# kalj/dealii-cuda

Measured on AMD Instinct MI355X. Metric: DoFs/s on 1305x Laplace vmult (bmop), p=4 3D uniform, higher is better.
Workload: dtype f64; 1 GPU; bmop: DEGREE_FE=4, DIMENSION=3, MATRIX_FREE_UNIFORM_MESH, hyper_cube(-1,1), 54^3 cells, 10218313 DoFs, 1 z-slab(s); cells_per_dir=54, n_dofs=10218313, n_cells=157464, parallelism=slab1, dof_numbering=caller's (lexicographic), finite=True, clock_ramp_steps=2000

## Files before the change

### dealii-cuda_amd/csrc/mfgpu_api.hip

```cpp
#include <hip/hip_runtime.h>

#include <type_traits>

#include <algorithm>
#include <cmath>
#include <cstdlib>
#include <cstring>
#include <memory>
#include <string>
#include <vector>

#include "mfgpu_kernels.h"

using namespace mfgpu;

struct EventTimer {
  std::vector<Event> ev;
  size_t used = 0;
  double ms = 0.0;
  int begin(hipStream_t st) {
    if (used + 2 > ev.size()) {
      Event e0, e1;
      int rc;
      if ((rc = e0.create(hipEventDefault)) || (rc = e1.create(hipEventDefault))) return rc;
      ev.push_back(std::move(e0));
      ev.push_back(std::move(e1));
    }
    HIP_TRY(hipEventRecord(ev[used].get(), st));
    return 0;
  }
  int end(hipStream_t st) {
    HIP_TRY(hipEventRecord(ev[used + 1].get(), st));
    used += 2;
    return 0;
  }
  int drain(double *total) {
    for (size_t i = 0; i + 1 < used; i += 2) {
      float t = 0.f;
      HIP_TRY(hipEventElapsedTime(&t, ev[i].get(), ev[i + 1].get()));
      ms += t;
    }
    used = 0;
    *total = ms;
    return 0;
  }
  void reset() {
    used = 0;
    ms = 0.0;
  }
};

struct mfgpu_handle {
  Plan plan;
  int dim = 0, n = 0, nd = 0, number_type = MFGPU_F64;
  bool hn = false;
  std::vector<double> S, Dt;
  std::vector<double> sv, sg;
  DeviceArray<uint32_t> d_batch_cell_off, d_batch_dof_off, d_bdofs;
  DeviceArray<uint8_t> d_bflags;
  DeviceArray<uint16_t> d_lmap;
  DeviceArray<uint16_t> d_lmapx;
  DeviceArray<uint16_t> d_perm;
  DeviceArray<uint32_t> d_bdofsp, d_idxp;
  DeviceArray<uint32_t> d_shtab;
  bool shared_records = false;
  size_t record_bytes = 0;
  DeviceArray<uint32_t> d_hnrec;
  DeviceArray<uint32_t> d_hn_slot;
  DeviceArray<void> d_coefp;
  DeviceArray<void> d_coef;
  DeviceArray<void> d_mass, d_massp;
  bool updatable = false;
  FoldGeometry geo;
  DeviceArray<uint32_t> d_cell_batch, d_cell_pos;
  size_t n_plane_cells = 0;
  DeviceArray<uint32_t> d_cmask, d_orphans;
  DeviceArray<void> d_hnw;
  DeviceArray<uint32_t> d_constrained;
  uint32_t n_constrained = 0;
  DeviceArray<void> d_tabsd;
  DeviceArray<void> d_tab2;
  bool twopass = true;
  DeviceArray<uint32_t> d_batch_nint, d_halo_off;
  std::vector<uint32_t> seg_end;
  std::vector<DeviceArray<uint32_t>> d_p2arr, d_p2tiles;
  std::vector<uint32_t> n_p2tiles;
  DeviceArray<uint32_t> d_p2rec, d_p2tab;
  bool p2_shared = false, p2_reverse = false, no_shared_records = false;
  Stream side;
  std::vector<Event> ev_seg;
  Event ev_side;
  bool side_pending = false;
  DeviceArray<void> d_halo;
  DeviceArray<unsigned long long> d_stamps;
  size_t lds = 0, device_bytes = 0;
  PlaneKernel planes = PlaneKernel::none;
  BatchKernel batches = BatchKernel::none;
  enum { kPlain, kMasked, kBatch };
  CellKernel<double> kernels_f64[3];
  CellKernel<float> kernels_f32[3];
  template <typename T>
  CellKernel<T> &kernel(int which) {
    if constexpr (std::is_same<T, double>::value) return kernels_f64[which];
    else return kernels_f32[which];
  }
  MultiKernel<double> multi_f64[kMaxFusedWidth - 1];
  MultiKernel<float> multi_f32[kMaxFusedWidth - 1];
  template <typename T>
  MultiKernel<T> &multi(int width) {
    if constexpr (std::is_same<T, double>::value) return multi_f64[width - 2];
    else return multi_f32[width - 2];
  }
  int multi_width = 1;
  DeviceArray<void> d_halo_multi;
  size_t halo_bytes = 0;
  uint32_t n_cus = 0, max_workgroups = 0;
  bool prof = false;
  EventTimer t_cells;
  EventTimer t_pass2;
  uint64_t prof_vmults = 0;
};

namespace {

template <typename T>
hipError_t bind_kernel(const mfgpu_handle *h, PlaneKernel pk, BatchKernel bk, bool hn, bool sh, CellKernel<T> *k) {
  const Plan &P = h->plan;
  const auto bind = pk == PlaneKernel::planes3 ? p_bind<T> : pk == PlaneKernel::planes4 ? q_bind<T>
                    : bk == BatchKernel::batches ? apply_bind<T> : bk == BatchKernel::x ? x_bind<T>
                    : bk == BatchKernel::g ? g_bind<T> : bk == BatchKernel::g2 ? g2_bind<T> : nullptr;
  if (!bind) return hipErrorInvalidValue;
  return bind(P.dim, P.n, hn, h->twopass, sh, h->d_mass.get() != nullptr, P.max_batch_dofs, k);
}

template <typename T>
int launch_bound(mfgpu_handle *h, int which, const ApplyArgs<T> &a, uint32_t nbat, hipStream_t st) {
  const CellKernel<T> &k = h->kernel<T>(which);
  if (!k.launch[0]) {
    set_error("cell-loop kernel not bound");
    return MFGPU_EINVAL;
  }
  uint32_t grid = (uint32_t)(k.per_cu < 1 ? 1 : k.per_cu) * h->n_cus;
  if (h->max_workgroups && h->max_workgroups < grid) grid = h->max_workgroups;
  HIP_TRY(k.launch[a.add != 0](a, h->S.data(), h->Dt.data(), k.lds, nbat < grid ? nbat : grid, st));
  return 0;
}

int check_symmetrize(int n, std::vector<double> &S, std::vector<double> &Dt) {
  const int p = n - 1;
  double err = 0, mag = 0;
  for (int r = 0; r < n; ++r)
    for (int c = 0; c < n; ++c) {
      const double s1 = S[r * n + c], s2 = S[(p - r) * n + (p - c)];
      const double d1 = Dt[r * n + c], d2 = -Dt[(p - r) * n + (p - c)];
      err = std::fmax(err, std::fmax(std::fabs(s1 - s2), std::fabs(d1 - d2)));
      mag = std::fmax(mag, std::fmax(std::fabs(s1), std::fabs(d1)));
    }
  if (err > 1e-10 * mag) {
    set_error("shape tables are not symmetric about the cell midpoint (unsupported)");
    return MFGPU_EUNSUPPORTED;
  }
  for (int r = 0; r < n; ++r)
    for (int c = 0; c < n; ++c) {
      const int r2 = p - r, c2 = p - c;
      if (r * n + c < r2 * n + c2) {
        const double s = 0.5 * (S[r * n + c] + S[r2 * n + c2]);
        S[r * n + c] = S[r2 * n + c2] = s;
        const double d = 0.5 * (Dt[r * n + c] - Dt[r2 * n + c2]);
        Dt[r * n + c] = d;
        Dt[r2 * n + c2] = -d;
      } else if (r == r2 && c == c2) {
        Dt[r * n + c] = 0.0;
      }
    }
  return 0;
}

int upload_pass2(mfgpu_handle *h, const uint32_t *priority, uint32_t n_priority) {
  const Plan &P = h->plan;
  std::vector<uint8_t> prio(P.n_dofs, 0);
  for (uint32_t i = 0; i < n_priority; ++i) {
    if (priority[i] >= P.n_dofs) {
      set_error("priority dof out of range");
      return MFGPU_EINVAL;
    }
    prio[priority[i]] = 1;
  }
  const size_t ng = 1 + h->seg_end.size();
  const bool shared = P.sh_p2_use && !h->no_shared_records && n_priority == 0 && ng == 2;
  std::vector<std::vector<uint32_t>> sd(ng), so(ng, std::vector<uint32_t>(1, 0u)), si(ng);
  auto add = [&](uint32_t dof, const uint32_t *slots, uint32_t k, size_t seg) {
    const size_t g = prio[dof & 0x7fffffffu] ? 0 : 1 + seg;
    sd[g].push_back(dof);
    si[g].insert(si[g].end(), slots, slots + k);
    so[g].push_back((uint32_t)si[g].size());
  };
  for (size_t i = 0; i < P.sdofs.size(); ++i) {
    size_t seg = 0;
    if (shared && P.s_off[i + 1] > P.s_off[i]) continue;
    if (P.s_off[i + 1] > P.s_off[i]) {
      const uint32_t slot = P.s_idx[P.s_off[i + 1] - 1];
      const uint32_t batch = (uint32_t)(std::upper_bound(P.halo_off.begin(), P.halo_off.end(), slot) - P.halo_off.begin()) - 1;
      seg = (size_t)(std::upper_bound(h->seg_end.begin(), h->seg_end.end(), batch) - h->seg_end.begin());
      if (seg >= h->seg_end.size()) seg = h->seg_end.size() - 1;
    }
    add(P.sdofs[i], P.s_idx.data() + P.s_off[i], P.s_off[i + 1] - P.s_off[i], seg);
  }
  const uint32_t zero_slot = P.halo_off.empty() ? 0u : P.halo_off.back();
  for (uint32_t orph : P.orphans) add(orph, &zero_slot, 1, 0);
  std::vector<DeviceArray<uint32_t>> d_arr(ng), d_tiles(ng);
  std::vector<uint32_t> n_tiles(ng, 0u);
  const bool reverse = (size_t)P.halo_off.back() * esize(h->number_type) <= ((size_t)256 << 20);
  DeviceArray<uint32_t> d_rec, d_tab;
  if (shared) {
    int rc;
    if ((rc = d_rec.upload(P.sh_p2rec.data(), P.sh_p2rec.size()))) return rc;
    if ((rc = d_tab.upload(P.sh_p2tab.data(), P.sh_p2tab.size()))) return rc;
  }
  for (size_t g = 0; g < ng; ++g) {
    std::vector<uint32_t> arr, tiles;
    build_pass2_classes(sd[g], so[g], si[g], arr, tiles);
    n_tiles[g] = (uint32_t)(tiles.size() / 4);
    if (reverse) {
      const size_t nt = tiles.size() / 4;
      for (size_t a = 0, b = nt ? nt - 1 : 0; a < b; ++a, --b)
        for (int w = 0; w < 4; ++w) std::swap(tiles[4 * a + w], tiles[4 * b + w]);
    }
    int rc;
    if ((rc = d_arr[g].upload(arr.data(), arr.size()))) return rc;
    if ((rc = d_tiles[g].upload(tiles.data(), tiles.size()))) return rc;
  }
  h->d_p2arr = std::move(d_arr);
  h->d_p2tiles = std::move(d_tiles);
  h->n_p2tiles = std::move(n_tiles);
  h->d_p2rec = std::move(d_rec);
  h->d_p2tab = std::move(d_tab);
  h->p2_shared = shared;
  h->p2_reverse = reverse;
  return 0;
}

template <typename T>
int relayout_planes(mfgpu_handle *h, const uint32_t *cell_batch, const uint32_t *cell_pos, bool coef, bool mass,
                    hipStream_t st) {
  const size_t total = h->n_plane_cells * (size_t)h->nd;
  if (coef)
    HIP_TRY(relayout_coef_launch<T>(h->d_coefp.as<T>(), h->d_coef.as<const T>(), cell_batch, cell_pos, total, h->n, st));
  if (mass)
    HIP_TRY(relayout_coef_launch<T>(h->d_massp.as<T>(), h->d_mass.as<const T>(), cell_batch, cell_pos, total, h->n, st));
  return 0;
}

template <typename T>
int update_typed(mfgpu_handle *h, const void *coef, const void *mass, hipStream_t st) {
  const FoldInputs<T> in = h->geo.inputs<T>();
  if (coef) HIP_TRY(fold_coefficient_launch<T>(h->d_coef.as<T>(), (const T *)coef, in, st));
  if (mass) HIP_TRY(fold_mass_launch<T>(h->d_mass.as<T>(), (const T *)mass, in, st));
  if (h->planes == PlaneKernel::none) return 0;
  return relayout_planes<T>(h, h->d_cell_batch.get(), h->d_cell_pos.get(), coef != nullptr, mass != nullptr, st);
}

template <typename T>
int create_arrays(mfgpu_handle *h, const mfgpu_desc &d) {
  const Plan &P = h->plan;
  const size_t ncell = P.n_cells, nd = (size_t)P.nd;
  size_t &acct = h->device_bytes;
  auto up = [&](auto &arr, const void *src, size_t n) {
    const int rc = arr.upload(src, n);
    acct += arr.bytes();
    return rc;
  };
  int rc;
  if ((rc = up(h->d_batch_cell_off, P.batch_cell_off.data(), P.batch_cell_off.size()))) return rc;
  if ((rc = up(h->d_batch_dof_off, P.batch_dof_off.data(), P.batch_dof_off.size()))) return rc;
  if ((rc = up(h->d_bdofs, P.bdofs.data(), P.bdofs.size()))) return rc;
  if ((rc = up(h->d_bflags, P.bflags.data(), P.bflags.size()))) return rc;
  if ((rc = up(h->d_lmap, P.lmap.data(), P.lmap.size()))) return rc;
  const bool general = h->batches == BatchKernel::g || h->batches == BatchKernel::g2;
  if (h->batches == BatchKernel::x && !h->hn) {
    const int n = P.n, n2 = n * n, PP = n2, CH = 256 / PP, ndl = n2 * n;
    std::vector<uint16_t> perm(512, 0xffff);
    for (int layout = 0; layout < 2; ++layout) {
      uint16_t *lanes = perm.data() + 256 * layout;
      std::vector<int> fill(32, 0), overflow;
      for (int q = 0; q < CH * PP; ++q) {
        const int cell = q / PP, pen = q % PP, a = pen % n, b = pen / n;
        const int base = cell * ndl + (layout == 0 ? a + n2 * b : a + n * b);
        const int r = base & 31;
        if (fill[r] < 8) lanes[32 * fill[r]++ + r] = (uint16_t)q;
        else overflow.push_back(q);
      }
      for (int l = 255; l >= 0 && !overflow.empty(); --l)
        if (lanes[l] == 0xffff) {
          lanes[l] = (uint16_t)overflow.back();
          overflow.pop_back();
        }
    }
    if ((rc = up(h->d_perm, perm.data(), perm.size()))) return rc;
  }
  if (h->batches == BatchKernel::x || general) {
    const size_t n = (size_t)P.n, np = (n + 1) & ~(size_t)1, runs = P.lmap.size() / n;
    std::vector<uint16_t> lx(runs * np, 0);
    for (size_t r = 0; r < runs; ++r)
      for (size_t i = 0; i < n; ++i) lx[r * np + i] = P.lmap[r * n + i];
    if ((rc = up(h->d_lmapx, lx.data(), lx.size()))) return rc;
  }
  if (h->batches == BatchKernel::g2) {
    std::vector<T> sd(2 * (size_t)P.n * P.n);
    for (int i = 0; i < P.n * P.n; ++i) {
      sd[i] = (T)h->S[i];
      sd[P.n * P.n + i] = (T)h->Dt[i];
    }
    if ((rc = up(h->d_tabsd, sd.data(), sd.size() * sizeof(T)))) return rc;
  }
  if (h->planes != PlaneKernel::none) {
    if ((rc = build_plane_records(h->plan, d.constraint_mask))) return rc;
    if (!P.pr_hn.empty()) {
      if ((rc = up(h->d_hnrec, P.pr_hn.data(), P.pr_hn.size()))) return rc;
      if ((rc = up(h->d_hn_slot, P.pr_hn_slot.data(), P.pr_hn_slot.size()))) return rc;
    }
    h->shared_records = P.sh_use && !(d.flags & MFGPU_NO_SHARED_RECORDS) &&
                        kernel_exists(h->planes, P.n, d.number_type, false, true, d.mass_coefficient != nullptr);
    const std::vector<uint32_t> &rd = h->shared_records ? P.sh_dofs : P.pr_dofs;
    const std::vector<uint32_t> &rx = h->shared_records ? P.sh_idx : P.pr_idx;
    if ((rc = up(h->d_bdofsp, rd.data(), rd.size()))) return rc;
    if ((rc = up(h->d_idxp, rx.data(), rx.size()))) return rc;
    if (h->shared_records && (rc = up(h->d_shtab, P.sh_batch.data(), P.sh_batch.size()))) return rc;
    h->record_bytes = h->d_bdofsp.bytes() + h->d_idxp.bytes() + h->d_shtab.bytes();
  }
  if ((rc = up(h->d_orphans, P.orphans.data(), P.orphans.size()))) return rc;
  if (h->twopass) {
    if ((rc = up(h->d_batch_nint, P.batch_nint.data(), P.batch_nint.size()))) return rc;
    if ((rc = up(h->d_halo_off, P.halo_off.data(), P.halo_off.size()))) return rc;
    if (h->planes != PlaneKernel::none && (uint64_t)P.halo_off.back() >= (1ull << 29)) {
      set_error("halo buffer too large for 32-bit byte offsets");
      return MFGPU_EUNSUPPORTED;
    }
    const size_t hb = ((size_t)P.halo_off.back() + 1) * sizeof(T);
    if ((rc = h->d_halo.alloc(hb, true))) return rc;
    acct += hb;
    h->halo_bytes = hb;
  }
  if (h->hn) {
    std::vector<uint32_t> cm(ncell);
    for (size_t i = 0; i < ncell; ++i) cm[i] = d.constraint_mask[P.cell_order[i]];
    if ((rc = up(h->d_cmask, cm.data(), ncell))) return rc;
    std::vector<T> w((size_t)h->n * h->n);
    for (size_t i = 0; i < w.size(); ++i) w[i] = (T)d.constraint_weights[i];
    if ((rc = up(h->d_hnw, w.data(), w.size() * sizeof(T)))) return rc;
  }
  FoldGeometry geo;
  if ((rc = geo.upload(d.JxW, d.inv_jac, P.cell_order.data(), P.dim, (uint32_t)ncell, (uint32_t)nd, general,
                       d.number_type)))
    return rc;
  DeviceArray<T> metric;
  if ((rc = fold_coefficient<T>(metric, d.coefficient, d.quadrature_points, geo.inputs<T>()))) return rc;
  h->d_coef = std::move(metric);
  acct += h->d_coef.bytes();
  if (d.mass_coefficient) {
    DeviceArray<T> mass;
    if ((rc = fold_mass<T>(mass, d.mass_coefficient, geo.inputs<T>()))) return rc;
    h->d_mass = std::move(mass);
    acct += h->d_mass.bytes();
  }
  if (h->updatable) {
    acct += geo.bytes();
    h->geo = std::move(geo);
  }
  if (h->planes != PlaneKernel::none) {
    const int n = P.n, NT = p_cells_per_wave(n) * n;
    const size_t nbat = P.n_plane_batches, total = nbat * (size_t)(n * n) * NT;
    const size_t ncell_p = P.batch_cell_off[nbat];
    std::vector<uint32_t> cb(ncell_p), cp(ncell_p);
    for (size_t b = 0; b < nbat; ++b)
      for (uint32_t c = P.batch_cell_off[b]; c < P.batch_cell_off[b + 1]; ++c) {
        cb[c] = (uint32_t)b;
        cp[c] = c - P.batch_cell_off[b];
      }
    DeviceArray<uint32_t> t_cb, t_cp;
    if ((rc = t_cb.upload(cb.data(), ncell_p))) return rc;
    if ((rc = t_cp.upload(cp.data(), ncell_p))) return rc;
    if ((rc = h->d_coefp.alloc(total * sizeof(T), true))) return rc;
    acct += h->d_coefp.bytes();
    h->n_plane_cells = ncell_p;
    if (d.mass_coefficient) {
      if ((rc = h->d_massp.alloc(total * sizeof(T), true))) return rc;
      acct += h->d_massp.bytes();
    }
    if ((rc = relayout_planes<T>(h, t_cb.get(), t_cp.get(), true, d.mass_coefficient != nullptr, nullptr))) return rc;
    HIP_TRY(hipDeviceSynchronize());
    if (h->updatable) {
      acct += t_cb.bytes() + t_cp.bytes();
      h->d_cell_batch = std::move(t_cb);
      h->d_cell_pos = std::move(t_cp);
    }
  }
  int dev = 0;
  hipDeviceProp_t prop;
  HIP_TRY(hipGetDevice(&dev));
  HIP_TRY(hipGetDeviceProperties(&prop, dev));
  h->n_cus = (uint32_t)prop.multiProcessorCount;
  h->max_workgroups = d.max_workgroups;
  if (h->planes != PlaneKernel::none) {
    CellKernel<T> &plain = h->kernel<T>(mfgpu_handle::kPlain), &masked = h->kernel<T>(mfgpu_handle::kMasked);
    HIP_TRY(bind_kernel<T>(h, h->planes, BatchKernel::none, false, h->shared_records, &plain));
    h->lds = plain.lds;
    if (P.n_plain_plane_batches < P.n_plane_batches) {
      HIP_TRY(bind_kernel<T>(h, h->planes, BatchKernel::none, true, false, &masked));
      h->lds = std::max(h->lds, masked.lds);
    }
  }
  if (h->batches == BatchKernel::none) return 0;
  CellKernel<T> &batch = h->kernel<T>(mfgpu_handle::kBatch);
  const hipError_t bind_batch_family = bind_kernel<T>(h, PlaneKernel::none, h->batches, h->hn, false, &batch);
  h->lds = batch.lds;
  if (h->lds > 160 * 1024) {
    set_error("batch needs more than 160 KiB of LDS; lower max_dofs_per_batch");
    return MFGPU_EINVAL;
  }
  HIP_TRY(bind_batch_family);
  if (h->twopass && h->planes == PlaneKernel::none)
    for (const int w : kFusedWidths) {
      if (!fused_kernel_exists(h->batches, P.n, d.number_type, h->hn, h->d_mass.get() != nullptr, w)) continue;
      MultiKernel<T> &mk = h->multi<T>(w);
      if (gm_bind<T>(P.n, h->hn, h->d_mass.get() != nullptr, w, P.max_batch_dofs, &mk) != hipSuccess) {
        (void)hipGetLastError();
        mk = MultiKernel<T>();
      } else
        h->multi_width = std::max(h->multi_width, w);
    }
  return 0;
}

void choose_segments(mfgpu_handle *h, uint32_t request) {
  const Plan &P = h->plan;
  const uint32_t nb = (uint32_t)(P.batch_cell_off.size() - 1);
  h->seg_end.assign(1, nb);
  if (!h->twopass || nb < 2 || request == 1) return;
  const uint32_t npl = P.n_plane_batches, nplain = P.n_plain_plane_batches;
  std::vector<uint32_t> cuts;
  if (npl > 0 && npl < nb) cuts.push_back(npl);
  if (nplain > 0 && nplain < npl) cuts.push_back(nplain);
  if (request > 1) {
    for (uint32_t i = 1; i < request; ++i) cuts.push_back((uint32_t)((uint64_t)nb * i / request));
  }
  if (request == 0 && !P.pr_hn.empty() && nplain == 0 && P.n == 5) cuts.push_back(nb / 2);
  std::sort(cuts.begin(), cuts.end());
  h->seg_end.clear();
  for (uint32_t c : cuts)
    if (c > 0 && c < nb && (h->seg_end.empty() || h->seg_end.back() != c)) h->seg_end.push_back(c);
  h->seg_end.push_back(nb);
}

template <typename T>
int create_typed(mfgpu_handle *h, const mfgpu_desc &d) {
  int rc = create_arrays<T>(h, d);
  if (rc) return rc;
  choose_segments(h, d.cell_loop_segments);
  if (!h->twopass) return 0;
  if (h->seg_end.size() > 1) {
    int prio_least = 0, prio_greatest = 0;
    HIP_TRY(hipDeviceGetStreamPriorityRange(&prio_least, &prio_greatest));
    if ((rc = h->side.create(hipStreamNonBlocking, prio_least))) return rc;
    if ((rc = h->ev_side.create(hipEventDisableTiming))) return rc;
    h->ev_seg.resize(h->seg_end.size() - 1);
    for (Event &e : h->ev_seg)
      if ((rc = e.create(hipEventDisableTiming))) return rc;
  }
  return upload_pass2(h, nullptr, 0);
}

template <typename T>
int launch_pass2_group(mfgpu_handle *h, size_t group, void *dst, const void *src, hipStream_t st, int add) {
  if (h->p2_shared && group == 1)
    HIP_TRY(reduce_owner_batches_launch<T>((T *)dst, (const T *)src, h->d_halo.as<const T>(), h->d_p2rec.get(),
                                           h->d_p2tab.get(), (uint32_t)(h->plan.batch_cell_off.size() - 1),
                                           (uint32_t)p_hs(h->plan.n) * 64u, h->p2_reverse ? 1 : 0, add, st));
  HIP_TRY(reduce_classes_launch<T>((T *)dst, (const T *)src, h->d_halo.as<const T>(), h->d_p2arr[group].get(),
                                   h->d_p2tiles[group].get(), h->n_p2tiles[group], add, st));
  return 0;
}

template <typename T>
int vmult_pass2(mfgpu_handle *h, int phase, void *dst, const void *src, hipStream_t st, int add) {
  if (!h->twopass) return 0;
  if (phase == 0) return launch_pass2_group<T>(h, 0, dst, src, st, add);
  int rc = launch_pass2_group<T>(h, h->seg_end.size(), dst, src, st, add);
  if (!rc && h->side_pending) {
    HIP_TRY(hipStreamWaitEvent(st, h->ev_side.get(), 0));
    h->side_pending = false;
  }
  return rc;
}

template <typename T>
int launch_cells(mfgpu_handle *h, ApplyArgs<T> a, uint32_t b0, uint32_t b1, hipStream_t st) {
  const Plan &P = h->plan;
  const uint32_t npl = P.n_plane_batches, nplain = P.n_plain_plane_batches;
  if (b0 < nplain) {
    a.batch0 = b0;
    a.batch_end = b1 < nplain ? b1 : nplain;
    if (const int rc = launch_bound<T>(h, mfgpu_handle::kPlain, a, a.batch_end - a.batch0, st)) return rc;
    b0 = a.batch_end;
  }
  if (b0 < npl && b0 < b1) {
    a.batch0 = b0;
    a.batch_end = b1 < npl ? b1 : npl;
    if (const int rc = launch_bound<T>(h, mfgpu_handle::kMasked, a, a.batch_end - a.batch0, st)) return rc;
    b0 = a.batch_end;
  }
  if (b0 >= b1) return 0;
  a.batch0 = b0;
  a.batch_end = b1;
  return launch_bound<T>(h, mfgpu_handle::kBatch, a, b1 - b0, st);
}

template <typename T>
ApplyArgs<T> make_args(mfgpu_handle *h, void *dst, const void *src, int add) {
  const Plan &P = h->plan;
  ApplyArgs<T> a;
  a.batch_cell_off = h->d_batch_cell_off.get();
  a.batch_dof_off = h->d_batch_dof_off.get();
  a.bdofs = h->d_bdofs.get();
  a.bflags = h->d_bflags.get();
  a.lmap = h->d_lmap.get();
  a.lmapx = h->d_lmapx.get();
  a.perm = h->d_perm.get();
  a.bdofsp = h->d_bdofsp.get();
  a.idxp = h->d_idxp.get();
  a.shtab = h->shared_records ? h->d_shtab.get() : nullptr;
  a.hnrec = h->d_hnrec.get();
  a.hn_slot = h->d_hn_slot.get();
  a.coefp = h->d_coefp.as<const T>();
  a.coef = h->d_coef.as<const T>();
  a.mass = h->d_mass.as<const T>();
  a.massp = h->d_massp.as<const T>();
  a.cmask = h->d_cmask.get();
  a.hn_weights = h->d_hnw.as<const T>();
  a.tabS = h->d_tabsd.as<const T>();
  a.tabDt = a.tabS ? a.tabS + (size_t)P.n * P.n : nullptr;
  a.batch_nint = h->d_batch_nint.get();
  a.halo_off = h->d_halo_off.get();
  a.halo = h->d_halo.as<T>();
  a.dst = (T *)dst;
  a.src = (const T *)src;
  a.nb_max = P.max_batch_dofs;
  a.add = add;
  a.stamps = h->d_stamps.get();
  a.dbg = 0;
  return a;
}

template <typename T>
int vmult_main(mfgpu_handle *h, void *dst, const void *src, hipStream_t st, int add) {
  const Plan &P = h->plan;
  ApplyArgs<T> a = make_args<T>(h, dst, src, add);
  int rc;
  if (h->prof && (rc = h->t_cells.begin(st))) return rc;
  if (h->twopass) {
    const size_t nseg = h->seg_end.size();
    if (h->side_pending) {
      HIP_TRY(hipStreamWaitEvent(st, h->ev_side.get(), 0));
      h->side_pending = false;
    }
    for (size_t s = 0; s < nseg; ++s) {
      if ((rc = launch_cells<T>(h, a, s ? h->seg_end[s - 1] : 0u, h->seg_end[s], st))) return rc;
      if (s + 1 < nseg) {
        HIP_TRY(hipEventRecord(h->ev_seg[s].get(), st));
        HIP_TRY(hipStreamWaitEvent(h->side.get(), h->ev_seg[s].get(), 0));
        if ((rc = launch_pass2_group<T>(h, 1 + s, dst, src, h->side.get(), add))) return rc;
      }
    }
    if (nseg > 1) {
      HIP_TRY(hipEventRecord(h->ev_side.get(), h->side.get()));
      h->side_pending = true;
    }
  } else {
    for (size_t c = 0; c + 1 < P.color_batch_off.size(); ++c) {
      if (P.color_batch_off[c + 1] == P.color_batch_off[c]) continue;
      if ((rc = launch_cells<T>(h, a, P.color_batch_off[c], P.color_batch_off[c + 1], st))) return rc;
    }
  }
  if (h->prof && (rc = h->t_cells.end(st))) return rc;
  if (!h->twopass)
    HIP_TRY(orphan_launch<T>((T *)dst, (const T *)src, h->d_orphans.get(), (uint32_t)P.orphans.size(), add, st));
  if (h->prof) h->prof_vmults++;
  return 0;
}

template <typename T>
int vmult_typed(mfgpu_handle *h, void *dst, const void *src, hipStream_t st, int add) {
  int rc = vmult_main<T>(h, dst, src, st, add);
  if (rc) return rc;
  const bool timed = h->prof && h->twopass;
  if (timed && (rc = h->t_pass2.begin(st))) return rc;
  rc = vmult_pass2<T>(h, 0, dst, src, st, add);
  if (!rc) rc = vmult_pass2<T>(h, 1, dst, src, st, add);
  if (!rc && timed) rc = h->t_pass2.end(st);
  return rc;
}

bool fused_by_default(int , int ) { return false; }

template <typename T>
int multi_fused_group(mfgpu_handle *h, T *dst, const T *src, int nv, size_t stride, hipStream_t st, int add) {
  const MultiKernel<T> &k = h->multi<T>(nv);
  if (!k.launch[0]) {
    set_error("fused kernel not bound");
    return MFGPU_EINVAL;
  }
  if (!h->d_halo_multi.get()) {
    const size_t bytes = (size_t)(h->multi_width - 1) * h->halo_bytes;
    if (const int rc = h->d_halo_multi.alloc(bytes, true)) return rc;
    HIP_TRY(hipStreamSynchronize(nullptr));
    h->device_bytes += bytes;
  }
  if (h->side_pending) {
    HIP_TRY(hipStreamWaitEvent(st, h->ev_side.get(), 0));
    h->side_pending = false;
  }
  MultiArgs<T> a;
  static_cast<ApplyArgs<T> &>(a) = make_args<T>(h, dst, src, add);
  a.stride = stride;
  for (int v = 0; v < kMaxFusedWidth; ++v)
    a.halos[v] = v == 0 ? a.halo
                 : v < nv ? reinterpret_cast<T *>(static_cast<char *>(h->d_halo_multi.get()) + (size_t)(v - 1) * h->halo_bytes)
                          : nullptr;
  const uint32_t nbat = (uint32_t)(h->plan.batch_cell_off.size() - 1);
  a.batch0 = 0;
  a.batch_end = nbat;
  uint32_t grid = (uint32_t)(k.per_cu < 1 ? 1 : k.per_cu) * h->n_cus;
  if (h->max_workgroups && h->max_workgroups < grid) grid = h->max_workgroups;
// ... 187 lines not shown
    set_error("JxW, inv_jac, shape tables and coefficient (or quadrature_points) are required");
    return MFGPU_EINVAL;
  }
  const bool hn = (d.flags & MFGPU_HANGING_NODES) != 0;
  if (hn && (!d.constraint_mask || !d.constraint_weights)) {
    set_error("MFGPU_HANGING_NODES needs constraint_mask and constraint_weights");
    return MFGPU_EINVAL;
  }
  std::unique_ptr<mfgpu_handle, decltype(&mfgpu_destroy)> h(new mfgpu_handle(), mfgpu_destroy);
  int rc = choose_kernel_and_plan(d, h->planes, h->batches, h->plan);
  if (rc) return rc;
  h->dim = d.dim;
  h->n = d.degree + 1;
  h->nd = h->plan.nd;
  h->number_type = d.number_type;
  h->hn = hn;
  h->twopass = !(d.flags & MFGPU_COLORED_SCATTER);
  h->no_shared_records = (d.flags & MFGPU_NO_SHARED_RECORDS) != 0;
  h->updatable = (d.flags & MFGPU_UPDATABLE_COEFFICIENTS) != 0;
  const int nn = h->n * h->n;
  std::vector<double> sv(nn), sg(nn);
  for (int i = 0; i < nn; ++i) {
    sv[i] = d.number_type == MFGPU_F64 ? ((const double *)d.shape_values)[i] : ((const float *)d.shape_values)[i];
    sg[i] = d.number_type == MFGPU_F64 ? ((const double *)d.shape_gradients)[i] : ((const float *)d.shape_gradients)[i];
  }
  h->sv = sv;
  h->sg = sg;
  rc = derive_tables(h->n, sv.data(), sg.data(), h->S, h->Dt);
  if (!rc) rc = check_symmetrize(h->n, h->S, h->Dt);
  if (!rc) rc = d.number_type == MFGPU_F64 ? create_typed<double>(h.get(), d) : create_typed<float>(h.get(), d);
  if (!rc && d.n_constrained) {
    h->n_constrained = d.n_constrained;
    rc = h->d_constrained.upload(d.constrained_dofs, d.n_constrained);
    h->device_bytes += h->d_constrained.bytes();
  }
  if (rc) return rc;
  *out = h.release();
  return 0;
}

void mfgpu_destroy(mfgpu_handle *h) {
  if (!h) return;
  if (h->side.get()) hipStreamSynchronize(h->side.get());
  delete h;
}

int mfgpu_vmult(mfgpu_handle *h, void *dst, const void *src, void *stream) {
  if (!h || !dst || !src) {
    set_error("null argument");
    return MFGPU_EINVAL;
  }
  if (dst == src) {
    set_error("vmult: dst and src must not alias");
    return MFGPU_EINVAL;
  }
  return h->number_type == MFGPU_F64 ? vmult_typed<double>(h, dst, src, (hipStream_t)stream, 0)
                                     : vmult_typed<float>(h, dst, src, (hipStream_t)stream, 0);
}

int mfgpu_vmult_add(mfgpu_handle *h, void *dst, const void *src, void *stream) {
  if (!h || !dst || !src) {
    set_error("null argument");
    return MFGPU_EINVAL;
  }
  if (dst == src) {
    set_error("vmult_add: dst and src must not alias");
    return MFGPU_EINVAL;
  }
  return h->number_type == MFGPU_F64 ? vmult_typed<double>(h, dst, src, (hipStream_t)stream, 1)
                                     : vmult_typed<float>(h, dst, src, (hipStream_t)stream, 1);
}

int mfgpu_vmult_multi(mfgpu_handle *h, void *dst, const void *src, uint32_t n_vectors, size_t stride, uint32_t flags,
                      void *stream) {
  if (!h || !dst || !src) {
    set_error("null argument");
    return MFGPU_EINVAL;
  }
  const size_t nd = h->plan.n_dofs;
  if (n_vectors == 0 || (n_vectors > 1 && stride < nd)) {
    set_error("mfgpu_vmult_multi: n_vectors must be >= 1 and stride >= n_dofs");
    return MFGPU_EINVAL;
  }
  if ((flags & ~(MFGPU_MULTI_ADD | MFGPU_MULTI_LOOP | MFGPU_MULTI_FUSED)) ||
      ((flags & MFGPU_MULTI_LOOP) && (flags & MFGPU_MULTI_FUSED))) {
    set_error("mfgpu_vmult_multi: bad flags (MFGPU_MULTI_LOOP and MFGPU_MULTI_FUSED exclude each other)");
    return MFGPU_EINVAL;
  }
  const size_t bytes = ((size_t)(n_vectors - 1) * stride + nd) * esize(h->number_type);
  const char *d0 = (const char *)dst, *s0 = (const char *)src;
  if (d0 < s0 + bytes && s0 < d0 + bytes) {
    set_error("mfgpu_vmult_multi: the dst range overlaps the src range");
    return MFGPU_EINVAL;
  }
  return h->number_type == MFGPU_F64 ? vmult_multi_typed<double>(h, dst, src, n_vectors, stride, flags, (hipStream_t)stream)
                                     : vmult_multi_typed<float>(h, dst, src, n_vectors, stride, flags, (hipStream_t)stream);
}

int mfgpu_multi_width(const mfgpu_handle *h) { return h ? h->multi_width : 0; }

int mfgpu_update_coefficients(mfgpu_handle *h, const void *coefficient_dev, const void *mass_coefficient_dev,
                              void *stream) {
  if (!h) {
    set_error("null argument");
    return MFGPU_EINVAL;
  }
  if (!h->updatable) {
    set_error("mfgpu_update_coefficients: the handle was created without MFGPU_UPDATABLE_COEFFICIENTS");
    return MFGPU_EINVAL;
  }
  if (!coefficient_dev && !mass_coefficient_dev) {
    set_error("mfgpu_update_coefficients: coefficient_dev and mass_coefficient_dev are both NULL");
    return MFGPU_EINVAL;
  }
  if (mass_coefficient_dev && !h->d_mass.get()) {
    set_error("mfgpu_update_coefficients: the handle was created without a mass term (its kernels have no mass "
              "instantiation bound); create it with mass_coefficient");
    return MFGPU_EINVAL;
  }
  return h->number_type == MFGPU_F64 ? update_typed<double>(h, coefficient_dev, mass_coefficient_dev, (hipStream_t)stream)
                                     : update_typed<float>(h, coefficient_dev, mass_coefficient_dev, (hipStream_t)stream);
}

uint32_t mfgpu_n_dofs(const mfgpu_handle *h) { return h ? h->plan.n_dofs : 0; }

size_t mfgpu_memory_consumption(const mfgpu_handle *h) { return h ? h->device_bytes : 0; }

int mfgpu_plan_stats(const mfgpu_handle *h, uint64_t s[8]) {
  if (!h || !s) return MFGPU_EINVAL;
  const Plan &P = h->plan;
  s[0] = P.batch_cell_off.size() - 1;
  s[1] = P.color_batch_off.size() - 1;
  s[2] = P.bdofs.size();
  s[3] = P.max_batch_dofs;
  s[4] = P.max_batch_cells;
  s[5] = P.orphans.size();
  s[6] = P.n_first;
  s[7] = P.n_add;
  if (h->twopass) {
    const uint32_t nb = (uint32_t)s[0], npl = P.n_plane_batches, nplain = P.n_plain_plane_batches;
    const uint32_t edge[4] = {0u, nplain, npl, nb};
    s[1] = 0;
    for (size_t g = 0; g < h->seg_end.size(); ++g) {
      const uint32_t s0 = g ? h->seg_end[g - 1] : 0u, s1 = h->seg_end[g];
      for (int f = 0; f < 3; ++f)
        if (std::max(s0, edge[f]) < std::min(s1, edge[f + 1])) ++s[1];
    }
    s[6] = P.sdofs.size();
    s[7] = P.halo_off.back();
  }
  return 0;
}

int mfgpu_record_stats(const mfgpu_handle *h, uint64_t s[4]) {
  if (!h || !s) return MFGPU_EINVAL;
  const Plan &P = h->plan;
  const size_t n = (size_t)P.n, nb = (size_t)p_kgu((int)n) * 64, nx = ((n * n + 1) / 2) * (p_cells_per_wave((int)n) * n);
  const bool planes = h->planes != PlaneKernel::none;
  s[0] = (h->shared_records ? 1 : 0) | (h->p2_shared ? 2 : 0);
  s[1] = planes ? P.sh_dofs.size() / nb : 0;
  s[2] = planes ? P.sh_idx.size() / nx : 0;
  s[3] = h->record_bytes;
  return 0;
}

const char *mfgpu_kernel_name(const mfgpu_handle *h) {
  if (!h) return "";
  const bool x = h->batches == BatchKernel::x;
  switch (h->planes) {
    case PlaneKernel::planes3: return x ? "apply_planes3+apply_batches_x" : "apply_planes3";
    case PlaneKernel::planes4: return x ? "apply_planes4+apply_batches_x" : "apply_planes4";
    default: break;
  }
  switch (h->batches) {
    case BatchKernel::x: return "apply_batches_x";
    case BatchKernel::g: return "apply_batches_g";
    case BatchKernel::g2: return "apply_batches_g2";
    default: return "apply_batches";
  }
}

int mfgpu_profile_enable(mfgpu_handle *h, int on) {
  if (!h) return MFGPU_EINVAL;
  h->prof = on != 0;
  h->t_cells.reset();
  h->t_pass2.reset();
  h->prof_vmults = 0;
  return 0;
}

int mfgpu_profile_read_pass2(mfgpu_handle *h, double *ms) {
  if (!h || !ms) return MFGPU_EINVAL;
  HIP_TRY(hipDeviceSynchronize());
  return h->t_pass2.drain(ms);
}

int mfgpu_profile_read(mfgpu_handle *h, double *ms, uint64_t *nv) {
  if (!h || !ms || !nv) return MFGPU_EINVAL;
  HIP_TRY(hipDeviceSynchronize());
  if (const int rc = h->t_cells.drain(ms)) return rc;
  *nv = h->prof_vmults;
  return 0;
}

#ifdef MFGPU_STAMPS
int mfgpu_debug_stamps(mfgpu_handle *h, unsigned long long *out, size_t n_batches) {
  if (!h) return MFGPU_EINVAL;
  const size_t nbt = h->plan.batch_cell_off.size() - 1;
  if (!h->d_stamps.get()) return h->d_stamps.alloc(2 * nbt * 16, true);
  if (out && n_batches == nbt) {
    HIP_TRY(hipDeviceSynchronize());
    HIP_TRY(hipMemcpy(out, h->d_stamps.get(), 2 * nbt * 16 * sizeof(unsigned long long), hipMemcpyDeviceToHost));
  }
  return 0;
}
#endif


int mfgpu_compute_inverse_diagonal(mfgpu_handle *h, void *inv_diag, void *stream) {
  if (!h || !inv_diag) {
    set_error("null argument");
    return MFGPU_EINVAL;
  }
  return h->number_type == MFGPU_F64 ? inverse_diagonal_typed<double>(h, inv_diag, (hipStream_t)stream)
                                     : inverse_diagonal_typed<float>(h, inv_diag, (hipStream_t)stream);
}

int mfgpu_set_constrained_values(mfgpu_handle *h, void *vec, double value, void *stream) {
  if (!h || !vec) {
    set_error("null argument");
    return MFGPU_EINVAL;
  }
  if (h->number_type == MFGPU_F64)
    HIP_TRY(set_values_launch<double>((double *)vec, h->d_constrained.get(), h->n_constrained, value, (hipStream_t)stream));
  else
    HIP_TRY(set_values_launch<float>((float *)vec, h->d_constrained.get(), h->n_constrained, (float)value,
                                     (hipStream_t)stream));
  return 0;
}

int mfgpu_vec_sadd(void *v, double s, double a, const void *w, size_t n, int nt, void *stream) {
  return vec_map(0, v, w, s, a, n, nt, stream);
}
int mfgpu_vec_equ(void *v, double a, const void *w, size_t n, int nt, void *stream) {
  return vec_map(1, v, w, 0.0, a, n, nt, stream);
}
int mfgpu_vec_scale(void *v, const void *w, size_t n, int nt, void *stream) {
  return vec_map(2, v, w, 0.0, 0.0, n, nt, stream);
}
int mfgpu_vec_divide(void *v, const void *w, size_t n, int nt, void *stream) {
  return vec_map(3, v, w, 0.0, 0.0, n, nt, stream);
}
int mfgpu_vec_invert(void *v, size_t n, int nt, void *stream) { return vec_map(4, v, nullptr, 0.0, 0.0, n, nt, stream); }
int mfgpu_vec_mul(void *v, double a, size_t n, int nt, void *stream) {
  return vec_map(5, v, nullptr, 0.0, a, n, nt, stream);
}
int mfgpu_vec_dot(const void *v, const void *w, size_t n, int nt, void *stream, double *result) {
  return vec_reduce(0, const_cast<void *>(v), nullptr, w, 0.0, n, nt, stream, result);
}
int mfgpu_vec_l2_norm(const void *v, size_t n, int nt, void *stream, double *result) {
  int rc = vec_reduce(0, const_cast<void *>(v), nullptr, v, 0.0, n, nt, stream, result);
  if (!rc) *result = std::sqrt(*result);
  return rc;
}
int mfgpu_vec_add_and_dot(void *v, double a, const void *x, const void *w, size_t n, int nt, void *stream,
                          double *result) {
  return vec_reduce(1, v, x, w, a, n, nt, stream, result);
}
int mfgpu_vec_all_zero(const void *v, size_t n, int nt, void *stream, int *result) {
  if (!result) return MFGPU_EINVAL;
  double cnt = 0.0;
  int rc = vec_reduce(2, const_cast<void *>(v), nullptr, nullptr, 0.0, n, nt, stream, &cnt);
  if (!rc) *result = cnt == 0.0;
  return rc;
}

int mfgpu_vec_alloc(void **dev, size_t n, int nt) {
  if (!dev) return MFGPU_EINVAL;
  *dev = nullptr;
  if (n == 0) return 0;
  HIP_TRY(hipMalloc(dev, n * esize(nt)));
  HIP_TRY(hipMemset(*dev, 0, n * esize(nt)));
  return 0;
}
int mfgpu_vec_free(void *dev) {
  if (dev) HIP_TRY(hipFree(dev));
  return 0;
}
int mfgpu_vec_fill(void *dev, size_t n, int nt, double value, void *stream) {
  if (!dev && n) return MFGPU_EINVAL;
  if (nt == MFGPU_F32)
    HIP_TRY(fill_launch<float>((float *)dev, n, (float)value, (hipStream_t)stream));
  else
    HIP_TRY(fill_launch<double>((double *)dev, n, value, (hipStream_t)stream));
  return 0;
}
int mfgpu_vec_from_host(void *dev, const void *host, size_t n, int nt) {
  if (n) HIP_TRY(hipMemcpy(dev, host, n * esize(nt), hipMemcpyHostToDevice));
  return 0;
}
int mfgpu_vec_to_host(void *host, const void *dev, size_t n, int nt) {
  if (n) HIP_TRY(hipMemcpy(host, dev, n * esize(nt), hipMemcpyDeviceToHost));
  return 0;
}
int mfgpu_device_synchronize(void) {
  HIP_TRY(hipDeviceSynchronize());
  return 0;
}
int mfgpu_device_memory_info(size_t *free_bytes, size_t *total_bytes) {
  if (!free_bytes || !total_bytes) return MFGPU_EINVAL;
  HIP_TRY(hipMemGetInfo(free_bytes, total_bytes));
  return 0;
}

}
// ... 1 lines not shown
```

### dealii-cuda_amd/csrc/mfgpu_internal.h

```cpp
#ifndef MFGPU_INTERNAL_H
#define MFGPU_INTERNAL_H

#include <cstdint>
#include <string>
#include <vector>

#include "../../include/mfgpu.h"

namespace mfgpu {

void set_error(const std::string &msg);

inline int ipow(int a, int e) {
  int r = 1;
  for (int i = 0; i < e; ++i) r *= a;
  return r;
}

constexpr int p_cells_per_wave(int n) { return 64 / n; }
constexpr int p_ji(int n) { return n == 3 ? 2 : n == 4 ? 5 : n == 5 ? 9 : n == 6 ? 14 : 23; }
constexpr int p_hs(int n) { return n == 3 ? 3 : n == 4 ? 6 : n == 5 ? 9 : n == 6 ? 14 : 18; }
constexpr int p_kgu(int n) { return p_ji(n) + p_hs(n); }
constexpr int p_cell_stride(int n) {
  int s = n * n * n;
  while ((s & 31) != (n & 31)) ++s;
  return s;
}

constexpr int q_plane_stride(int n) { return n >= 6 ? 65 : n == 5 ? 33 : n == 4 ? 17 : 33; }
constexpr int q_cell_stride(int n) { return n * q_plane_stride(n); }
constexpr int p_priv_max(int n) { return n >= 5 ? 384 : n == 4 ? 256 : 192; }
constexpr int kHnOpRounds = 2;
constexpr int p_hn_rows(int n) { return p_priv_max(n) / 64 + 3 * kHnOpRounds * 3 + 2; }

template <typename T>
constexpr size_t q_region_doubles(int n) {
  const size_t t = ((size_t)(p_cells_per_wave(n) + 1) * q_cell_stride(n) * sizeof(T) + 7) / 8;
  const size_t u = (size_t)p_kgu(n) * 64 + p_priv_max(n);
  return t > u ? t : u;
}
template <typename T>
constexpr size_t q_lds_bytes(int n, bool hn) {
  return (q_region_doubles<T>(n) + (hn ? (size_t)n * n : 0)) * 8;
}

constexpr uint8_t kFlagConstrained = 1;
constexpr uint8_t kFlagAdd = 2;

struct Plan {
  int dim = 0, degree = 0, n = 0, nd = 0;
  uint32_t n_dofs = 0, n_cells = 0;
  std::vector<uint32_t> cell_order;
  std::vector<uint32_t> batch_cell_off;
  std::vector<uint32_t> batch_dof_off;
  std::vector<uint32_t> color_batch_off;
  std::vector<uint32_t> bdofs;
  std::vector<uint8_t> bflags;
  std::vector<uint16_t> lmap;
  std::vector<uint32_t> orphans;
  std::vector<uint32_t> batch_nint;
  std::vector<uint32_t> halo_off;
  std::vector<uint32_t> sdofs;
  std::vector<uint32_t> s_off;
  std::vector<uint32_t> s_idx;
  std::vector<uint32_t> chunks;
  std::vector<uint32_t> gstarts;
  uint32_t max_batch_dofs = 0, max_batch_cells = 0;
  uint32_t n_plane_batches = 0;
  uint32_t n_plain_plane_batches = 0;
  std::vector<uint32_t> pr_dofs, pr_idx, pr_hn, pr_hn_slot;
  std::vector<uint32_t> sh_dofs, sh_idx, sh_batch;
  bool sh_use = false;
  std::vector<uint32_t> sh_p2rec, sh_p2tab;
  bool sh_p2_use = false;
  uint64_t n_first = 0, n_add = 0;
};

struct PlanLimits {
  uint32_t max_cells = 0, max_dofs = 0;
  uint32_t interior_max = 0, shared_max = 0, halo_stride = 0;
  bool segregate_masked = false;
  bool masked_planes = false;
  uint32_t private_max = 0;
};

int build_plan(const mfgpu_desc &d, Plan &plan, uint32_t max_chunks = 3, const PlanLimits *limits = nullptr);

struct HnLine {
  uint16_t node[8];
};
void hn_cell_lines(unsigned mask, int n, std::vector<HnLine> (&lines)[3], std::vector<uint16_t> &nodes);

enum class PlaneKernel : uint8_t { none, planes3, planes4 };
enum class BatchKernel : uint8_t { none, batches, x, g, g2 };
int choose_kernel_and_plan(const mfgpu_desc &d, PlaneKernel &pk, BatchKernel &bk, Plan &plan);

constexpr bool planes4_wide(int n) { return n >= 6; }
constexpr bool kernel_exists(PlaneKernel k, int n, int number_type, bool hn, bool sh, bool mass) {
  switch (k) {
    case PlaneKernel::planes3: return n >= 3 && n <= 5 && !(sh && hn);
    case PlaneKernel::planes4:
      return planes4_wide(n) ? n <= 7 && !hn && !sh && !mass
                             : n >= 3 && !sh && !(mass && n == 5 && number_type == MFGPU_F64);
    default: return false;
  }
}
constexpr bool kernel_exists(BatchKernel k, int n, int , bool , bool sh, bool ) {
  return k != BatchKernel::none && n >= 2 && n <= 7 && !sh;
}
constexpr int kFusedWidths[] = {3, 2};
constexpr bool fused_kernel_exists(BatchKernel k, int n, int number_type, bool hn, bool , int nv) {
  return k == BatchKernel::g && n >= 2 && n <= 7 && (nv == 2 || nv == 3) &&
         !(hn && number_type == MFGPU_F64 && n >= (nv == 3 ? 6 : 7));
}
std::vector<uint32_t> multi_groups(uint32_t n_vectors, const std::vector<uint32_t> &widths);
int build_plane_records(Plan &plan, const uint32_t *constraint_mask);
constexpr int kShBatchWords = 4;
constexpr double kShareMaxFraction = 0.5;
void share_plane_records(Plan &plan);
constexpr int kP2Header = 16, kP2MaxK = 12, kP2SlotBits = 12;
void share_pass2_records(Plan &plan);

int derive_tables(int n, const double *shape_values, const double *shape_gradients,
                  std::vector<double> &S, std::vector<double> &Dt);

int handle_number_type(const mfgpu_handle *h);
int handle_set_priority_dofs(mfgpu_handle *h, const uint32_t *ids, uint32_t n);
int handle_vmult_phase(mfgpu_handle *h, int phase, void *dst, const void *src, void *stream, int add);
int handle_n_batches(const mfgpu_handle *h);
bool handle_ranged_ok(const mfgpu_handle *h);
int handle_batches_touching(const mfgpu_handle *h, const uint32_t *ids, uint32_t n, std::vector<uint8_t> &flags);
int handle_cells_range(mfgpu_handle *h, uint32_t b0, uint32_t b1, void *dst, const void *src, void *stream, int add);
int handle_cells_two_ranges(mfgpu_handle *h, uint32_t b0, uint32_t b1, uint32_t c0, uint32_t c1, void *dst,
                            const void *src, void *stream, int add);
int handle_pass2_group(mfgpu_handle *h, int group, void *dst, const void *src, void *stream, int add);

}

struct mfgpu_plan {
  mfgpu::Plan plan;
};

#endif
```

### dealii-cuda_amd/csrc/mfgpu_kernels.h

```cpp
#ifndef MFGPU_KERNELS_H
#define MFGPU_KERNELS_H

#include <hip/hip_runtime.h>

#include <type_traits>

#include "mfgpu_device.h"
#include "mfgpu_internal.h"

namespace mfgpu {

template <typename T>
struct ApplyArgs {
  const uint32_t *batch_cell_off;
  const uint32_t *batch_dof_off;
  const uint32_t *bdofs;
  const uint8_t *bflags;
  const uint16_t *lmap;
  const uint16_t *lmapx;
  const uint16_t *perm;
  const uint32_t *bdofsp;
  const uint32_t *idxp;
  const T *coefp;
  const uint32_t *hnrec;
  const uint32_t *hn_slot;
  const T *coef;
  const uint32_t *cmask;
  const T *hn_weights;
  const T *tabS, *tabDt;
  const uint32_t *batch_nint;
  const uint32_t *halo_off;
  T *halo;
  T *dst;
  const T *src;
  uint32_t batch0;
  uint32_t batch_end;
  uint32_t hole0 = 0xffffffffu, hole_len = 0;
  uint32_t nb_max;
  int add;
  unsigned long long *stamps;
  int dbg;
  const uint32_t *shtab = nullptr;
  const T *mass = nullptr;
  const T *massp = nullptr;
};

constexpr int kMaxFusedWidth = 3;
template <typename T>
struct MultiArgs : ApplyArgs<T> {
  size_t stride = 0;
  T *halos[kMaxFusedWidth];
};
constexpr size_t kMaxLdsBytes = 160 * 1024;

template <typename T, int n>
struct Tables {
  T S[((n + 1) / 2) * n];
  T Dt[((n + 1) / 2) * n];
};

template <typename T, int n>
inline Tables<T, n> make_tables(const double *S, const double *Dt) {
  Tables<T, n> tab;
  for (int i = 0; i < ((n + 1) / 2) * n; ++i) {
    tab.S[i] = (T)S[i];
    tab.Dt[i] = (T)Dt[i];
  }
  return tab;
}

template <typename T, typename Args = ApplyArgs<T>>
struct CellKernel {
  size_t lds = 0;
  int per_cu = 0;
  hipError_t (*launch[2])(const Args &a, const double *S, const double *Dt, size_t lds, uint32_t grid,
                          hipStream_t st) = {nullptr, nullptr};
};

template <typename T, int Block, auto K, auto MakeTab, typename Args = ApplyArgs<T>>
hipError_t launch_cell_kernel(const Args &a, const double *S, const double *Dt, size_t lds, uint32_t grid,
                              hipStream_t st) {
  if constexpr (std::is_null_pointer_v<decltype(MakeTab)>)
    hipLaunchKernelGGL(K, dim3(grid), dim3(Block), lds, st, a);
  else
    hipLaunchKernelGGL(K, dim3(grid), dim3(Block), lds, st, a, MakeTab(S, Dt));
  return hipGetLastError();
}

template <typename T, int Block, auto K0, auto K1, auto MakeTab, typename Args = ApplyArgs<T>>
hipError_t bind_cell_kernel(size_t lds, CellKernel<T, Args> *k) {
  k->lds = lds;
  for (const void *f : {(const void *)K1, (const void *)K0})
    if (const hipError_t e = hipFuncSetAttribute(f, hipFuncAttributeMaxDynamicSharedMemorySize, (int)lds)) return e;
  k->launch[0] = launch_cell_kernel<T, Block, K0, MakeTab, Args>;
  k->launch[1] = launch_cell_kernel<T, Block, K1, MakeTab, Args>;
  return hipOccupancyMaxActiveBlocksPerMultiprocessor(&k->per_cu, (const void *)K0, Block, lds);
}

template <typename F>
hipError_t dispatch_flags(F &&f) { return f(); }
template <typename F, typename... B>
hipError_t dispatch_flags(F &&f, bool flag, B... rest) {
  return dispatch_flags(
      [&](auto... c) { return flag ? f(std::true_type{}, c...) : f(std::false_type{}, c...); }, rest...);
}
template <typename F, typename... B>
hipError_t dispatch_instantiation(int n, F &&f, B... flags) {
  auto at = [&](auto N) { return dispatch_flags([&](auto... c) { return f(N, c...); }, flags...); };
  switch (n) {
    case 2: return at(std::integral_constant<int, 2>{});
    case 3: return at(std::integral_constant<int, 3>{});
    case 4: return at(std::integral_constant<int, 4>{});
    case 5: return at(std::integral_constant<int, 5>{});
    case 6: return at(std::integral_constant<int, 6>{});
    case 7: return at(std::integral_constant<int, 7>{});
    default: return hipErrorInvalidValue;
  }
}
template <typename T>
constexpr int number_type_of = sizeof(T) == 8 ? MFGPU_F64 : MFGPU_F32;

#define MFGPU_CELL_LOOP_FAMILY(F)                                                                              \
  template <typename T>                                                                                        \
  hipError_t F##_bind(int dim, int n, bool hn, bool twopass, bool sh, bool mass, uint32_t nb_max, CellKernel<T> *k);
MFGPU_CELL_LOOP_FAMILY(apply)
MFGPU_CELL_LOOP_FAMILY(x)
MFGPU_CELL_LOOP_FAMILY(g)
MFGPU_CELL_LOOP_FAMILY(g2)
MFGPU_CELL_LOOP_FAMILY(p)
MFGPU_CELL_LOOP_FAMILY(q)
#undef MFGPU_CELL_LOOP_FAMILY
template <typename T>
using MultiKernel = CellKernel<T, MultiArgs<T>>;
template <typename T>
hipError_t gm_bind(int n, bool hn, bool mass, int nv, uint32_t nb_max, MultiKernel<T> *k);

void build_pass2_classes(const std::vector<uint32_t> &sdofs, const std::vector<uint32_t> &s_off,
                         const std::vector<uint32_t> &s_idx, std::vector<uint32_t> &arr, std::vector<uint32_t> &tiles);
template <typename T>
hipError_t reduce_classes_launch(T *dst, const T *src, const T *halo, const uint32_t *arr, const uint32_t *tiles,
                                 uint32_t n_tiles, int add, hipStream_t st);
template <typename T>
hipError_t reduce_classes_multi_launch(int nv, T *dst, const T *src, size_t stride, T *const *halos, const uint32_t *arr,
                                       const uint32_t *tiles, uint32_t n_tiles, int add, hipStream_t st);
template <typename T>
hipError_t reduce_owner_batches_launch(T *dst, const T *src, const T *halo, const uint32_t *rec, const uint32_t *tab,
                                       uint32_t n_batches, uint32_t hstride, int reverse, int add, hipStream_t st);
template <typename T>
hipError_t relayout_coef_launch(T *out, const T *in, const uint32_t *cell_batch, const uint32_t *cell_pos,
                                size_t total, int n, hipStream_t st);
template <typename T>
hipError_t fold_general_launch(T *M, const T *coef, const T *jxw, const T *jinv, const uint32_t *order,
                               uint32_t n_cells, uint32_t nd, hipStream_t st);
template <typename T>
hipError_t fold_general2_launch(T *M, const T *coef, const T *jxw, const T *jinv, const uint32_t *order,
                                uint32_t n_cells, uint32_t nd, hipStream_t st);
template <typename T>
hipError_t orphan_launch(T *dst, const T *src, const uint32_t *orph, uint32_t n, int add, hipStream_t st);
template <typename T>
hipError_t coefficient_launch(T *coef, const T *qpts, size_t nq, int dim, hipStream_t st);
template <typename T>
hipError_t fold_launch(T *c, const T *coef, const T *jxw, const T *j0, const uint32_t *order,
                       uint32_t n_cells, uint32_t nd, hipStream_t st);
template <typename T>
hipError_t fill_launch(T *v, size_t n, T a, hipStream_t st);
template <typename T>
struct FoldInputs {
  const T *jxw = nullptr, *jinv = nullptr;
  const uint32_t *order = nullptr;
  int dim = 0;
  uint32_t n_cells = 0, nd = 0;
  bool general = false;
  size_t metric_entries() const { return (size_t)n_cells * nd * (general ? (dim == 3 ? 6 : 3) : 1); }
};
template <typename T>
hipError_t fold_coefficient_launch(T *out, const T *coef, const FoldInputs<T> &in, hipStream_t st);
template <typename T>
hipError_t fold_mass_launch(T *out, const T *c, const FoldInputs<T> &in, hipStream_t st);
struct FoldGeometry {
  DeviceArray<void> jxw, jinv;
  DeviceArray<uint32_t> order;
  int dim = 0;
  uint32_t n_cells = 0, nd = 0;
  bool general = false;
  int upload(const void *JxW, const void *inv_jac, const uint32_t *cell_order, int dim_, uint32_t n_cells_, uint32_t nd_,
             bool general_, int number_type);
  size_t bytes() const { return jxw.bytes() + jinv.bytes() + order.bytes(); }
  template <typename T>
  FoldInputs<T> inputs(const T *jxw_resident = nullptr) const {
    FoldInputs<T> in;
    in.jxw = jxw_resident ? jxw_resident : jxw.as<const T>();
    in.jinv = jinv.as<const T>();
    in.order = order.get();
    in.dim = dim, in.n_cells = n_cells, in.nd = nd, in.general = general;
    return in;
  }
};
template <typename T>
int fold_mass(DeviceArray<T> &out, const void *mass_coefficient, const FoldInputs<T> &in);
template <typename T>
int fold_coefficient(DeviceArray<T> &out, const void *coefficient, const void *quadrature_points,
                     const FoldInputs<T> &in);

template <typename T>
hipError_t diag_launch(int dim, int n, T *diag, uint32_t n_batches, const uint32_t *batch_cell_off,
                       const uint32_t *batch_dof_off, const uint32_t *bdofs, const uint16_t *lmap, const T *coef,
                       const uint32_t *cmask, const T *hn_weights, const T *tab2, hipStream_t st);
template <typename T>
hipError_t diag_general_launch(int n, T *diag, uint32_t n_batches, const uint32_t *batch_cell_off,
                               const uint32_t *batch_dof_off, const uint32_t *bdofs, const uint16_t *lmap,
                               const T *metric, const uint32_t *cmask, const T *hn_weights, const T *tab,
                               hipStream_t st);
template <typename T>
hipError_t diag_general2_launch(int n, T *diag, uint32_t n_batches, const uint32_t *batch_cell_off,
                                const uint32_t *batch_dof_off, const uint32_t *bdofs, const uint16_t *lmap,
                                const T *metric, const uint32_t *cmask, const T *hn_weights, const T *tab,
                                hipStream_t st);
template <typename T>
hipError_t diag_mass_launch(int dim, int n, T *diag, uint32_t n_batches, const uint32_t *batch_cell_off,
                            const uint32_t *batch_dof_off, const uint32_t *bdofs, const uint16_t *lmap, const T *mass,
                            const uint32_t *cmask, const T *hn_weights, const T *tab, bool squared, hipStream_t st);
template <typename T>
hipError_t set_values_launch(T *v, const uint32_t *idx, uint32_t n, T value, hipStream_t st);
template <typename T>
hipError_t vec_map_launch(int op, T *v, const T *w, T s, T a, size_t n, hipStream_t st);
template <typename T>
hipError_t vec_reduce_launch(int op, T *v, const T *x, const T *w, T a, size_t n, hipStream_t st, double *out);

}
#endif
```

### dealii-cuda_amd/csrc/mfgpu_kernels_p.hip

```cpp
#include <hip/hip_runtime.h>

#include "mfgpu_cell.h"
#include "mfgpu_kernels.h"
#include "mfgpu_planes.h"

namespace mfgpu {

#define MFGPU_PIN_VMEM() __builtin_amdgcn_sched_barrier(0x380)

template <int n, typename T, bool ADD, bool HN, bool SH = false, bool MASS = false>
__global__ void __launch_bounds__(64) __attribute__((amdgpu_waves_per_eu(1, 1)))
apply_planes3(const ApplyArgs<T> A, const TablesEO<T, n> tab) {
  constexpr int n2 = n * n;
  constexpr int CW = p_cells_per_wave(n);
  constexpr int NT = CW * n;
  constexpr int KGU = p_kgu(n);
  constexpr int JI = p_ji(n);
  constexpr int HS = KGU - JI;
  constexpr int SA = p_cell_stride(n);
  constexpr int NIW = (n2 + 1) / 2;
  extern __shared__ __attribute__((aligned(16))) unsigned char smem_raw[];
  constexpr int PRIV = HN ? p_priv_max(n) : 0;
  double *ua = reinterpret_cast<double *>(smem_raw);
  T *Aw = reinterpret_cast<T *>(ua + KGU * 64 + PRIV + (HN ? n2 : 0));
  T *Bw = Aw + (CW + 1) * SA;
  double *Wl = ua + KGU * 64 + PRIV;

  const int lane = threadIdx.x;
  if (HN) {
    if (lane < n2) Wl[lane] = (double)A.hn_weights[lane];
  }
  const int lc = lane / n, k = lane - lc * n;
  const bool lane_on = lane < NT;
  const int tk = lane_on ? lane : NT - 1;

  uint32_t b, bstride, bend;
  {
    const uint32_t nbt = A.batch_end - A.batch0 - A.hole_len, G = gridDim.x;
    if (G >= 8 && nbt >= G) {
      const uint32_t xcd = blockIdx.x & 7u, slot = blockIdx.x >> 3;
      const uint32_t q = G >> 3, rem = G & 7u;
      const uint32_t wlo = xcd * q + (xcd < rem ? xcd : rem);
      const uint32_t w = q + (xcd < rem ? 1u : 0u);
      b = A.batch0 + (uint32_t)((uint64_t)nbt * wlo / G) + slot;
      bend = A.batch0 + (uint32_t)((uint64_t)nbt * (wlo + w) / G);
      bstride = w;
    } else {
      b = A.batch0 + blockIdx.x;
      bend = A.batch_end - A.hole_len;
      bstride = G;
    }
  }
  if (b >= bend) return;
  const uint32_t hole0 = A.hole0, hole_len = A.hole_len;
  auto next_of = [&](uint32_t x) {
    const uint32_t l = (x >= hole0 ? x - hole_len : x) + bstride;
    return l < bend ? (l >= hole0 ? l + hole_len : l) : x;
  };
  if (b >= hole0) b += hole_len;
  static_assert(kernel_exists(PlaneKernel::planes3, n, number_type_of<T>, HN, SH, MASS), "no such instantiation");
  struct Meta {
    uint32_t base, drec, irec;
  };
  auto meta_request = [&](uint32_t bb) -> uint32_t {
    return A.shtab[(size_t)bb * kShBatchWords + (lane & (kShBatchWords - 1))];
  };
  auto meta_of = [&](uint32_t v) -> Meta {
    return Meta{(uint32_t)__builtin_amdgcn_readlane((int)v, 0), (uint32_t)__builtin_amdgcn_readlane((int)v, 1),
                (uint32_t)__builtin_amdgcn_readlane((int)v, 2)};
  };

  auto load_dofs = [&](uint32_t rec, uint32_t (&g)[KGU]) {
    const uint32_t *p = A.bdofsp + (size_t)rec * (KGU * 64) + lane;
#pragma unroll
    for (int j = 0; j < KGU; ++j) g[j] = SH ? p[j * 64] : nt_load(p + j * 64);
  };
  auto src_at = [&](uint32_t base, uint32_t g) -> T {
    const T *const sp = SH ? A.src + base : A.src;
    return *reinterpret_cast<const T *>(reinterpret_cast<const char *>(sp) + (uint32_t)(g * (uint32_t)sizeof(T)));
  };
  auto dst_at = [&](uint32_t base, uint32_t g) -> T * {
    T *const dp = SH ? A.dst + base : A.dst;
    return reinterpret_cast<T *>(reinterpret_cast<char *>(dp) + (uint32_t)(g * (uint32_t)sizeof(T)));
  };
  auto load_ix = [&](uint32_t rec, uint32_t (&ix)[NIW]) {
    const uint32_t *p = A.idxp + (size_t)rec * (NIW * NT) + tk;
#pragma unroll
    for (int w = 0; w < NIW; ++w) ix[w] = SH ? p[w * NT] : nt_load(p + w * NT);
  };
  auto stage_src = [&](const uint32_t (&g)[KGU], const T (&sv)[KGU]) {
#pragma unroll
    for (int j = 0; j < KGU; ++j) {
      double v = (double)sv[j];
      if (j >= JI) {
        const unsigned long long keep = (unsigned long long)(long long)~((int)g[j] >> 31);
        v = __longlong_as_double((long long)((unsigned long long)__double_as_longlong(v) & keep));
      }
      ua[lane + j * 64] = v;
    }
  };
  auto ixb = [&](const uint32_t (&ix)[NIW], int i) -> uint32_t {
    return (i & 1) ? (ix[i >> 1] >> 16) : (ix[i >> 1] & 0xffffu);
  };
  auto scatter_slot = [&](int j, uint32_t bb, uint32_t base, uint32_t g, T r, T oldv) {
    if (j < JI) {
      *dst_at(base, g) = ADD ? oldv + r : r;
    } else {
      T *const hp = A.halo + (size_t)bb * (HS * 64) + lane;
      hp[(j - JI) * 64] = r;
    }
  };

  uint32_t b1 = next_of(b), b2 = next_of(b1);
  uint32_t Gp[KGU], Gc[KGU], Gn[KGU], Gnn[KGU];
  uint32_t IXc[NIW], IXn[NIW];
  constexpr int CR = PRIV / 64, HROWS = HN ? p_hn_rows(n) : 1;
  uint32_t Hc[HROWS], Hn[HROWS];
  auto load_hn = [&](uint32_t bb, uint32_t (&H)[HROWS]) {
    const uint32_t slot = A.hn_slot[bb];
    if (slot != 0xffffffffu) {
      const uint32_t *p = A.hnrec + (size_t)slot * (HROWS * 64) + lane;
#pragma unroll
      for (int w = 0; w < HROWS; ++w) H[w] = nt_load(p + w * 64);
    } else {
#pragma unroll
      for (int w = 0; w < HROWS; ++w) H[w] = 0u;
    }
  };
  T Cc[n2];
  T Mm[MASS ? n2 : 1];
  T SVn[KGU], R[KGU], old[KGU];
  Meta Mp{0u, 0u, 0u}, Mc = Mp, M1 = Mp, M2 = Mp;
  uint32_t Mv = 0u;
  if (SH) {
    Mc = meta_of(meta_request(b));
    M1 = meta_of(meta_request(b1));
    M2 = meta_of(meta_request(b2));
    Mp = Mc;
  }
  load_dofs(SH ? Mc.drec : b, Gc);
  load_dofs(SH ? M1.drec : b1, Gn);
  load_ix(SH ? Mc.irec : b, IXc);
  if (HN) load_hn(b, Hc);
  constexpr uint32_t kDummyIx = 8u * (uint32_t)(KGU * 64 - 1) * 0x10001u;
#pragma unroll
  for (int w = 0; w < NIW; ++w) IXc[w] = lane_on ? IXc[w] : kDummyIx;
  {
    const T *p = A.coefp + (size_t)b * (n2 * NT) + tk;
#pragma unroll
    for (int r = 0; r < n2; ++r) Cc[r] = nt_load(p + r * NT);
  }
  if (MASS) {
    const T *p = A.massp + (size_t)b * (n2 * NT) + tk;
#pragma unroll
    for (int r = 0; r < n2; ++r) Mm[r] = nt_load(p + r * NT);
  }
#pragma unroll
  for (int j = 0; j < KGU; ++j) {
    SVn[j] = src_at(Mc.base, Gc[j]);
    Gp[j] = Gc[j];
    R[j] = T(0);
    old[j] = T(0);
  }
  stage_src(Gc, SVn);
  WaveSync::sync();

  const int pxy = lc * SA + n2 * k;
  const int pyz = lc * SA + k;
  uint32_t bp = b;

  while (true) {
    const bool has_next = b1 != b;
    constexpr int kH2 = HN ? HROWS - 2 : 0, kH1 = HN ? HROWS - 1 : 0;
    const uint32_t hn_ncopy = HN ? (uint32_t)__builtin_amdgcn_readfirstlane(Hc[kH2] & 0xffffu) : 0u;
    auto hn_count = [&](int dir) -> uint32_t {
      const uint32_t w = dir == 0 ? Hc[kH2] >> 16 : dir == 1 ? Hc[kH1] & 0xffffu : Hc[kH1] >> 16;
      return (uint32_t)__builtin_amdgcn_readfirstlane(w);
    };
    auto hn_pass = [&](int dir, bool transposed, const double (&Wr)[n2]) {
      const uint32_t count = hn_count(dir);
#pragma unroll
      for (int r = 0; r < kHnOpRounds; ++r) {
        if ((uint32_t)(r * 64) >= count) break;
        const bool on = (uint32_t)(r * 64 + lane) < count;
        const uint32_t *ww = &Hc[CR + (dir * kHnOpRounds + r) * 3];
        double v[n], o[n];
        uint32_t pos[n];
#pragma unroll
        for (int t = 0; t < n; ++t) {
          pos[t] = on ? (ww[t >> 1] >> (16 * (t & 1))) & 0xffffu : (uint32_t)(KGU * 64 + PRIV - 1);
          v[t] = ua[pos[t]];
        }
#pragma unroll
        for (int i = 0; i < n; ++i) {
          double acc = 0.0;
#pragma unroll
          for (int k2 = 0; k2 < n; ++k2) acc = fma(transposed ? Wr[k2 * n + i] : Wr[i * n + k2], v[k2], acc);
          o[i] = acc;
        }
        if (on) {
#pragma unroll
          for (int i = 0; i < n; ++i) ua[pos[i]] = o[i];
        }
      }
    };
    if (HN && hn_ncopy) {
      double Wr[n2];
#pragma unroll
      for (int i = 0; i < n2; ++i) Wr[i] = Wl[i];
      double cv[CR > 0 ? CR : 1];
#pragma unroll
      for (int r = 0; r < CR; ++r) cv[r] = (uint32_t)(r * 64 + lane) < hn_ncopy ? ua[Hc[r] & 0xffffu] : 0.0;
#pragma unroll
      for (int r = 0; r < CR; ++r)
        if ((uint32_t)(r * 64 + lane) < hn_ncopy) ua[Hc[r] >> 16] = cv[r];
      WaveSync::sync();
      hn_pass(0, false, Wr);
      WaveSync::sync();
      hn_pass(1, false, Wr);
      WaveSync::sync();
      hn_pass(2, false, Wr);
      WaveSync::sync();
    }
    STAMP(0);
    RSTAMP(8);
    WGSTAMP(10);
    load_dofs(SH ? M2.drec : b2, Gnn);
    load_ix(SH ? M1.irec : b1, IXn);
    if (SH) Mv = meta_request(next_of(b2));
    if (HN) load_hn(b1, Hn);
    if (ADD) {
#pragma unroll
      for (int j = 0; j < JI; ++j) old[j] = *dst_at(Mp.base, Gp[j]);
    }
    STAMP(1);
    auto hookA = [&](int) {};
    auto hookB = [&](int s) {
      MFGPU_PIN_VMEM();
#pragma unroll
      for (int j = (KGU * s) / (5 * n); j < (KGU * (s + 1)) / (5 * n); ++j)
        scatter_slot(j, bp, Mp.base, Gp[j], R[j], old[j]);
#pragma unroll
      for (int j = (KGU * s) / (5 * n); j < (KGU * (s + 1)) / (5 * n); ++j)
        SVn[j] = src_at(M1.base, Gn[j]);
      MFGPU_PIN_VMEM();
    };
    const T *const cnext = A.coefp + (size_t)b1 * (n2 * NT) + tk;
    const T *const mnext = MASS ? A.massp + (size_t)b1 * (n2 * NT) + tk : nullptr;
    auto hookC = [&](int s) {
      MFGPU_PIN_VMEM();
#pragma unroll
      for (int r = (n2 * s) / (2 * n); r < (n2 * (s + 1)) / (2 * n); ++r)
        Cc[r] = nt_load(cnext + r * NT);
      if (MASS) {
#pragma unroll
        for (int r = (n2 * s) / (2 * n); r < (n2 * (s + 1)) / (2 * n); ++r)
          Mm[r] = nt_load(mnext + r * NT);
      }
      MFGPU_PIN_VMEM();
    };

    {
// ... 253 lines not shown
```

### dealii-cuda_amd/csrc/mfgpu_pass2.hip

```cpp
#include <hip/hip_runtime.h>

#include <algorithm>

#include "mfgpu_kernels.h"

namespace mfgpu {

namespace {

template <typename T, int K>
__device__ __forceinline__ void reduce_two(T *__restrict__ dst, const T *__restrict__ src, const T *__restrict__ halo,
                                           const uint32_t *__restrict__ p, uint32_t cnt, uint32_t i0, uint32_t k,
                                           int add) {
  const uint32_t i1 = i0 + 256u;
  const uint32_t d0 = p[i0], d1 = p[i1];
  constexpr int KU = K > 0 ? K : 1;
  uint32_t s0[KU], s1[KU];
#pragma unroll
  for (int t = 0; t < KU; ++t) {
    s0[t] = p[(size_t)(1 + t) * cnt + i0];
    s1[t] = p[(size_t)(1 + t) * cnt + i1];
  }
  const bool on0 = d0 != 0xffffffffu, on1 = d1 != 0xffffffffu;
  const uint32_t g0 = d0 & 0x7fffffffu, g1 = d1 & 0x7fffffffu;
  T v0 = T(0), v1 = T(0), o0 = T(0), o1 = T(0);
  if (on0) {
    if (d0 >> 31) {
      v0 = src[g0];
    } else {
      T q[KU];
#pragma unroll
      for (int t = 0; t < KU; ++t) q[t] = halo[s0[t]];
      v0 = q[0];
#pragma unroll
      for (int t = 1; t < KU; ++t) v0 += q[t];
      if (K == 0)
        for (uint32_t t = 1; t < k; ++t) v0 += halo[p[(size_t)(1 + t) * cnt + i0]];
    }
    if (add) o0 = dst[g0];
  }
  if (on1) {
    if (d1 >> 31) {
      v1 = src[g1];
    } else {
      T q[KU];
#pragma unroll
      for (int t = 0; t < KU; ++t) q[t] = halo[s1[t]];
      v1 = q[0];
#pragma unroll
      for (int t = 1; t < KU; ++t) v1 += q[t];
      if (K == 0)
        for (uint32_t t = 1; t < k; ++t) v1 += halo[p[(size_t)(1 + t) * cnt + i1]];
    }
    if (add) o1 = dst[g1];
  }
  if (on0) dst[g0] = add ? o0 + v0 : v0;
  if (on1) dst[g1] = add ? o1 + v1 : v1;
}

template <typename T>
__global__ void __launch_bounds__(256)
reduce_classes(T *__restrict__ dst, const T *__restrict__ src, const T *__restrict__ halo,
               const uint32_t *__restrict__ arr, const uint4 *__restrict__ tiles, int add) {
  const uint4 td = tiles[blockIdx.x];
  const uint32_t *p = arr + td.x;
  const uint32_t i0 = td.w + threadIdx.x;
  switch (td.y) {
    case 1: reduce_two<T, 1>(dst, src, halo, p, td.z, i0, 1, add); break;
    case 2: reduce_two<T, 2>(dst, src, halo, p, td.z, i0, 2, add); break;
    case 3: reduce_two<T, 3>(dst, src, halo, p, td.z, i0, 3, add); break;
    case 4: reduce_two<T, 4>(dst, src, halo, p, td.z, i0, 4, add); break;
    case 8: reduce_two<T, 8>(dst, src, halo, p, td.z, i0, 8, add); break;
    default: reduce_two<T, 0>(dst, src, halo, p, td.z, i0, td.y, add); break;
  }
}

template <typename T>
struct MultiHalos {
  const T *h[kMaxFusedWidth];
};

template <typename T, int K, int NV>
__device__ __forceinline__ void reduce_two_multi(T *__restrict__ dst, const T *__restrict__ src, size_t stride,
                                                 const MultiHalos<T> &halos, const uint32_t *__restrict__ p,
                                                 uint32_t cnt, uint32_t i0, uint32_t k, int add) {
  const uint32_t i1 = i0 + 256u;
  const uint32_t d0 = p[i0], d1 = p[i1];
  constexpr int KU = K > 0 ? K : 1;
  uint32_t s0[KU], s1[KU];
#pragma unroll
  for (int t = 0; t < KU; ++t) {
    s0[t] = p[(size_t)(1 + t) * cnt + i0];
    s1[t] = p[(size_t)(1 + t) * cnt + i1];
  }
  const bool on0 = d0 != 0xffffffffu, on1 = d1 != 0xffffffffu;
  const uint32_t g0 = d0 & 0x7fffffffu, g1 = d1 & 0x7fffffffu;
#pragma unroll
  for (int v = 0; v < NV; ++v) {
    const T *__restrict__ halo = halos.h[v];
    const T *__restrict__ sv = src + (size_t)v * stride;
    T *__restrict__ dv = dst + (size_t)v * stride;
    T v0 = T(0), v1 = T(0), o0 = T(0), o1 = T(0);
    if (on0) {
      if (d0 >> 31) {
        v0 = sv[g0];
      } else {
        T q[KU];
#pragma unroll
        for (int t = 0; t < KU; ++t) q[t] = halo[s0[t]];
        v0 = q[0];
#pragma unroll
        for (int t = 1; t < KU; ++t) v0 += q[t];
        if (K == 0)
          for (uint32_t t = 1; t < k; ++t) v0 += halo[p[(size_t)(1 + t) * cnt + i0]];
      }
      if (add) o0 = dv[g0];
    }
    if (on1) {
      if (d1 >> 31) {
        v1 = sv[g1];
      } else {
        T q[KU];
#pragma unroll
        for (int t = 0; t < KU; ++t) q[t] = halo[s1[t]];
        v1 = q[0];
#pragma unroll
        for (int t = 1; t < KU; ++t) v1 += q[t];
        if (K == 0)
          for (uint32_t t = 1; t < k; ++t) v1 += halo[p[(size_t)(1 + t) * cnt + i1]];
      }
      if (add) o1 = dv[g1];
    }
    if (on0) dv[g0] = add ? o0 + v0 : v0;
    if (on1) dv[g1] = add ? o1 + v1 : v1;
  }
}

template <typename T, int NV>
__global__ void __launch_bounds__(256)
reduce_classes_multi(T *__restrict__ dst, const T *__restrict__ src, size_t stride, const MultiHalos<T> halos,
                     const uint32_t *__restrict__ arr, const uint4 *__restrict__ tiles, int add) {
  const uint4 td = tiles[blockIdx.x];
  const uint32_t *p = arr + td.x;
  const uint32_t i0 = td.w + threadIdx.x;
  switch (td.y) {
    case 1: reduce_two_multi<T, 1, NV>(dst, src, stride, halos, p, td.z, i0, 1, add); break;
    case 2: reduce_two_multi<T, 2, NV>(dst, src, stride, halos, p, td.z, i0, 2, add); break;
    case 3: reduce_two_multi<T, 3, NV>(dst, src, stride, halos, p, td.z, i0, 3, add); break;
    case 4: reduce_two_multi<T, 4, NV>(dst, src, stride, halos, p, td.z, i0, 4, add); break;
    case 8: reduce_two_multi<T, 8, NV>(dst, src, stride, halos, p, td.z, i0, 8, add); break;
    default: reduce_two_multi<T, 0, NV>(dst, src, stride, halos, p, td.z, i0, td.y, add); break;
  }
}

template <typename T, int K>
__device__ __forceinline__ void reduce_owned(T *__restrict__ dst, const T *__restrict__ src,
                                             const T *__restrict__ halo, const uint32_t *__restrict__ r, uint32_t e,
                                             uint32_t d, uint32_t kk, uint32_t kw, uint32_t hslot0, uint32_t hstride,
                                             int add) {
  const T *const hb = halo + hslot0;
  auto partial = [&](uint32_t w) -> T {
    return hb[(w >> kP2SlotBits) * hstride + (w & ((1u << kP2SlotBits) - 1u))];
  };
  constexpr int KU = K > 0 ? K : 1;
  uint32_t w[KU];
#pragma unroll
  for (int t = 0; t < KU; ++t) w[t] = (uint32_t)t < kk ? r[r[3 + t] + e] : 0u;
  if (d == 0xffffffffu) return;
  T v;
  if (d >> 31) {
    v = src[d & 0x7fffffffu];
  } else {
    T q[KU];
#pragma unroll
    for (int t = 0; t < KU; ++t) q[t] = (uint32_t)t < kk ? partial(w[t]) : T(0);
    v = q[0];
#pragma unroll
    for (int t = 1; t < KU; ++t)
      if ((uint32_t)t < kk) v += q[t];
    if (K == 0)
      for (uint32_t t = 1; t < kw; ++t)
        if (t < kk) v += partial(r[r[3 + t] + e]);
  }
  T *const out = dst + (d & 0x7fffffffu);
  *out = add ? *out + v : v;
}

template <typename T>
__global__ void __launch_bounds__(256)
reduce_owner_batches(T *__restrict__ dst, const T *__restrict__ src, const T *__restrict__ halo,
                     const uint32_t *__restrict__ rec, const uint2 *__restrict__ tab, uint32_t n_batches,
                     uint32_t hstride, int reverse, int add) {
  const uint32_t ob = reverse ? n_batches - 1u - blockIdx.x : blockIdx.x;
  const uint2 t = tab[ob];
  const uint32_t *const r = rec + t.y;
  const uint32_t e0 = r[1];
  dst += t.x;
  src += t.x;
  for (uint32_t e = threadIdx.x; e < e0; e += 256u) {
    const uint32_t d = r[kP2Header + e], kk = r[kP2Header + e0 + e];
    const uint32_t kw = (uint32_t)__builtin_amdgcn_readfirstlane((int)kk);
    const uint32_t h0 = ob * hstride;
    switch (kw) {
      case 0: break;
      case 1: reduce_owned<T, 1>(dst, src, halo, r, e, d, kk, kw, h0, hstride, add); break;
      case 2: reduce_owned<T, 2>(dst, src, halo, r, e, d, kk, kw, h0, hstride, add); break;
      case 3: reduce_owned<T, 3>(dst, src, halo, r, e, d, kk, kw, h0, hstride, add); break;
      case 4: reduce_owned<T, 4>(dst, src, halo, r, e, d, kk, kw, h0, hstride, add); break;
      case 5: case 6: case 7:
      case 8: reduce_owned<T, 8>(dst, src, halo, r, e, d, kk, kw, h0, hstride, add); break;
      default: reduce_owned<T, 0>(dst, src, halo, r, e, d, kk, kw, h0, hstride, add); break;
    }
  }
}

}

void build_pass2_classes(const std::vector<uint32_t> &sdofs, const std::vector<uint32_t> &s_off,
                         const std::vector<uint32_t> &s_idx, std::vector<uint32_t> &arr, std::vector<uint32_t> &tiles) {
  arr.clear();
  tiles.clear();
  const size_t ns = sdofs.size();
  uint32_t kmax = 0;
  for (size_t i = 0; i < ns; ++i) kmax = std::max(kmax, s_off[i + 1] - s_off[i]);
  std::vector<std::vector<uint32_t>> members(kmax + 1);
  for (size_t i = 0; i < ns; ++i) {
    uint32_t k = s_off[i + 1] - s_off[i];
    if (k == 0) k = 1;
    members[k].push_back((uint32_t)i);
  }
  for (uint32_t k = 1; k <= kmax; ++k) {
    const std::vector<uint32_t> &m = members[k];
    if (m.empty()) continue;
    const uint32_t entries = (uint32_t)((m.size() + 511) / 512 * 512);
    const uint32_t base = (uint32_t)arr.size();
    arr.resize(arr.size() + (size_t)(1 + k) * entries, 0u);
    for (uint32_t e = 0; e < entries; ++e) arr[base + e] = e < m.size() ? sdofs[m[e]] : 0xffffffffu;
    for (size_t e = 0; e < m.size(); ++e) {
      const uint32_t i = m[e], cnt = s_off[i + 1] - s_off[i];
      for (uint32_t t = 0; t < k; ++t) arr[base + (size_t)(1 + t) * entries + e] = t < cnt ? s_idx[s_off[i] + t] : 0u;
    }
    for (uint32_t first = 0; first < entries; first += 512) {
      tiles.push_back(base);
      tiles.push_back(k);
      tiles.push_back(entries);
      tiles.push_back(first);
    }
  }
}

template <typename T>
hipError_t reduce_classes_launch(T *dst, const T *src, const T *halo, const uint32_t *arr, const uint32_t *tiles,
                                 uint32_t n_tiles, int add, hipStream_t st) {
  if (n_tiles == 0) return hipSuccess;
  hipLaunchKernelGGL(reduce_classes<T>, dim3(n_tiles), dim3(256), 0, st, dst, src, halo, arr,
                     reinterpret_cast<const uint4 *>(tiles), add);
  return hipGetLastError();
}
template <typename T>
hipError_t reduce_classes_multi_launch(int nv, T *dst, const T *src, size_t stride, T *const *halos, const uint32_t *arr,
                                       const uint32_t *tiles, uint32_t n_tiles, int add, hipStream_t st) {
  if (n_tiles == 0) return hipSuccess;
  if (nv != 2 && nv != 3) return hipErrorInvalidValue;
  MultiHalos<T> mh;
  for (int v = 0; v < kMaxFusedWidth; ++v) mh.h[v] = v < nv ? halos[v] : nullptr;
  const uint4 *t4 = reinterpret_cast<const uint4 *>(tiles);
  if (nv == 2)
    hipLaunchKernelGGL((reduce_classes_multi<T, 2>), dim3(n_tiles), dim3(256), 0, st, dst, src, stride, mh, arr, t4, add);
  else
    hipLaunchKernelGGL((reduce_classes_multi<T, 3>), dim3(n_tiles), dim3(256), 0, st, dst, src, stride, mh, arr, t4, add);
  return hipGetLastError();
}
template hipError_t reduce_classes_multi_launch<double>(int, double *, const double *, size_t, double *const *,
                                                        const uint32_t *, const uint32_t *, uint32_t, int, hipStream_t);
template hipError_t reduce_classes_multi_launch<float>(int, float *, const float *, size_t, float *const *,
                                                       const uint32_t *, const uint32_t *, uint32_t, int, hipStream_t);
template <typename T>
hipError_t reduce_owner_batches_launch(T *dst, const T *src, const T *halo, const uint32_t *rec, const uint32_t *tab,
                                       uint32_t n_batches, uint32_t hstride, int reverse, int add, hipStream_t st) {
  if (n_batches == 0) return hipSuccess;
  hipLaunchKernelGGL(reduce_owner_batches<T>, dim3(n_batches), dim3(256), 0, st, dst, src, halo, rec,
                     reinterpret_cast<const uint2 *>(tab), n_batches, hstride, reverse, add);
  return hipGetLastError();
}
template hipError_t reduce_owner_batches_launch<double>(double *, const double *, const double *, const uint32_t *,
                                                        const uint32_t *, uint32_t, uint32_t, int, int, hipStream_t);
template hipError_t reduce_owner_batches_launch<float>(float *, const float *, const float *, const uint32_t *,
                                                       const uint32_t *, uint32_t, uint32_t, int, int, hipStream_t);
template hipError_t reduce_classes_launch<double>(double *, const double *, const double *, const uint32_t *,
                                                  const uint32_t *, uint32_t, int, hipStream_t);
template hipError_t reduce_classes_launch<float>(float *, const float *, const float *, const uint32_t *,
                                                 const uint32_t *, uint32_t, int, hipStream_t);

}
```

### dealii-cuda_amd/csrc/mfgpu_plan.cpp

```cpp
#include <algorithm>
#include <cassert>
#include <cmath>
#include <cstring>
#include <numeric>
#include <unordered_map>

#include "mfgpu_internal.h"

namespace mfgpu {

static thread_local std::string g_err;
void set_error(const std::string &msg) { g_err = msg; }
const char *last_error() { return g_err.c_str(); }

int derive_tables(int n, const double *sv, const double *sg, std::vector<double> &S,
                  std::vector<double> &Dt) {
  std::vector<long double> A(n * n), B(n * n);
  for (int i = 0; i < n * n; ++i) {
    A[i] = sv[i];
    B[i] = sg[i];
  }
  for (int c = 0; c < n; ++c) {
    int piv = c;
    for (int r = c + 1; r < n; ++r)
// ... 327 lines not shown
      for (size_t k = 0; k < cand.size(); ++k) {
        const uint32_t c2 = cand[k];
        if (cell_batch[c2] != NONE) continue;
        cand[w++] = c2;
        if (gain[c2] > best_gain) {
          best_gain = gain[c2];
          best = c2;
        }
      }
      cand.resize(w);
      if (best == NONE) break;
      if (ndofs + (nd - best_gain) > NBmax_b) break;
      if (cls && masked_planes && npriv + priv_of(best) > limits->private_max) break;
      next = best;
    }
    if (last_ok == 0) last_ok = 1;
    for (size_t k = last_ok; k < cells.size(); ++k) cell_batch[cells[k]] = NONE;
    cells.resize(last_ok);
    if (seed < nc && cell_batch[seed] != b) seed = 0;
  }
  if (segregate && !masked_planes) {
    std::vector<uint32_t> idx(batches.size());
    std::iota(idx.begin(), idx.end(), 0u);
    std::stable_sort(idx.begin(), idx.end(), [&](uint32_t a, uint32_t b2) { return batch_masked[a] < batch_masked[b2]; });
    std::vector<std::vector<uint32_t>> sorted_batches(batches.size());
    std::vector<uint8_t> sorted_masked(batches.size());
    for (size_t k = 0; k < idx.size(); ++k) {
      sorted_batches[k] = std::move(batches[idx[k]]);
      sorted_masked[k] = batch_masked[idx[k]];
    }
    batches.swap(sorted_batches);
    batch_masked.swap(sorted_masked);
  } else if (!segregate) {
    batch_masked.assign(batches.size(), 0);
  }
  uint32_t nb = (uint32_t)batches.size();
  if ((d.flags & MFGPU_HANGING_NODES) && d.constraint_mask)
    for (auto &cells : batches)
      std::stable_partition(cells.begin(), cells.end(), [&](uint32_t c) { return d.constraint_mask[c] != 0; });

  const uint32_t interior_max = limits ? limits->interior_max : 0u;
  std::vector<std::vector<uint32_t>> bd;
  std::vector<uint32_t> ntouch, nint;
  std::vector<uint8_t> shared_flag;
  for (;;) {
    nb = (uint32_t)batches.size();
    bd.assign(nb, {});
    ntouch.assign(N, 0);
    for (uint32_t b = 0; b < nb; ++b) {
      std::vector<uint32_t> &v = bd[b];
      v.reserve(batches[b].size() * nd);
      for (uint32_t c : batches[b])
        for (uint32_t i = 0; i < nd; ++i) v.push_back(l2g[(uint64_t)c * nd + i]);
      std::sort(v.begin(), v.end());
      v.erase(std::unique(v.begin(), v.end()), v.end());
      if (v.size() > (batch_masked[b] && !masked_planes ? NBmax1 : NBmax) || v.size() > 8191u) {
        set_error("internal: batch exceeds the kernel's dof slots (degenerate loc2glob?)");
        return MFGPU_EINVAL;
      }
      for (uint32_t g : v) ntouch[g]++;
    }
    shared_flag.assign(N, 0);
    for (uint32_t g = 0; g < N; ++g) shared_flag[g] = ntouch[g] >= 2;
    if (interior_max)
      for (uint32_t b = 0; b < nb; ++b)
        if (!batch_masked[b] || masked_planes)
          for (uint32_t g : bd[b])
            if (ntouch[g] == 1 && constrained[g]) shared_flag[g] = 1;
    nint.assign(nb, 0);
    std::vector<uint32_t> too_big;
    for (uint32_t b = 0; b < nb; ++b) {
      std::vector<uint32_t> &v = bd[b];
      std::stable_partition(v.begin(), v.end(), [&](uint32_t g) { return !shared_flag[g]; });
      uint32_t k = 0;
      while (k < v.size() && !shared_flag[v[k]]) ++k;
      if (interior_max && (!batch_masked[b] || masked_planes)) {
        uint32_t keep = std::min(k, interior_max);
        if (keep == v.size() && keep > 0) --keep;
        for (uint32_t t = keep; t < k; ++t) shared_flag[v[t]] = 1;
        k = keep;
        if (v.size() - k > limits->shared_max) too_big.push_back(b);
      }
      nint[b] = k;
    }
    if (too_big.empty()) break;
    for (size_t i = too_big.size(); i-- > 0;) {
      const uint32_t b = too_big[i];
      if (batches[b].size() < 2) {
        set_error("one cell has more pass-2 dofs than the plane kernel's dof-list slots hold");
        return MFGPU_EUNSUPPORTED;
      }
      const size_t half = batches[b].size() / 2;
      std::vector<uint32_t> second(batches[b].begin() + half, batches[b].end());
      batches[b].resize(half);
      batches.insert(batches.begin() + b + 1, std::move(second));
      batch_masked.insert(batch_masked.begin() + b + 1, batch_masked[b]);
    }
  }

  std::vector<uint64_t> dof_colors(N, 0);
  std::vector<uint32_t> bcolor(nb, 0);
  uint32_t ncolors = 0;
  for (uint32_t b = 0; b < nb; ++b) {
    uint64_t forbidden = 0;
    for (uint32_t g : bd[b]) forbidden |= dof_colors[g];
    uint32_t c = 0;
    while (c < 64 && (forbidden >> c) & 1) ++c;
    if (c >= 64) {
      set_error("more than 64 batch colours needed");
      return MFGPU_EUNSUPPORTED;
    }
    bcolor[b] = c;
    ncolors = std::max(ncolors, c + 1);
    for (uint32_t g : bd[b]) dof_colors[g] |= (1ull << c);
  }
  const bool colored = (d.flags & MFGPU_COLORED_SCATTER) != 0;
  std::vector<uint32_t> order(nb);
  std::iota(order.begin(), order.end(), 0u);
  if (colored) {
    std::stable_sort(order.begin(), order.end(),
                     [&](uint32_t a, uint32_t b2) { return bcolor[a] < bcolor[b2]; });
    P.color_batch_off.assign(ncolors + 1, 0);
    for (uint32_t b = 0; b < nb; ++b) P.color_batch_off[bcolor[b] + 1]++;
    for (uint32_t c = 0; c < ncolors; ++c) P.color_batch_off[c + 1] += P.color_batch_off[c];
  } else {
    P.color_batch_off.assign({0u, nb});
  }

  std::vector<uint32_t> rank_of(nb);
  for (uint32_t k = 0; k < nb; ++k) rank_of[order[k]] = k;
  std::vector<uint32_t> shared_ids;
  for (uint32_t g = 0; g < N; ++g)
    if (shared_flag[g]) shared_ids.push_back(g);
  const size_t ns = shared_ids.size();
  std::vector<uint32_t> sid(N, NONE), t_off(ns + 1, 0);
  for (size_t i = 0; i < ns; ++i) {
    sid[shared_ids[i]] = (uint32_t)i;
    t_off[i + 1] = t_off[i] + ntouch[shared_ids[i]];
  }
  std::vector<uint32_t> touchers(t_off[ns]);
  {
    std::vector<uint32_t> fill(t_off.begin(), t_off.end() - 1);
    for (uint32_t k = 0; k < nb; ++k)
      for (size_t t = nint[order[k]]; t < bd[order[k]].size(); ++t) touchers[fill[sid[bd[order[k]][t]]]++] = k;
  }
  auto seq_less = [&](uint32_t a, uint32_t b2) {
    const uint32_t la = t_off[a + 1] - t_off[a], lb = t_off[b2 + 1] - t_off[b2];
    const uint32_t *pa = &touchers[t_off[a]], *pb = &touchers[t_off[b2]];
    for (uint32_t i = 0; i < la && i < lb; ++i)
      if (pa[i] != pb[i]) return pa[i] < pb[i];
    if (la != lb) return la < lb;
    return a < b2;
  };
  auto same_group = [&](uint32_t a, uint32_t b2) {
    const uint32_t la = t_off[a + 1] - t_off[a], lb = t_off[b2 + 1] - t_off[b2];
    return la == lb && std::equal(&touchers[t_off[a]], &touchers[t_off[a]] + la, &touchers[t_off[b2]]);
  };
  std::vector<uint32_t> sorder(ns);
  std::iota(sorder.begin(), sorder.end(), 0u);
  std::sort(sorder.begin(), sorder.end(), seq_less);
  std::vector<uint32_t> spos(N, NONE);
  for (size_t i = 0; i < ns; ++i) spos[shared_ids[sorder[i]]] = (uint32_t)i;
  for (uint32_t b = 0; b < nb; ++b)
    std::sort(bd[b].begin() + nint[b], bd[b].end(), [&](uint32_t x, uint32_t y) { return spos[x] < spos[y]; });

  P.cell_order.clear();
  P.cell_order.reserve(nc);
  P.batch_cell_off.assign(1, 0);
  P.batch_dof_off.assign(1, 0);
  P.bdofs.clear();
  P.bflags.clear();
  P.lmap.assign((size_t)nc * nd, 0);
  std::vector<uint8_t> touched(N, 0);
  std::vector<uint16_t> pos_in_batch(N, 0);
  P.max_batch_dofs = P.max_batch_cells = 0;
  P.n_first = P.n_add = 0;
  P.batch_nint.clear();
  P.halo_off.assign(1, 0);
  for (uint32_t k = 0; k < nb; ++k) {
    const uint32_t b = order[k];
    const std::vector<uint32_t> &v = bd[b];
    P.batch_nint.push_back(nint[b]);
    P.halo_off.push_back(P.halo_off.back() +
                         (interior_max && (!batch_masked[b] || masked_planes) ? limits->halo_stride
                                                                              : (uint32_t)(v.size() - nint[b])));
    for (uint32_t g : v) {
      uint8_t f = 0;
      if (constrained[g]) f |= kFlagConstrained;
      if (touched[g]) {
        f |= kFlagAdd;
        ++P.n_add;
      } else {
        touched[g] = 1;
        ++P.n_first;
      }
      P.bdofs.push_back(g | (constrained[g] ? 0x80000000u : 0u));
      P.bflags.push_back(f);
    }
    for (size_t t = 0; t < v.size(); ++t) pos_in_batch[v[t]] = (uint16_t)t;
    for (uint32_t c : batches[b]) {
      const size_t pos = P.cell_order.size();
      P.cell_order.push_back(c);
      for (uint32_t i = 0; i < nd; ++i) P.lmap[pos * nd + i] = pos_in_batch[l2g[(uint64_t)c * nd + i]];
    }
    P.batch_cell_off.push_back((uint32_t)P.cell_order.size());
    P.batch_dof_off.push_back((uint32_t)P.bdofs.size());
    P.max_batch_dofs = std::max<uint32_t>(P.max_batch_dofs, (uint32_t)v.size());
    P.max_batch_cells = std::max<uint32_t>(P.max_batch_cells, (uint32_t)batches[b].size());
  }
  P.n_plane_batches = P.n_plain_plane_batches = 0;
  if (interior_max) {
    for (uint32_t k = 0; k < nb; ++k) {
      P.n_plain_plane_batches += batch_masked[order[k]] ? 0u : 1u;
      P.n_plane_batches += (batch_masked[order[k]] && !masked_planes) ? 0u : 1u;
    }
    if (masked_planes && P.n_plain_plane_batches < P.n_plane_batches) P.n_plain_plane_batches = 0;
  }
  P.orphans.clear();
  for (uint32_t g = 0; g < N; ++g)
    if (!touched[g]) P.orphans.push_back(g | (constrained[g] ? 0x80000000u : 0u));
  {
    P.sdofs.resize(ns);
    for (size_t i = 0; i < ns; ++i) {
      const uint32_t g = shared_ids[sorder[i]];
      P.sdofs[i] = g | (constrained[g] ? 0x80000000u : 0u);
    }
    P.s_off.assign(ns + 1, 0);
    for (size_t i = 0; i < ns; ++i) P.s_off[i + 1] = P.s_off[i] + ntouch[P.sdofs[i] & 0x7fffffffu];
    P.s_idx.assign(P.s_off[ns], 0);
    std::vector<uint32_t> fill(P.s_off.begin(), P.s_off.end() - 1);
    for (uint32_t k = 0; k < nb; ++k) {
      const uint32_t ni = P.batch_nint[k];
      const uint32_t d0 = P.batch_dof_off[k], d1 = P.batch_dof_off[k + 1];
      for (uint32_t t = d0 + ni; t < d1; ++t) {
        const uint32_t g = P.bdofs[t] & 0x7fffffffu;
        P.s_idx[fill[spos[g]]++] = P.halo_off[k] + (t - d0 - ni);
      }
    }
    P.chunks.clear();
    P.gstarts.clear();
    for (size_t i = 0; i < ns;) {
      size_t j = i + 1;
      while (j < ns && same_group(sorder[i], sorder[j])) ++j;
      const uint32_t k = P.s_off[i + 1] - P.s_off[i], tstart = (uint32_t)P.gstarts.size();
      for (uint32_t t = 0; t < k; ++t) P.gstarts.push_back(P.s_idx[P.s_off[i] + t]);
      for (size_t o = i; o < j; o += 64) {
        const uint32_t cnt = (uint32_t)std::min<size_t>(64, j - o);
        P.chunks.push_back((uint32_t)o);
        P.chunks.push_back(cnt | (k << 16));
        P.chunks.push_back(tstart);
        P.chunks.push_back((uint32_t)(o - i));
      }
      i = j;
    }
  }
  return 0;
}

int build_plane_records(Plan &P, const uint32_t *constraint_mask) {
  const int n = P.n, n2 = n * n, NT = p_cells_per_wave(n) * n, NIW = (n2 + 1) / 2;
  const int JI = p_ji(n) * 64, NB = p_kgu(n) * 64;
  const size_t nbat = P.n_plane_batches;
  const uint32_t dummy = 8u * (uint32_t)(NB - 1);
  std::vector<uint32_t> &bd = P.pr_dofs, &ix = P.pr_idx;
  bd.assign((size_t)NB * nbat, 0u);
  ix.assign((size_t)NIW * NT * nbat, dummy | (dummy << 16));
  std::vector<uint32_t> slot_of;
  const int HROWS = p_hn_rows(n), CR = p_priv_max(n) / 64;
  std::vector<uint32_t> &hnrec = P.pr_hn;
  hnrec.clear();
  P.pr_hn_slot.assign(nbat, 0xffffffffu);
  std::vector<HnLine> lines[3];
  std::vector<uint16_t> pnodes;
  std::vector<uint32_t> priv_pos((size_t)P.nd);
  for (size_t b = 0; b < nbat; ++b) {
    const uint32_t c0 = P.batch_cell_off[b], nc = P.batch_cell_off[b + 1] - c0;
    const uint32_t d0 = P.batch_dof_off[b], nbd = P.batch_dof_off[b + 1] - d0, ni = P.batch_nint[b];
    if ((int)nc * n > NT || (int)ni > JI || (int)(nbd - ni) >= NB - JI || nbd == ni) {
      set_error("internal: batch does not fit the plane kernel's dof-list slots");
      return MFGPU_EINVAL;
    }
    slot_of.assign(nbd, 0u);
    for (uint32_t t = 0; t < nbd; ++t) slot_of[t] = t < ni ? t : (uint32_t)JI + (t - ni);
    for (int t = 0; t < NB; ++t) {
      uint32_t src_t;
      if (t < JI) src_t = (uint32_t)t < ni ? (uint32_t)t : ni;
      else src_t = std::min<uint32_t>(ni + (uint32_t)(t - JI), nbd - 1);
      bd[b * NB + t] = P.bdofs[d0 + src_t];
    }
    bool hnb = false;
    if (constraint_mask && b >= P.n_plain_plane_batches)
      for (uint32_t c = 0; c < nc; ++c) hnb = hnb || constraint_mask[P.cell_order[c0 + c]] != 0;
    uint32_t next_priv = (uint32_t)NB;
    std::vector<uint32_t> copies, ops_d[3];
    for (uint32_t c = 0; c < nc; ++c) {
      const unsigned mask = hnb ? constraint_mask[P.cell_order[c0 + c]] : 0u;
      std::fill(priv_pos.begin(), priv_pos.end(), 0xffffffffu);
      if (mask) {
        hn_cell_lines(mask, n, lines, pnodes);
        for (uint16_t node : pnodes) {
          if (next_priv >= (uint32_t)NB + (uint32_t)p_priv_max(n)) {
            set_error("internal: batch exceeds the plane kernel's private hanging-node entries");
            return MFGPU_EINVAL;
          }
          priv_pos[node] = next_priv;
          copies.push_back((next_priv << 16) | slot_of[P.lmap[(size_t)(c0 + c) * P.nd + node]]);
          ++next_priv;
        }
        for (int dir = 0; dir < 3; ++dir)
          for (const HnLine &L : lines[dir]) {
            uint32_t w[3] = {0u, 0u, 0u};
            for (int t = 0; t < n; ++t) w[t >> 1] |= priv_pos[L.node[t]] << (16 * (t & 1));
            ops_d[dir].insert(ops_d[dir].end(), w, w + 3);
          }
      }
      for (int k = 0; k < n; ++k)
        for (int i = 0; i < n2; ++i) {
          const int node = i + n2 * k;
          const uint32_t pos = priv_pos[node] != 0xffffffffu ? priv_pos[node] : slot_of[P.lmap[(size_t)(c0 + c) * P.nd + node]];
          const uint32_t off = 8u * pos;
          uint32_t &w = ix[(b * NIW + i / 2) * NT + c * n + k];
          w = (i & 1) ? ((w & 0xffffu) | (off << 16)) : ((w & 0xffff0000u) | off);
        }
    }
    if (hnb) {
      P.pr_hn_slot[b] = (uint32_t)(hnrec.size() / ((size_t)HROWS * 64));
      hnrec.resize(hnrec.size() + (size_t)HROWS * 64, 0u);
      uint32_t *rec = hnrec.data() + (size_t)P.pr_hn_slot[b] * HROWS * 64;
      for (size_t e = 0; e < copies.size(); ++e) rec[e] = copies[e];
      for (int dir = 0; dir < 3; ++dir) {
        const size_t nops = ops_d[dir].size() / 3;
        if (nops > (size_t)kHnOpRounds * 64) {
          set_error("internal: more hanging-node lines in a batch than the plane kernel's record holds");
          return MFGPU_EINVAL;
        }
        for (size_t e = 0; e < nops; ++e)
          for (int w = 0; w < 3; ++w)
            rec[(size_t)(CR + (dir * kHnOpRounds + (int)(e / 64)) * 3 + w) * 64 + e % 64] = ops_d[dir][e * 3 + w];
      }
      const uint32_t h0 = (uint32_t)copies.size() | ((uint32_t)(ops_d[0].size() / 3) << 16);
      const uint32_t h1 = (uint32_t)(ops_d[1].size() / 3) | ((uint32_t)(ops_d[2].size() / 3) << 16);
      for (int l = 0; l < 64; ++l) {
        rec[(size_t)(HROWS - 2) * 64 + l] = h0;
        rec[(size_t)(HROWS - 1) * 64 + l] = h1;
      }
    }
  }
  share_plane_records(P);
  share_pass2_records(P);
  return 0;
}

namespace {
uint64_t hash_words(const uint32_t *w, size_t n) {
  uint64_t h = 1469598103934665603ull;
  for (size_t i = 0; i < n; ++i) h = (h ^ w[i]) * 1099511628211ull;
  return h;
}

uint32_t intern_record(std::vector<uint32_t> &table, std::unordered_multimap<uint64_t, uint32_t> &seen,
                       const uint32_t *rec, size_t len) {
  const uint64_t h = hash_words(rec, len);
  const auto range = seen.equal_range(h);
  for (auto it = range.first; it != range.second; ++it)
    if (!std::memcmp(table.data() + (size_t)it->second * len, rec, len * sizeof(uint32_t))) return it->second;
  const uint32_t id = (uint32_t)(table.size() / len);
  table.insert(table.end(), rec, rec + len);
  seen.emplace(h, id);
  return id;
}
}

void share_plane_records(Plan &P) {
  const int n = P.n, NT = p_cells_per_wave(n) * n, NIW = (n * n + 1) / 2;
  const size_t NB = (size_t)p_kgu(n) * 64, NX = (size_t)NIW * NT, nbat = P.n_plane_batches;
  P.sh_dofs.clear();
  P.sh_idx.clear();
  P.sh_batch.assign(nbat * kShBatchWords, 0u);
  std::unordered_multimap<uint64_t, uint32_t> seen_d, seen_x;
  std::vector<uint32_t> rel(NB);
  for (size_t b = 0; b < nbat; ++b) {
    const uint32_t *g = P.pr_dofs.data() + b * NB;
    uint32_t base = 0x7fffffffu;
    for (size_t t = 0; t < NB; ++t) base = std::min(base, g[t] & 0x7fffffffu);
    for (size_t t = 0; t < NB; ++t) rel[t] = g[t] - base;
    uint32_t *e = P.sh_batch.data() + b * kShBatchWords;
    e[0] = base;
    e[1] = intern_record(P.sh_dofs, seen_d, rel.data(), NB);
    e[2] = intern_record(P.sh_idx, seen_x, P.pr_idx.data() + b * NX, NX);
  }
  const size_t shared = P.sh_dofs.size() + P.sh_idx.size() + P.sh_batch.size();
  const size_t expanded = P.pr_dofs.size() + P.pr_idx.size();
  P.sh_use = nbat > 0 && P.pr_hn.empty() && (double)shared <= kShareMaxFraction * (double)expanded;
}

void share_pass2_records(Plan &P) {
  P.sh_p2rec.clear();
  P.sh_p2tab.clear();
  P.sh_p2_use = false;
  const size_t nb = P.batch_cell_off.size() - 1;
  const uint32_t hs = (uint32_t)p_hs(P.n) * 64u;
  if (nb == 0 || P.n_plane_batches != nb || P.halo_off.size() != nb + 1 || hs > (1u << kP2SlotBits)) return;
  for (size_t b = 0; b <= nb; ++b)
    if (P.halo_off[b] != (uint64_t)b * hs) return;
  std::vector<std::vector<uint32_t>> owned(nb);
  size_t expanded = 0;
  for (size_t i = 0; i < P.sdofs.size(); ++i) {
    const uint32_t k = P.s_off[i + 1] - P.s_off[i];
    expanded += 1 + (k ? k : 1);
    if (k == 0) continue;
    if (k > (uint32_t)kP2MaxK) return;
    const uint32_t owner = P.s_idx[P.s_off[i]] / hs;
    for (uint32_t t = 0; t < k; ++t) {
      const uint32_t tb = P.s_idx[P.s_off[i] + t] / hs;
      if (tb >= nb || tb < owner || tb - owner >= (1u << (32 - kP2SlotBits))) return;
    }
    owned[owner].push_back((uint32_t)i);
  }
  P.sh_p2tab.assign(2 * nb, 0u);
  std::unordered_multimap<uint64_t, std::pair<uint32_t, uint32_t>> seen;
  std::vector<uint32_t> rec;
  for (size_t b = 0; b < nb; ++b) {
    std::vector<uint32_t> &m = owned[b];
    auto k_of = [&](uint32_t i) { return P.s_off[i + 1] - P.s_off[i]; };
    std::stable_sort(m.begin(), m.end(), [&](uint32_t x, uint32_t y) { return k_of(x) > k_of(y); });
    const uint32_t base = P.sh_batch[b * kShBatchWords], ne = (uint32_t)m.size(), kmax = ne ? k_of(m[0]) : 0u;
    auto pad = [](uint32_t x) { return (x + 63u) & ~63u; };
    const uint32_t e0 = pad(ne);
    rec.assign(kP2Header, 0u);
    rec[0] = ne;
    rec[1] = e0;
    rec[2] = kmax;
    rec.resize(kP2Header + 2 * (size_t)e0, 0u);
    for (uint32_t e = 0; e < e0; ++e) rec[kP2Header + e] = e < ne ? P.sdofs[m[e]] - base : 0xffffffffu;
    for (uint32_t e = 0; e < ne; ++e) rec[kP2Header + e0 + e] = k_of(m[e]);
    for (uint32_t t = 0; t < kmax; ++t) {
      uint32_t cnt = 0;
      while (cnt < ne && k_of(m[cnt]) > t) ++cnt;
      rec[3 + t] = (uint32_t)rec.size();
      rec.resize(rec.size() + pad(cnt), 0u);
      for (uint32_t e = 0; e < cnt; ++e) {
        const uint32_t slot = P.s_idx[P.s_off[m[e]] + t], tb = slot / hs;
        rec[rec[3 + t] + e] = ((tb - (uint32_t)b) << kP2SlotBits) | (slot - tb * hs);
      }
    }
    const uint64_t h = hash_words(rec.data(), rec.size());
    uint32_t off = 0xffffffffu;
    const auto range = seen.equal_range(h);
    for (auto it = range.first; it != range.second && off == 0xffffffffu; ++it)
      if (it->second.second == rec.size() &&
          !std::memcmp(P.sh_p2rec.data() + it->second.first, rec.data(), rec.size() * sizeof(uint32_t)))
        off = it->second.first;
    if (off == 0xffffffffu) {
      off = (uint32_t)P.sh_p2rec.size();
      P.sh_p2rec.insert(P.sh_p2rec.end(), rec.begin(), rec.end());
      seen.emplace(h, std::make_pair(off, (uint32_t)rec.size()));
    }
    P.sh_p2tab[2 * b] = base;
    P.sh_p2tab[2 * b + 1] = off;
  }
  const size_t shared = P.sh_p2rec.size() + P.sh_p2tab.size();
  P.sh_p2_use = (double)shared <= kShareMaxFraction * (double)expanded;
}

int choose_kernel_and_plan(const mfgpu_desc &d, PlaneKernel &pk, BatchKernel &bk, Plan &plan) {
  const bool general = !(d.flags & MFGPU_UNIFORM_J0), hn = (d.flags & MFGPU_HANGING_NODES) != 0;
  const bool colored = (d.flags & MFGPU_COLORED_SCATTER) != 0;
  if (d.kernel > MFGPU_KERNEL_PLANES_2W) {
    set_error("unknown mfgpu_desc.kernel");
    return MFGPU_EINVAL;
  }
  const bool pk_ok = d.dim == 3 && !general && !colored && d.degree >= 2 && d.degree <= 6 &&
                     d.n_dofs < (1u << 29);
  const bool xk_ok = d.dim == 3 && !general && !colored;
  const bool want_planes = d.kernel == MFGPU_KERNEL_PLANES || d.kernel == MFGPU_KERNEL_PLANES_2W;
  if ((want_planes && !pk_ok) || (d.kernel == MFGPU_KERNEL_PENCILS_X && !xk_ok) ||
      (d.kernel == MFGPU_KERNEL_PENCILS && general)) {
    set_error("mfgpu_desc.kernel: this kernel family does not cover the description (see include/mfgpu.h)");
    return MFGPU_EUNSUPPORTED;
  }
  const bool planes4 = d.kernel == MFGPU_KERNEL_PLANES_2W || d.degree >= 5 ||
                       (d.kernel == MFGPU_KERNEL_AUTO && d.degree == 3 && d.number_type == MFGPU_F64);
  const PlaneKernel plane_kind = planes4 ? PlaneKernel::planes4 : PlaneKernel::planes3;
  const bool mass = d.mass_coefficient != nullptr;
  auto plane_kernel_exists = [&](bool with_hn) {
    return kernel_exists(plane_kind, d.degree + 1, d.number_type, with_hn, false, mass);
  };
  const bool mass_without_planes = mass && pk_ok && !plane_kernel_exists(false);
  if (mass_without_planes && want_planes) {
    set_error("mfgpu_desc.kernel: this plane kernel has no mass-term instantiation at this degree (apply_planes4w at "
              "p = 5, 6; apply_planes4 at p = 4 in double); use MFGPU_KERNEL_AUTO or MFGPU_KERNEL_PENCILS_X");
    return MFGPU_EUNSUPPORTED;
  }
  bool planes = pk_ok && !mass_without_planes && (want_planes || (d.kernel == MFGPU_KERNEL_AUTO &&
                                     (d.degree >= 4 || (d.degree == 3 && (hn || d.number_type == MFGPU_F64)))));
  bool pencils_x = xk_ok && !planes && d.kernel != MFGPU_KERNEL_PENCILS;
  PlanLimits lim;
  if (planes) {
    lim.max_cells = (uint32_t)p_cells_per_wave(d.degree + 1);
    lim.max_dofs = (uint32_t)p_kgu(d.degree + 1) * 64u - 1u;
    lim.interior_max = (uint32_t)p_ji(d.degree + 1) * 64u;
    lim.halo_stride = (uint32_t)p_hs(d.degree + 1) * 64u;
    lim.shared_max = lim.halo_stride - 1u;
    lim.segregate_masked = hn;
    lim.masked_planes = hn && plane_kernel_exists(true);
    lim.private_max = (uint32_t)p_priv_max(d.degree + 1);
  }
  int rc = build_plan(d, plan, (pencils_x && d.degree == 3) ? 4u : 3u, planes ? &lim : nullptr);
  if (rc == MFGPU_EUNSUPPORTED && planes && d.kernel == MFGPU_KERNEL_AUTO && xk_ok) {
    planes = false;
    pencils_x = true;
    plan = Plan();
    rc = build_plan(d, plan, d.degree == 3 ? 4u : 3u, nullptr);
  }
  if (!rc && planes) {
    const uint32_t nbat = (uint32_t)plan.batch_cell_off.size() - 1;
    pencils_x = plan.n_plane_batches < nbat;
    if (plan.n_plane_batches == 0) planes = false;
  }
  pk = planes ? plane_kind : PlaneKernel::none;
  bk = pencils_x ? BatchKernel::x : general ? (d.dim == 2 ? BatchKernel::g2 : BatchKernel::g)
                                   : planes ? BatchKernel::none : BatchKernel::batches;
  assert(rc || (pk != PlaneKernel::none) == (plan.n_plane_batches > 0));
  return rc;
}

}

namespace mfgpu {
std::vector<uint32_t> multi_groups(uint32_t n_vectors, const std::vector<uint32_t> &widths) {
  std::vector<uint32_t> groups;
  uint32_t left = n_vectors;
  for (uint32_t w : widths)
    for (; w > 1 && left >= w; left -= w) groups.push_back(w);
  groups.insert(groups.end(), left, 1u);
  return groups;
}
}

extern "C" {

const char *mfgpu_last_error(void) { return mfgpu::last_error(); }

int mfgpu_plan_create(const mfgpu_desc *desc, mfgpu_plan **out) {
  if (!desc || !out) {
    mfgpu::set_error("null argument");
    return MFGPU_EINVAL;
  }
  mfgpu_plan *p = new mfgpu_plan();
  mfgpu::PlaneKernel pk;
  mfgpu::BatchKernel bk;
  mfgpu_desc d = *desc;
  d.mass_coefficient = nullptr;
  int rc = mfgpu::choose_kernel_and_plan(d, pk, bk, p->plan);
  if (!rc && pk != mfgpu::PlaneKernel::none) rc = mfgpu::build_plane_records(p->plan, desc->constraint_mask);
  if (rc) {
    delete p;
    return rc;
  }
  *out = p;
  return 0;
}

void mfgpu_plan_destroy(mfgpu_plan *p) { delete p; }

size_t mfgpu_desc_size(void) { return sizeof(mfgpu_desc); }

int mfgpu_suggest_renumbering(const mfgpu_desc *desc, uint32_t *new_index) {
  if (!desc || !new_index) {
    mfgpu::set_error("null argument");
    return MFGPU_EINVAL;
  }
  mfgpu::Plan P;
  mfgpu::PlaneKernel pk;
  mfgpu::BatchKernel bk;
  mfgpu_desc d = *desc;
  d.mass_coefficient = nullptr;
  int rc = mfgpu::choose_kernel_and_plan(d, pk, bk, P);
  if (rc) return rc;
  const uint32_t NONE = 0xffffffffu;
  std::fill(new_index, new_index + desc->n_dofs, NONE);
  uint32_t next = 0;
  const size_t nb = P.batch_cell_off.size() - 1;
  for (size_t b = 0; b < nb; ++b) {
    const uint32_t d0 = P.batch_dof_off[b];
    const uint32_t ni = P.batch_nint.empty() ? P.batch_dof_off[b + 1] - d0 : P.batch_nint[b];
    for (uint32_t t = 0; t < ni; ++t) {
      const uint32_t g = P.bdofs[d0 + t] & 0x7fffffffu;
      if (new_index[g] == NONE) new_index[g] = next++;
    }
  }
  for (uint32_t e : P.sdofs) {
    const uint32_t g = e & 0x7fffffffu;
    if (new_index[g] == NONE) new_index[g] = next++;
  }
  for (uint32_t g = 0; g < desc->n_dofs; ++g)
    if (new_index[g] == NONE) new_index[g] = next++;
  if (next != desc->n_dofs) {
    mfgpu::set_error("internal: renumbering is not a permutation");
    return MFGPU_EINVAL;
  }
  return 0;
}

int64_t mfgpu_plan_array_u32(const mfgpu_plan *p, int what, const uint32_t **ptr) {
  if (!p || !ptr) return MFGPU_EINVAL;
  const std::vector<uint32_t> *v = nullptr;
  switch (what) {
    case 0: v = &p->plan.batch_cell_off; break;
    case 1: v = &p->plan.batch_dof_off; break;
    case 2: v = &p->plan.color_batch_off; break;
    case 3: v = &p->plan.cell_order; break;
    case 4: v = &p->plan.bdofs; break;
    case 5: v = &p->plan.orphans; break;
    case 6: v = &p->plan.batch_nint; break;
    case 7: v = &p->plan.halo_off; break;
    case 8: v = &p->plan.sdofs; break;
    case 9: v = &p->plan.s_off; break;
    case 10: v = &p->plan.s_idx; break;
    case 11: v = &p->plan.chunks; break;
    case 12: v = &p->plan.gstarts; break;
    case 13: v = &p->plan.pr_dofs; break;
    case 14: v = &p->plan.pr_idx; break;
    case 15: v = &p->plan.pr_hn; break;
    case 16: v = &p->plan.pr_hn_slot; break;
    case 17: v = &p->plan.sh_dofs; break;
    case 18: v = &p->plan.sh_idx; break;
    case 19: v = &p->plan.sh_batch; break;
    case 20: v = &p->plan.sh_p2rec; break;
    case 21: v = &p->plan.sh_p2tab; break;
    default: mfgpu::set_error("bad array id"); return MFGPU_EINVAL;
  }
  *ptr = v->data();
  return (int64_t)v->size();
}

int mfgpu_plan_multi_groups(uint32_t n_vectors, const uint32_t *widths, uint32_t n_widths, uint32_t *groups,
                            uint32_t capacity) {
  if ((!widths && n_widths) || (!groups && capacity)) return MFGPU_EINVAL;
  const std::vector<uint32_t> g = mfgpu::multi_groups(n_vectors, std::vector<uint32_t>(widths, widths + n_widths));
  for (size_t i = 0; i < g.size() && i < capacity; ++i) groups[i] = g[i];
  return (int)g.size();
}

int mfgpu_plan_shares_records(const mfgpu_plan *p) {
  return p ? (p->plan.sh_use ? 1 : 0) | (p->plan.sh_p2_use ? 2 : 0) : 0;
}

int64_t mfgpu_plan_lmap(const mfgpu_plan *p, const uint16_t **ptr) {
  if (!p || !ptr) return MFGPU_EINVAL;
  *ptr = p->plan.lmap.data();
  return (int64_t)p->plan.lmap.size();
}

int64_t mfgpu_plan_bflags(const mfgpu_plan *p, const uint8_t **ptr) {
  if (!p || !ptr) return MFGPU_EINVAL;
  *ptr = p->plan.bflags.data();
  return (int64_t)p->plan.bflags.size();
}

}
```

### dealii-cuda_amd/pymfgpu/__init__.py

```python
from __future__ import annotations

import ctypes as C
import os

import numpy as np

_HERE = os.path.dirname(os.path.abspath(__file__))
LIB_PATH = os.environ.get("MFGPU_LIB") or os.path.join(os.path.dirname(_HERE), "lib", "libmfgpu.so")

F64, F32 = 0, 1
OK, EINVAL = 0, -1
EUNSUPPORTED = -4
MULTI_ADD, MULTI_LOOP, MULTI_FUSED = 1, 2, 4
UNIFORM_J0, HANGING_NODES, COLORED_SCATTER, NO_SHARED_RECORDS = 1, 2, 1 << 8, 1 << 9
UPDATABLE_COEFFICIENTS = 1 << 10
KERNEL_AUTO, KERNEL_PENCILS, KERNEL_PENCILS_X, KERNEL_PLANES, KERNEL_PLANES_2W = 0, 1, 2, 3, 4


class MfgpuError(RuntimeError):
    pass


class Desc(C.Structure):
    _fields_ = [
        ("dim", C.c_int32), ("degree", C.c_int32), ("number_type", C.c_int32), ("flags", C.c_uint32),
        ("n_dofs", C.c_uint32), ("n_cells", C.c_uint32),
        ("loc2glob", C.c_void_p), ("constraint_mask", C.c_void_p),
        ("JxW", C.c_void_p), ("inv_jac", C.c_void_p), ("coefficient", C.c_void_p),
        ("quadrature_points", C.c_void_p), ("shape_values", C.c_void_p), ("shape_gradients", C.c_void_p),
        ("constraint_weights", C.c_void_p), ("constrained_dofs", C.c_void_p),
        ("n_constrained", C.c_uint32), ("max_cells_per_batch", C.c_uint32), ("max_dofs_per_batch", C.c_uint32),
        ("kernel", C.c_uint32), ("cell_loop_segments", C.c_uint32), ("max_workgroups", C.c_uint32),
        ("mass_coefficient", C.c_void_p),
    ]


SYMBOLS = [
    "mfgpu_vmult_multi", "mfgpu_multi_width", "mfgpu_plan_multi_groups",
    "mfgpu_create", "mfgpu_vmult", "mfgpu_vmult_add", "mfgpu_n_dofs", "mfgpu_memory_consumption",
    "mfgpu_destroy", "mfgpu_last_error", "mfgpu_plan_stats", "mfgpu_kernel_name", "mfgpu_compute_inverse_diagonal", "mfgpu_set_constrained_values",
    "mfgpu_vec_sadd", "mfgpu_vec_equ", "mfgpu_vec_scale", "mfgpu_vec_divide", "mfgpu_vec_invert", "mfgpu_vec_mul",
    "mfgpu_vec_dot", "mfgpu_vec_l2_norm", "mfgpu_vec_add_and_dot", "mfgpu_vec_all_zero", "mfgpu_profile_enable", "mfgpu_profile_read", "mfgpu_profile_read_pass2",
    "mfgpu_plan_create", "mfgpu_plan_destroy", "mfgpu_plan_array_u32", "mfgpu_plan_lmap", "mfgpu_plan_bflags",
    "mfgpu_plan_shares_records", "mfgpu_record_stats",
    "mfgpu_vec_alloc", "mfgpu_vec_free", "mfgpu_vec_fill", "mfgpu_vec_from_host", "mfgpu_vec_to_host",
    "mfgpu_device_synchronize", "mfgpu_device_memory_info", "mfgpu_mesh_create_uniform", "mfgpu_mesh_create_adaptive", "mfgpu_mesh_create_ball", "mfgpu_mesh_create_from_leaves",
    "mfgpu_mesh_cell_levels", "mfgpu_mesh_destroy",
    "mfgpu_mesh_desc", "mfgpu_mesh_dof_coords", "mfgpu_mesh_interface_dofs",
    "mfgpu_dist_unique_id", "mfgpu_dist_create", "mfgpu_dist_connect_local", "mfgpu_dist_attach", "mfgpu_dist_schedule",
    "mfgpu_vmult_dist_begin", "mfgpu_vmult_dist_end", "mfgpu_vmult_dist", "mfgpu_dist_destroy",
    "mfgpu_transfer_create", "mfgpu_transfer_create_from_meshes", "mfgpu_transfer_prolongate",
    "mfgpu_transfer_restrict_and_add", "mfgpu_transfer_memory_consumption", "mfgpu_transfer_destroy",
    "mfgpu_mesh_transfer_patches", "mfgpu_suggest_renumbering", "mfgpu_mesh_renumber",
    "mfgpu_level_create", "mfgpu_level_operator", "mfgpu_level_vmult_interface_down", "mfgpu_level_vmult_interface_up",
    "mfgpu_level_destroy", "mfgpu_index_pairs_create", "mfgpu_vec_copy_pairs", "mfgpu_index_pairs_destroy",
    "mfgpu_mesh_create_adaptive_mg", "mfgpu_mg_hierarchy_create", "mfgpu_mg_n_levels", "mfgpu_mg_level_mesh",
    "mfgpu_mg_edge_dofs", "mfgpu_mg_copy_pairs", "mfgpu_mg_transfer_arrays", "mfgpu_mg_hierarchy_destroy",
    "mfgpu_integrator_create", "mfgpu_integrator_rhs", "mfgpu_integrator_l2_error", "mfgpu_integrator_error_points",
    "mfgpu_integrator_destroy",
    "mfgpu_vec_convert", "mfgpu_vec_copy_pairs_convert", "mfgpu_vec_chebyshev_start", "mfgpu_vec_chebyshev_update",
    "mfgpu_desc_size",
    "mfgpu_update_coefficients", "mfgpu_level_update_coefficients", "mfgpu_integrator_update_coefficients",
    "mfgpu_integrator_evaluate",
]

_lib = None


def lib():
    global _lib
    if _lib is None:
        if not os.path.exists(LIB_PATH):
            raise MfgpuError(f"{LIB_PATH} not found: build it with __graft_entry__.build() "
                             "(make -C dealii-cuda_amd); there is no fallback path")
        L = C.CDLL(LIB_PATH)
        L.mfgpu_last_error.restype = C.c_char_p
        L.mfgpu_create.argtypes = [C.POINTER(Desc), C.POINTER(C.c_void_p)]
        L.mfgpu_desc_size.argtypes = []
        L.mfgpu_desc_size.restype = C.c_size_t
        L.mfgpu_vmult.argtypes = [C.c_void_p, C.c_void_p, C.c_void_p, C.c_void_p]
        L.mfgpu_vmult_add.argtypes = [C.c_void_p, C.c_void_p, C.c_void_p, C.c_void_p]
        L.mfgpu_n_dofs.argtypes = [C.c_void_p]
        L.mfgpu_n_dofs.restype = C.c_uint32
        L.mfgpu_memory_consumption.argtypes = [C.c_void_p]
        L.mfgpu_memory_consumption.restype = C.c_size_t
        L.mfgpu_destroy.argtypes = [C.c_void_p]
        L.mfgpu_destroy.restype = None
        L.mfgpu_plan_stats.argtypes = [C.c_void_p, C.POINTER(C.c_uint64)]
        L.mfgpu_device_memory_info.argtypes = [C.POINTER(C.c_size_t), C.POINTER(C.c_size_t)]
        L.mfgpu_kernel_name.argtypes = [C.c_void_p]
        L.mfgpu_kernel_name.restype = C.c_char_p
        L.mfgpu_compute_inverse_diagonal.argtypes = [C.c_void_p, C.c_void_p, C.c_void_p]
        L.mfgpu_set_constrained_values.argtypes = [C.c_void_p, C.c_void_p, C.c_double, C.c_void_p]
        vp, d, z, i = C.c_void_p, C.c_double, C.c_size_t, C.c_int
        L.mfgpu_vec_sadd.argtypes = [vp, d, d, vp, z, i, vp]
        L.mfgpu_vec_equ.argtypes = [vp, d, vp, z, i, vp]
        L.mfgpu_vec_scale.argtypes = [vp, vp, z, i, vp]
        L.mfgpu_vec_divide.argtypes = [vp, vp, z, i, vp]
        L.mfgpu_vec_invert.argtypes = [vp, z, i, vp]
        L.mfgpu_vec_mul.argtypes = [vp, d, z, i, vp]
        L.mfgpu_vec_dot.argtypes = [vp, vp, z, i, vp, C.POINTER(d)]
        L.mfgpu_vec_l2_norm.argtypes = [vp, z, i, vp, C.POINTER(d)]
        L.mfgpu_vec_add_and_dot.argtypes = [vp, d, vp, vp, z, i, vp, C.POINTER(d)]
        L.mfgpu_vec_all_zero.argtypes = [vp, z, i, vp, C.POINTER(i)]
        L.mfgpu_profile_enable.argtypes = [C.c_void_p, C.c_int]
        L.mfgpu_profile_read.argtypes = [C.c_void_p, C.POINTER(C.c_double), C.POINTER(C.c_uint64)]
        L.mfgpu_profile_read_pass2.argtypes = [C.c_void_p, C.POINTER(C.c_double)]
        L.mfgpu_plan_create.argtypes = [C.POINTER(Desc), C.POINTER(C.c_void_p)]
        L.mfgpu_plan_destroy.argtypes = [C.c_void_p]
        L.mfgpu_plan_destroy.restype = None
        L.mfgpu_plan_array_u32.argtypes = [C.c_void_p, C.c_int, C.POINTER(C.c_void_p)]
        L.mfgpu_plan_array_u32.restype = C.c_int64
        L.mfgpu_plan_lmap.argtypes = [C.c_void_p, C.POINTER(C.c_void_p)]
        L.mfgpu_plan_lmap.restype = C.c_int64
        L.mfgpu_plan_bflags.argtypes = [C.c_void_p, C.POINTER(C.c_void_p)]
        L.mfgpu_plan_bflags.restype = C.c_int64
        L.mfgpu_plan_shares_records.argtypes = [C.c_void_p]
        L.mfgpu_record_stats.argtypes = [C.c_void_p, C.POINTER(C.c_uint64)]
        L.mfgpu_vec_alloc.argtypes = [C.POINTER(C.c_void_p), C.c_size_t, C.c_int]
        L.mfgpu_vec_free.argtypes = [C.c_void_p]
        L.mfgpu_vec_fill.argtypes = [C.c_void_p, C.c_size_t, C.c_int, C.c_double, C.c_void_p]
        L.mfgpu_vec_from_host.argtypes = [C.c_void_p, C.c_void_p, C.c_size_t, C.c_int]
        L.mfgpu_vec_to_host.argtypes = [C.c_void_p, C.c_void_p, C.c_size_t, C.c_int]
        L.mfgpu_mesh_create_uniform.argtypes = [C.c_int, C.c_int, C.POINTER(C.c_uint32), C.c_double, C.c_double,
                                                C.c_uint32, C.c_uint32, C.c_int, C.POINTER(C.c_void_p)]
        L.mfgpu_mesh_create_adaptive.argtypes = [C.c_int, C.c_int, C.c_int, C.c_int, C.POINTER(C.c_void_p)]
        L.mfgpu_mesh_create_ball.argtypes = [C.c_int, C.c_int, C.c_int, C.c_int, C.POINTER(C.c_void_p)]
        L.mfgpu_mesh_create_from_leaves.argtypes = [C.c_int, C.c_int, C.c_void_p, C.c_uint32, C.c_int, C.POINTER(C.c_void_p)]
        L.mfgpu_mesh_cell_levels.argtypes = [C.c_void_p, C.POINTER(C.c_void_p)]
        L.mfgpu_mesh_cell_levels.restype = C.c_int64
        L.mfgpu_mesh_destroy.argtypes = [C.c_void_p]
        L.mfgpu_mesh_destroy.restype = None
        L.mfgpu_mesh_desc.argtypes = [C.c_void_p, C.POINTER(Desc)]
        L.mfgpu_mesh_dof_coords.argtypes = [C.c_void_p, C.POINTER(C.c_void_p)]
        L.mfgpu_mesh_dof_coords.restype = C.c_int64
        L.mfgpu_mesh_interface_dofs.argtypes = [C.c_void_p, C.c_int, C.POINTER(C.c_void_p)]
        L.mfgpu_mesh_interface_dofs.restype = C.c_int64
        L.mfgpu_transfer_create.argtypes = [C.c_int, C.c_int, C.c_int, C.c_uint32, C.c_void_p, C.c_void_p, C.c_uint32,
                                            C.c_uint32, C.c_void_p, C.c_uint32, C.c_void_p, C.POINTER(C.c_void_p)]
        L.mfgpu_transfer_create_from_meshes.argtypes = [C.c_void_p, C.c_void_p, C.POINTER(C.c_void_p)]
        L.mfgpu_transfer_prolongate.argtypes = [C.c_void_p, C.c_void_p, C.c_void_p, C.c_void_p]
        L.mfgpu_transfer_restrict_and_add.argtypes = [C.c_void_p, C.c_void_p, C.c_void_p, C.c_void_p]
        L.mfgpu_transfer_memory_consumption.argtypes = [C.c_void_p]
        L.mfgpu_transfer_memory_consumption.restype = C.c_size_t
        L.mfgpu_mesh_transfer_patches.argtypes = [C.c_void_p, C.c_void_p, C.c_void_p, C.c_void_p]
        L.mfgpu_mesh_transfer_patches.restype = C.c_int64
        L.mfgpu_suggest_renumbering.argtypes = [C.POINTER(Desc), C.c_void_p]
        L.mfgpu_mesh_renumber.argtypes = [C.c_void_p, C.c_void_p]
        L.mfgpu_level_create.argtypes = [C.POINTER(Desc), C.c_void_p, C.c_uint32, C.POINTER(C.c_void_p)]
        L.mfgpu_level_operator.argtypes = [C.c_void_p]
        L.mfgpu_level_operator.restype = C.c_void_p
        L.mfgpu_level_vmult_interface_down.argtypes = [C.c_void_p, C.c_void_p, C.c_void_p, C.c_void_p]
        L.mfgpu_level_vmult_interface_up.argtypes = [C.c_void_p, C.c_void_p, C.c_void_p, C.c_void_p]
        L.mfgpu_mesh_create_adaptive_mg.argtypes = [C.c_int, C.c_int, C.c_int, C.c_int, C.POINTER(C.c_void_p)]
        L.mfgpu_mg_hierarchy_create.argtypes = [C.c_void_p, C.POINTER(C.c_void_p)]
        L.mfgpu_mg_n_levels.argtypes = [C.c_void_p]
        L.mfgpu_mg_level_mesh.argtypes = [C.c_void_p, C.c_int]
        L.mfgpu_mg_level_mesh.restype = C.c_void_p
        L.mfgpu_mg_edge_dofs.argtypes = [C.c_void_p, C.c_int, C.POINTER(C.c_void_p)]
        L.mfgpu_mg_edge_dofs.restype = C.c_int64
        L.mfgpu_mg_copy_pairs.argtypes = [C.c_void_p, C.c_int, C.POINTER(C.c_void_p), C.POINTER(C.c_void_p)]
        L.mfgpu_mg_copy_pairs.restype = C.c_int64
        L.mfgpu_mg_transfer_arrays.argtypes = [C.c_void_p, C.c_int, C.POINTER(C.c_void_p), C.POINTER(C.c_void_p)]
        L.mfgpu_mg_transfer_arrays.restype = C.c_int64
        L.mfgpu_mg_hierarchy_destroy.argtypes = [C.c_void_p]
        L.mfgpu_mg_hierarchy_destroy.restype = None
        L.mfgpu_index_pairs_create.argtypes = [C.c_void_p, C.c_void_p, C.c_uint32, C.POINTER(C.c_void_p)]
# ... 106 lines not shown
        return int(self.desc.n_cells)

    @property
    def nd(self):
        return (self.desc.degree + 1) ** self.desc.dim

    def arrays(self):
        d = self.desc
        dt = np_dtype(d.number_type)
        nd, nc, n = self.nd, d.n_cells, d.degree + 1
        out = dict(
            loc2glob=_view(d.loc2glob, nc * nd, np.uint32).reshape(nc, nd),
            JxW=_view(d.JxW, nc * nd, dt).reshape(nc, nd),
            inv_jac=(_view(d.inv_jac, nc, dt) if d.flags & UNIFORM_J0
                     else _view(d.inv_jac, nc * nd * d.dim * d.dim, dt).reshape(nc, nd, d.dim, d.dim)),
            quadrature_points=_view(d.quadrature_points, nc * nd * d.dim, dt).reshape(nc, nd, d.dim),
            shape_values=_view(d.shape_values, n * n, dt),
            shape_gradients=_view(d.shape_gradients, n * n, dt),
            constraint_weights=_view(d.constraint_weights, n * n, np.float64),
            constrained_dofs=_view(d.constrained_dofs, d.n_constrained, np.uint32),
            constraint_mask=_view(d.constraint_mask, nc, np.uint32) if d.constraint_mask else None,
        )
        return out

    def set_mass_coefficient(self, c):
        if c is None:
            self._mass, self.desc.mass_coefficient = None, None
            return
        self._mass = np.ascontiguousarray(c, dtype=np_dtype(self.desc.number_type)).reshape(-1)
        assert self._mass.size == self.n_cells * self.nd
        self.desc.mass_coefficient = self._mass.ctypes.data

    def dof_coords(self):
        p = C.c_void_p()
        cnt = lib().mfgpu_mesh_dof_coords(self._h, C.byref(p))
        return _view(p.value, cnt, np.float64).reshape(-1, self.desc.dim)

    def suggest_renumbering(self):
        out = np.zeros(self.n_dofs, dtype=np.uint32)
        _check(lib().mfgpu_suggest_renumbering(C.byref(self.desc), out.ctypes.data))
        return out

    def renumber(self, new_index):
        ni = np.ascontiguousarray(new_index, dtype=np.uint32)
        assert ni.size == self.n_dofs
        _check(lib().mfgpu_mesh_renumber(self._h, ni.ctypes.data))
        _check(lib().mfgpu_mesh_desc(self._h, C.byref(self.desc)))

    def transfer_patches(self, fine: "Mesh"):
        p, dim = self.desc.degree, self.desc.dim
        cd = np.zeros((self.n_cells, (p + 1) ** dim), dtype=np.uint32)
        fd = np.zeros((self.n_cells, (2 * p + 1) ** dim), dtype=np.uint32)
        rc = lib().mfgpu_mesh_transfer_patches(self._h, fine._h, cd.ctypes.data, fd.ctypes.data)
        if rc < 0:
            _check(int(rc))
        return cd, fd

    def interface_dofs(self, which):
        p = C.c_void_p()
        cnt = lib().mfgpu_mesh_interface_dofs(self._h, which, C.byref(p))
        return _view(p.value, cnt, np.uint32).copy()


def make_desc(dim, degree, n_dofs, loc2glob, JxW, inv_jac, coefficient, constrained,
              shape_values, shape_gradients, number_type=F64, constraint_mask=None,
              constraint_weights=None, quadrature_points=None, max_cells_per_batch=0, max_dofs_per_batch=0,
              colored=False, kernel=0, cell_loop_segments=0, max_workgroups=0, mass_coefficient=None):
    dt = np_dtype(number_type)
    keep = []

    def ptr(a, dtype):
        if a is None:
            return None
        a = np.ascontiguousarray(a, dtype=dtype)
        keep.append(a)
        return a.ctypes.data

    d = Desc()
    d.dim, d.degree, d.number_type = dim, degree, number_type
    l2g = np.ascontiguousarray(loc2glob, dtype=np.uint32)
    d.n_dofs = int(n_dofs)
    d.n_cells = l2g.size // ((degree + 1) ** dim)
    uniform = np.asarray(inv_jac).size == d.n_cells
    assert uniform or np.asarray(inv_jac).size == l2g.size * dim * dim
    d.flags = ((UNIFORM_J0 if uniform else 0) | (HANGING_NODES if constraint_mask is not None else 0)
               | (COLORED_SCATTER if colored else 0))
    d.loc2glob = ptr(l2g, np.uint32)
    d.constraint_mask = ptr(constraint_mask, np.uint32)
    d.JxW = ptr(JxW, dt)
    d.inv_jac = ptr(inv_jac, dt)
    d.coefficient = ptr(coefficient, dt)
    d.quadrature_points = ptr(quadrature_points, dt)
    d.shape_values = ptr(shape_values, dt)
    d.shape_gradients = ptr(shape_gradients, dt)
    d.constraint_weights = ptr(constraint_weights, np.float64)
    c = np.ascontiguousarray(constrained, dtype=np.uint32)
    d.constrained_dofs = ptr(c, np.uint32)
    d.n_constrained = c.size
    d.max_cells_per_batch = max_cells_per_batch
    d.max_dofs_per_batch = max_dofs_per_batch
    d.kernel = kernel
    d.cell_loop_segments = cell_loop_segments
    d.max_workgroups = max_workgroups
    d.mass_coefficient = ptr(mass_coefficient, dt)
    return d, keep


class Plan:

    def __init__(self, desc: Desc, keep=None):
        self._keep = keep
        self.nd = (desc.degree + 1) ** desc.dim
        h = C.c_void_p()
        _check(lib().mfgpu_plan_create(C.byref(desc), C.byref(h)))
        self._h = h

    def __del__(self):
        if getattr(self, "_h", None) and _lib is not None:
            _lib.mfgpu_plan_destroy(self._h)
            self._h = None

    def _u32(self, what):
        p = C.c_void_p()
        cnt = lib().mfgpu_plan_array_u32(self._h, what, C.byref(p))
        if cnt < 0:
            _check(int(cnt))
        return _view(p.value, cnt, np.uint32).copy()

    batch_cell_off = property(lambda s: s._u32(0))
    batch_dof_off = property(lambda s: s._u32(1))
    color_batch_off = property(lambda s: s._u32(2))
    cell_order = property(lambda s: s._u32(3))
    bdofs = property(lambda s: s._u32(4) & np.uint32(0x7fffffff))
    bdofs_constrained = property(lambda s: (s._u32(4) >> np.uint32(31)).astype(bool))
    orphans = property(lambda s: s._u32(5))
    batch_nint = property(lambda s: s._u32(6))
    halo_off = property(lambda s: s._u32(7))
    sdofs = property(lambda s: s._u32(8))
    s_off = property(lambda s: s._u32(9))
    s_idx = property(lambda s: s._u32(10))
    chunks = property(lambda s: s._u32(11).reshape(-1, 4))
    gstarts = property(lambda s: s._u32(12))
    pr_dofs = property(lambda s: s._u32(13))
    pr_idx = property(lambda s: s._u32(14))
    pr_hn = property(lambda s: s._u32(15))
    pr_hn_slot = property(lambda s: s._u32(16))
    sh_dofs = property(lambda s: s._u32(17))
    sh_idx = property(lambda s: s._u32(18))
    sh_batch = property(lambda s: s._u32(19).reshape(-1, 4))
    shares_records = property(lambda s: bool(lib().mfgpu_plan_shares_records(s._h) & 1))
    sh_p2rec = property(lambda s: s._u32(20))
    sh_p2tab = property(lambda s: s._u32(21).reshape(-1, 2))
    shares_pass2_records = property(lambda s: bool(lib().mfgpu_plan_shares_records(s._h) & 2))

    @property
    def lmap(self):
        p = C.c_void_p()
        cnt = lib().mfgpu_plan_lmap(self._h, C.byref(p))
        return _view(p.value, cnt, np.uint16).reshape(-1, self.nd).copy()

    @property
    def bflags(self):
        p = C.c_void_p()
        cnt = lib().mfgpu_plan_bflags(self._h, C.byref(p))
        return _view(p.value, cnt, np.uint8).copy()


class DeviceVector:

    def __init__(self, n, number_type=F64):
        self.n, self.number_type = int(n), number_type
        p = C.c_void_p()
        _check(lib().mfgpu_vec_alloc(C.byref(p), self.n, number_type))
        self.ptr = p.value

    def __del__(self):
        if getattr(self, "ptr", None) and _lib is not None:
            _lib.mfgpu_vec_free(self.ptr)
            self.ptr = None

    def fill(self, value, stream=None):
        _check(lib().mfgpu_vec_fill(self.ptr, self.n, self.number_type, float(value), stream))

    def from_host(self, a):
        a = np.ascontiguousarray(a, dtype=np_dtype(self.number_type))
        assert a.size == self.n
        _check(lib().mfgpu_vec_from_host(self.ptr, a.ctypes.data, self.n, self.number_type))

    def to_host(self):
        a = np.empty(self.n, dtype=np_dtype(self.number_type))
        _check(lib().mfgpu_vec_to_host(a.ctypes.data, self.ptr, self.n, self.number_type))
        return a

    def swap(self, other):
        self.ptr, other.ptr = other.ptr, self.ptr
        self.n, other.n = other.n, self.n

    def _a(self, other=None):
        if other is not None:
            assert other.n == self.n and other.number_type == self.number_type
        return self.n, self.number_type

    def sadd(self, s, a, w, stream=None):
        _check(lib().mfgpu_vec_sadd(self.ptr, float(s), float(a), w.ptr, *self._a(w), stream))

    def add(self, a, w, stream=None):
        self.sadd(1.0, a, w, stream)

    def equ(self, a, w, stream=None):
        _check(lib().mfgpu_vec_equ(self.ptr, float(a), w.ptr, *self._a(w), stream))

    def scale(self, w, stream=None):
        _check(lib().mfgpu_vec_scale(self.ptr, w.ptr, *self._a(w), stream))

    def divide(self, w, stream=None):
        _check(lib().mfgpu_vec_divide(self.ptr, w.ptr, *self._a(w), stream))

    def invert(self, stream=None):
        _check(lib().mfgpu_vec_invert(self.ptr, *self._a(), stream))

    def mul(self, a, stream=None):
        _check(lib().mfgpu_vec_mul(self.ptr, float(a), *self._a(), stream))

    def dot(self, w, stream=None):
        r = C.c_double()
        _check(lib().mfgpu_vec_dot(self.ptr, w.ptr, *self._a(w), stream, C.byref(r)))
        return r.value

    def l2_norm(self, stream=None):
        r = C.c_double()
        _check(lib().mfgpu_vec_l2_norm(self.ptr, *self._a(), stream, C.byref(r)))
        return r.value

    def add_and_dot(self, a, x, w, stream=None):
        r = C.c_double()
        self._a(x)
        _check(lib().mfgpu_vec_add_and_dot(self.ptr, float(a), x.ptr, w.ptr, *self._a(w), stream, C.byref(r)))
        return r.value

    def all_zero(self, stream=None):
        r = C.c_int()
        _check(lib().mfgpu_vec_all_zero(self.ptr, *self._a(), stream, C.byref(r)))
        return bool(r.value)


class Operator:

    def __init__(self, desc: Desc, keep=None):
        self._keep = keep
        self.number_type = desc.number_type
        h = C.c_void_p()
        _check(lib().mfgpu_create(C.byref(desc), C.byref(h)))
        self._h = h

    def __del__(self):
        self.clear()

    def clear(self):
        if getattr(self, "_h", None) and _lib is not None:
            _lib.mfgpu_destroy(self._h)
            self._h = None

    def n(self):
        return int(lib().mfgpu_n_dofs(self._h))

    m = n

    def vmult(self, dst, src, stream=None):
        _check(lib().mfgpu_vmult(self._h, _ptr(dst), _ptr(src), stream))

    def vmult_add(self, dst, src, stream=None):
        _check(lib().mfgpu_vmult_add(self._h, _ptr(dst), _ptr(src), stream))

    def vmult_multi(self, dst, src, n_vectors, stride=None, add=False, mode=None, stream=None):
        flags = (MULTI_ADD if add else 0) | (mode or 0)
        _check(lib().mfgpu_vmult_multi(self._h, _ptr(dst), _ptr(src), int(n_vectors),
                                       self.n() if stride is None else int(stride), flags, stream))

    def multi_width(self):
        return int(lib().mfgpu_multi_width(self._h))

    def memory_consumption(self):
        return int(lib().mfgpu_memory_consumption(self._h))

    def plan_stats(self):
        s = (C.c_uint64 * 8)()
        _check(lib().mfgpu_plan_stats(self._h, s))
        keys = ["n_batches", "n_launches", "batch_dofs", "max_batch_dofs", "max_batch_cells", "n_orphans",
                "first_touch_or_shared_dofs", "rmw_adds_or_halo_slots"]
        out = dict(zip(keys, [int(v) for v in s]))
        r = (C.c_uint64 * 4)()
        _check(lib().mfgpu_record_stats(self._h, r))
        out.update(index_records="shared" if r[0] & 1 else "expanded",
                   pass2_records="shared" if r[0] & 2 else "expanded", distinct_dof_records=int(r[1]),
                   distinct_index_records=int(r[2]), index_record_bytes=int(r[3]))
        return out

    def kernel_name(self):
        return lib().mfgpu_kernel_name(self._h).decode()

    def compute_inverse_diagonal(self, inv_diag, stream=None):
        _check(lib().mfgpu_compute_inverse_diagonal(self._h, _ptr(inv_diag), stream))

    def set_constrained_values(self, vec, value, stream=None):
        _check(lib().mfgpu_set_constrained_values(self._h, _ptr(vec), float(value), stream))

    def update_coefficients(self, coef=None, mass=None, stream=None):
        _check(lib().mfgpu_update_coefficients(self._h, _optr(coef), _optr(mass), stream))

    def profile_enable(self, on=True):
        _check(lib().mfgpu_profile_enable(self._h, int(on)))

    def profile_read(self):
        ms, nv = C.c_double(), C.c_uint64()
        _check(lib().mfgpu_profile_read(self._h, C.byref(ms), C.byref(nv)))
        return ms.value, int(nv.value)

    def profile_read_pass2(self):
        ms = C.c_double()
        _check(lib().mfgpu_profile_read_pass2(self._h, C.byref(ms)))
        return ms.value


class Integrator:

    def __init__(self, desc: Desc, keep=None):
        self._keep = keep
        self.dim, self.degree, self.n_cells = int(desc.dim), int(desc.degree), int(desc.n_cells)
        h = C.c_void_p()
        _check(lib().mfgpu_integrator_create(C.byref(desc), C.byref(h)))
        self._h = h

    def __del__(self):
        if getattr(self, "_h", None) and _lib is not None:
            _lib.mfgpu_integrator_destroy(self._h)
            self._h = None

    @property
    def n_error_points(self):
        return (self.degree + 2) ** self.dim

    def rhs(self, dst, f=None, u_b=None, stream=None):
        _check(lib().mfgpu_integrator_rhs(self._h, _ptr(dst), None if f is None else _ptr(f),
                                          None if u_b is None else _ptr(u_b), stream))

    def l2_error(self, u, exact=None, per_cell=None, stream=None):
        r = C.c_double()
        _check(lib().mfgpu_integrator_l2_error(self._h, _ptr(u), None if exact is None else _ptr(exact),
                                               None if per_cell is None else _ptr(per_cell), stream, C.byref(r)))
        return r.value

    def update_coefficients(self, coef=None, mass=None, stream=None):
        _check(lib().mfgpu_integrator_update_coefficients(self._h, _optr(coef), _optr(mass), stream))

    def evaluate(self, u, values=None, gradients=None, stream=None):
        _check(lib().mfgpu_integrator_evaluate(self._h, _ptr(u), _optr(values), _optr(gradients), stream))

    def error_points(self):
        v = DeviceVector(self.n_cells * self.n_error_points * self.dim)
        _check(lib().mfgpu_integrator_error_points(self._h, v.ptr, None))
        return v.to_host().reshape(self.n_cells, self.n_error_points, self.dim)


class MgHierarchy:

    def __init__(self, mesh: "Mesh"):
        h = C.c_void_p()
        _check(lib().mfgpu_mg_hierarchy_create(mesh._h, C.byref(h)))
        self._h = h
        self.n_levels = int(lib().mfgpu_mg_n_levels(h))

    def level_mesh(self, level):
        m = Mesh.__new__(Mesh)
        m._owner = self
        m._h = C.c_void_p(lib().mfgpu_mg_level_mesh(self._h, level))
        m.desc = Desc()
        _check(lib().mfgpu_mesh_desc(m._h, C.byref(m.desc)))
        return m

    def edge_dofs(self, level):
        p = C.c_void_p()
        n = lib().mfgpu_mg_edge_dofs(self._h, level, C.byref(p))
        return _view(p.value, n, np.uint32).copy()

    def copy_pairs(self, level):
        a, b = C.c_void_p(), C.c_void_p()
        n = lib().mfgpu_mg_copy_pairs(self._h, level, C.byref(a), C.byref(b))
        return _view(a.value, n, np.uint32).copy(), _view(b.value, n, np.uint32).copy()

    def transfer_arrays(self, level, nd, nfd):
        a, b = C.c_void_p(), C.c_void_p()
        n = lib().mfgpu_mg_transfer_arrays(self._h, level, C.byref(a), C.byref(b))
        return _view(a.value, n * nd, np.uint32).reshape(n, nd).copy(), _view(b.value, n * nfd, np.uint32).reshape(n, nfd).copy()

    def __del__(self):
        if getattr(self, "_h", None) and _lib is not None:
            _lib.mfgpu_mg_hierarchy_destroy(self._h)
            self._h = None


class Level:

    def __init__(self, desc: Desc, edge_dofs, keep=None):
        self._keep = keep
        e = np.ascontiguousarray(edge_dofs, dtype=np.uint32)
        h = C.c_void_p()
        _check(lib().mfgpu_level_create(C.byref(desc), e.ctypes.data if e.size else None, e.size, C.byref(h)))
        self._h = h
        self.number_type = desc.number_type

    def vmult(self, dst, src, stream=None):
        _check(lib().mfgpu_vmult(lib().mfgpu_level_operator(self._h), _ptr(dst), _ptr(src), stream))

    def compute_inverse_diagonal(self, inv_diag, stream=None):
        _check(lib().mfgpu_compute_inverse_diagonal(lib().mfgpu_level_operator(self._h), _ptr(inv_diag), stream))

    def update_coefficients(self, coef=None, mass=None, stream=None):
        _check(lib().mfgpu_level_update_coefficients(self._h, _optr(coef), _optr(mass), stream))

    def vmult_interface_down(self, dst, src, stream=None):
        _check(lib().mfgpu_level_vmult_interface_down(self._h, _ptr(dst), _ptr(src), stream))

    def vmult_interface_up(self, dst, src, stream=None):
        _check(lib().mfgpu_level_vmult_interface_up(self._h, _ptr(dst), _ptr(src), stream))

    def __del__(self):
        if getattr(self, "_h", None) and _lib is not None:
            _lib.mfgpu_level_destroy(self._h)
            self._h = None


class Transfer:

    def __init__(self, handle):
        self._h = handle

    @classmethod
    def from_arrays(cls, dim, degree, coarse_cell_dofs, fine_patch_dofs, n_coarse_dofs, n_fine_dofs, coarse_dirichlet,
                    number_type=F64, prolongation_1d=None):
        cd = np.ascontiguousarray(coarse_cell_dofs, dtype=np.uint32)
        fd = np.ascontiguousarray(fine_patch_dofs, dtype=np.uint32)
        di = np.ascontiguousarray(coarse_dirichlet, dtype=np.uint32)
        p1 = None if prolongation_1d is None else np.ascontiguousarray(prolongation_1d, dtype=np.float64)
        n_cells = cd.size // ((degree + 1) ** dim)
        assert fd.size == n_cells * (2 * degree + 1) ** dim
        h = C.c_void_p()
        _check(lib().mfgpu_transfer_create(dim, degree, number_type, n_cells, cd.ctypes.data, fd.ctypes.data, n_coarse_dofs,
                                           n_fine_dofs, di.ctypes.data if di.size else None, di.size,
# ... 152 lines not shown
```

### include/mfgpu.h

```cpp
#ifndef MFGPU_H
#define MFGPU_H

#include <stddef.h>
#include <stdint.h>

#ifdef __cplusplus
extern "C" {
#endif

#define MFGPU_OK 0
#define MFGPU_EINVAL (-1)
#define MFGPU_EHIP (-2)
#define MFGPU_ENOMEM (-3)
#define MFGPU_EUNSUPPORTED (-4)

#define MFGPU_F64 0
#define MFGPU_F32 1

#define MFGPU_UNIFORM_J0 (1u << 0)
#define MFGPU_HANGING_NODES (1u << 1)

#define MFGPU_COLORED_SCATTER (1u << 8)

#define MFGPU_NO_SHARED_RECORDS (1u << 9)

#define MFGPU_UPDATABLE_COEFFICIENTS (1u << 10)

typedef struct mfgpu_handle mfgpu_handle;

typedef struct mfgpu_desc {
  int32_t dim;
  int32_t degree;
  int32_t number_type;
  uint32_t flags;
  uint32_t n_dofs;
  uint32_t n_cells;
  const uint32_t *loc2glob;
  const uint32_t *constraint_mask;
  const void *JxW;
  const void *inv_jac;
  const void *coefficient;
  const void *quadrature_points;
  const void *shape_values;
  const void *shape_gradients;
  const double *constraint_weights;
  const uint32_t *constrained_dofs;
  uint32_t n_constrained;
  uint32_t max_cells_per_batch;
  uint32_t max_dofs_per_batch;
  uint32_t kernel;
  uint32_t cell_loop_segments;
  uint32_t max_workgroups;
  const void *mass_coefficient;
} mfgpu_desc;

size_t mfgpu_desc_size(void);

#define MFGPU_KERNEL_AUTO 0
#define MFGPU_KERNEL_PENCILS 1
#define MFGPU_KERNEL_PENCILS_X 2
#define MFGPU_KERNEL_PLANES 3
#define MFGPU_KERNEL_PLANES_2W 4


int mfgpu_create(const mfgpu_desc *desc, mfgpu_handle **out);

int mfgpu_vmult(mfgpu_handle *h, void *dst_dev, const void *src_dev, void *stream);

int mfgpu_vmult_add(mfgpu_handle *h, void *dst_dev, const void *src_dev, void *stream);

#define MFGPU_MULTI_ADD   (1u << 0)
#define MFGPU_MULTI_LOOP  (1u << 1)
#define MFGPU_MULTI_FUSED (1u << 2)

int mfgpu_vmult_multi(mfgpu_handle *h, void *dst_dev, const void *src_dev, uint32_t n_vectors, size_t stride,
                      uint32_t flags, void *stream);
int mfgpu_multi_width(const mfgpu_handle *h);

int mfgpu_update_coefficients(mfgpu_handle *h, const void *coefficient_dev, const void *mass_coefficient_dev,
                              void *stream);

uint32_t mfgpu_n_dofs(const mfgpu_handle *h);

size_t mfgpu_memory_consumption(const mfgpu_handle *h);

void mfgpu_destroy(mfgpu_handle *h);

const char *mfgpu_last_error(void);

int mfgpu_plan_stats(const mfgpu_handle *h, uint64_t stats[8]);

int mfgpu_record_stats(const mfgpu_handle *h, uint64_t stats[4]);

const char *mfgpu_kernel_name(const mfgpu_handle *h);

int mfgpu_profile_enable(mfgpu_handle *h, int on);
int mfgpu_profile_read(mfgpu_handle *h, double *kernel_ms_total, uint64_t *n_vmults);
int mfgpu_profile_read_pass2(mfgpu_handle *h, double *pass2_ms_total);

typedef struct mfgpu_plan mfgpu_plan;
int mfgpu_plan_create(const mfgpu_desc *desc, mfgpu_plan **out);
void mfgpu_plan_destroy(mfgpu_plan *p);
int64_t mfgpu_plan_array_u32(const mfgpu_plan *p, int what, const uint32_t **ptr);
int mfgpu_plan_shares_records(const mfgpu_plan *p);
int mfgpu_plan_multi_groups(uint32_t n_vectors, const uint32_t *widths, uint32_t n_widths, uint32_t *groups,
                            uint32_t capacity);
int64_t mfgpu_plan_lmap(const mfgpu_plan *p, const uint16_t **ptr);
int64_t mfgpu_plan_bflags(const mfgpu_plan *p, const uint8_t **ptr);

int mfgpu_suggest_renumbering(const mfgpu_desc *desc, uint32_t *new_index );

int mfgpu_compute_inverse_diagonal(mfgpu_handle *h, void *inv_diag, void *stream);
int mfgpu_set_constrained_values(mfgpu_handle *h, void *vec, double value, void *stream);

int mfgpu_vec_sadd(void *v, double s, double a, const void *w, size_t n, int number_type, void *stream);
int mfgpu_vec_equ(void *v, double a, const void *w, size_t n, int number_type, void *stream);
int mfgpu_vec_scale(void *v, const void *w, size_t n, int number_type, void *stream);
int mfgpu_vec_divide(void *v, const void *w, size_t n, int number_type, void *stream);
int mfgpu_vec_invert(void *v, size_t n, int number_type, void *stream);
int mfgpu_vec_mul(void *v, double a, size_t n, int number_type, void *stream);
int mfgpu_vec_dot(const void *v, const void *w, size_t n, int number_type, void *stream, double *result);
int mfgpu_vec_l2_norm(const void *v, size_t n, int number_type, void *stream, double *result);
int mfgpu_vec_add_and_dot(void *v, double a, const void *x, const void *w, size_t n, int number_type,
                          void *stream, double *result);
int mfgpu_vec_all_zero(const void *v, size_t n, int number_type, void *stream, int *result);

int mfgpu_vec_alloc(void **dev, size_t n, int number_type);
int mfgpu_vec_free(void *dev);
int mfgpu_vec_fill(void *dev, size_t n, int number_type, double value, void *stream);
int mfgpu_vec_from_host(void *dev, const void *host, size_t n, int number_type);
int mfgpu_vec_to_host(void *host, const void *dev, size_t n, int number_type);
int mfgpu_device_synchronize(void);
int mfgpu_device_memory_info(size_t *free_bytes, size_t *total_bytes);

typedef struct mfgpu_dist mfgpu_dist;
int mfgpu_dist_unique_id(void *id128);
int mfgpu_dist_create(const void *id128, int rank, int world, const uint32_t *lower_ids, uint32_t n_lower,
                      const uint32_t *upper_ids, uint32_t n_upper, const uint32_t *constrained_dofs,
                      uint32_t n_constrained, uint32_t n_dofs, int number_type, mfgpu_dist **out);
int mfgpu_dist_connect_local(mfgpu_dist *lower_rank, mfgpu_dist *upper_rank);
int mfgpu_dist_attach(mfgpu_dist *d, mfgpu_handle *h);
int mfgpu_dist_schedule(const mfgpu_dist *d, uint32_t info[4]);
int mfgpu_vmult_dist_begin(mfgpu_handle *h, mfgpu_dist *d, void *dst_dev, const void *src_dev, void *stream);
int mfgpu_vmult_dist_end(mfgpu_handle *h, mfgpu_dist *d, void *dst_dev, void *stream);
int mfgpu_vmult_dist(mfgpu_handle *h, mfgpu_dist *d, void *dst_dev, const void *src_dev, void *stream);
void mfgpu_dist_destroy(mfgpu_dist *d);

typedef struct mfgpu_transfer mfgpu_transfer;
int mfgpu_transfer_create(int dim, int degree, int number_type, uint32_t n_coarse_cells,
                          const uint32_t *coarse_cell_dofs ,
                          const uint32_t *fine_patch_dofs  , uint32_t n_coarse_dofs,
                          uint32_t n_fine_dofs, const uint32_t *coarse_dirichlet, uint32_t n_coarse_dirichlet,
                          const double *prolongation_1d ,
                          mfgpu_transfer **out);
int mfgpu_transfer_prolongate(mfgpu_transfer *t, void *dst_fine_dev, const void *src_coarse_dev, void *stream);
int mfgpu_transfer_restrict_and_add(mfgpu_transfer *t, void *dst_coarse_dev, const void *src_fine_dev, void *stream);
size_t mfgpu_transfer_memory_consumption(const mfgpu_transfer *t);
void mfgpu_transfer_destroy(mfgpu_transfer *t);

typedef struct mfgpu_level mfgpu_level;
int mfgpu_level_create(const mfgpu_desc *desc, const uint32_t *edge_dofs, uint32_t n_edge, mfgpu_level **out);
mfgpu_handle *mfgpu_level_operator(mfgpu_level *level);
int mfgpu_level_vmult_interface_down(mfgpu_level *level, void *dst_dev, const void *src_dev, void *stream);
int mfgpu_level_vmult_interface_up(mfgpu_level *level, void *dst_dev, const void *src_dev, void *stream);
int mfgpu_level_update_coefficients(mfgpu_level *level, const void *coefficient_dev, const void *mass_coefficient_dev,
                                    void *stream);
void mfgpu_level_destroy(mfgpu_level *level);

typedef struct mfgpu_index_pairs mfgpu_index_pairs;
int mfgpu_index_pairs_create(const uint32_t *dst_idx, const uint32_t *src_idx, uint32_t n, mfgpu_index_pairs **out);
int mfgpu_vec_copy_pairs(const mfgpu_index_pairs *p, void *dst_dev, const void *src_dev, int number_type, void *stream);
void mfgpu_index_pairs_destroy(mfgpu_index_pairs *p);

int mfgpu_vec_convert(void *dst, int dst_type, const void *src, int src_type, size_t n, void *stream);
int mfgpu_vec_copy_pairs_convert(const mfgpu_index_pairs *p, void *dst, int dst_type, const void *src, int src_type,
                                 void *stream);
int mfgpu_vec_chebyshev_start(void *x, void *upd, void *r, const void *b, const void *t, const void *dinv, double f,
                              int zero_start, size_t n, int number_type, void *stream);
int mfgpu_vec_chebyshev_update(void *x, void *upd, void *r, const void *t, const void *dinv, double f1, double f2,
                               size_t n, int number_type, void *stream);

typedef struct mfgpu_integrator mfgpu_integrator;
int mfgpu_integrator_create(const mfgpu_desc *desc, mfgpu_integrator **out);
int mfgpu_integrator_rhs(mfgpu_integrator *it, void *rhs, const void *f_qp, const void *u_b, void *stream);
int mfgpu_integrator_l2_error(mfgpu_integrator *it, const void *u, const void *exact, void *per_cell, void *stream,
                              double *l2);
int mfgpu_integrator_error_points(mfgpu_integrator *it, void *points, void *stream);
int mfgpu_integrator_update_coefficients(mfgpu_integrator *it, const void *coefficient_dev,
                                         const void *mass_coefficient_dev, void *stream);
int mfgpu_integrator_evaluate(mfgpu_integrator *it, const void *u, void *values_qp, void *gradients_qp, void *stream);
void mfgpu_integrator_destroy(mfgpu_integrator *it);

typedef struct mfgpu_mesh mfgpu_mesh;

int mfgpu_mesh_create_uniform(int dim, int degree, const uint32_t *n_per_dir, double lo, double hi,
                              uint32_t slab_begin, uint32_t slab_end, int number_type,
                              mfgpu_mesh **out);
int mfgpu_mesh_create_adaptive(int dim, int degree, int n_ref, int number_type, mfgpu_mesh **out);
int mfgpu_mesh_create_ball(int dim, int degree, int n_ref, int number_type, mfgpu_mesh **out);
int mfgpu_transfer_create_from_meshes(const mfgpu_mesh *coarse, const mfgpu_mesh *fine, mfgpu_transfer **out);
int64_t mfgpu_mesh_transfer_patches(const mfgpu_mesh *coarse, const mfgpu_mesh *fine, uint32_t *coarse_cell_dofs,
                                    uint32_t *fine_patch_dofs);
int mfgpu_mesh_renumber(mfgpu_mesh *m, const uint32_t *new_index);
int mfgpu_mesh_create_adaptive_mg(int dim, int degree, int n_ref, int number_type, mfgpu_mesh **out);
typedef struct mfgpu_mg_hierarchy mfgpu_mg_hierarchy;
int mfgpu_mg_hierarchy_create(const mfgpu_mesh *adaptive, mfgpu_mg_hierarchy **out);
int mfgpu_mg_n_levels(const mfgpu_mg_hierarchy *h);
const mfgpu_mesh *mfgpu_mg_level_mesh(const mfgpu_mg_hierarchy *h, int level);
int64_t mfgpu_mg_edge_dofs(const mfgpu_mg_hierarchy *h, int level, const uint32_t **ptr);
int64_t mfgpu_mg_copy_pairs(const mfgpu_mg_hierarchy *h, int level, const uint32_t **active_dofs, const uint32_t **level_dofs);
int64_t mfgpu_mg_transfer_arrays(const mfgpu_mg_hierarchy *h, int level, const uint32_t **coarse_cell_dofs,
                                 const uint32_t **fine_patch_dofs);
void mfgpu_mg_hierarchy_destroy(mfgpu_mg_hierarchy *h);
int mfgpu_mesh_create_from_leaves(int dim, int degree, const uint32_t *leaves, uint32_t n_leaves,
                                  int number_type, mfgpu_mesh **out);
int64_t mfgpu_mesh_cell_levels(const mfgpu_mesh *m, const uint32_t **ptr);
void mfgpu_mesh_destroy(mfgpu_mesh *m);
int mfgpu_mesh_desc(const mfgpu_mesh *m, mfgpu_desc *desc);
int64_t mfgpu_mesh_dof_coords(const mfgpu_mesh *m, const double **ptr);
int64_t mfgpu_mesh_interface_dofs(const mfgpu_mesh *m, int which, const uint32_t **ptr);

#ifdef __cplusplus
}
#endif
#endif
```

Before: 81.58 billion DoFs/s.

## Let owning batch store shared dofs directly to dst instead of halo

Each shared dof on a plane batch gets an owner batch. In pass 1 that batch writes its partial sum straight into the destination vector rather than into a halo slot. Pass 2 then reads that partial from dst, and skips the dof entirely when it has only one toucher. The aim is less halo traffic and fewer pass-2 reads and writes. The costs are a flag bit stolen from dof ids, an ownership mask in the shared pass-2 records, and a padding-target change that must avoid conflicting writes.

Result: slower. 71.59 billion DoFs/s (-12.2%).

```diff
diff --git a/dealii-cuda_amd/csrc/mfgpu_api.hip b/dealii-cuda_amd/csrc/mfgpu_api.hip
--- a/dealii-cuda_amd/csrc/mfgpu_api.hip
+++ b/dealii-cuda_amd/csrc/mfgpu_api.hip
@@ -87,6 +87,8 @@
   std::vector<uint32_t> n_p2tiles;
   DeviceArray<uint32_t> d_p2rec, d_p2tab;
   bool p2_shared = false, p2_reverse = false, no_shared_records = false;
+  bool owner_store = false;
+  uint64_t n_owner_stored = 0, n_dof_records = 0;
   Stream side;
   std::vector<Event> ev_seg;
   Event ev_side;
@@ -190,7 +192,7 @@
   const bool shared = P.sh_p2_use && !h->no_shared_records && n_priority == 0 && ng == 2;
   std::vector<std::vector<uint32_t>> sd(ng), so(ng, std::vector<uint32_t>(1, 0u)), si(ng);
   auto add = [&](uint32_t dof, const uint32_t *slots, uint32_t k, size_t seg) {
-    const size_t g = prio[dof & 0x7fffffffu] ? 0 : 1 + seg;
+    const size_t g = prio[dof & (h->owner_store ? kDofIdMask : 0x7fffffffu)] ? 0 : 1 + seg;
     sd[g].push_back(dof);
     si[g].insert(si[g].end(), slots, slots + k);
     so[g].push_back((uint32_t)si[g].size());
@@ -204,7 +206,8 @@
       seg = (size_t)(std::upper_bound(h->seg_end.begin(), h->seg_end.end(), batch) - h->seg_end.begin());
       if (seg >= h->seg_end.size()) seg = h->seg_end.size() - 1;
     }
-    add(P.sdofs[i], P.s_idx.data() + P.s_off[i], P.s_off[i + 1] - P.s_off[i], seg);
+    const bool own = h->owner_store && i < P.s_own.size() && P.s_own[i];
+    add(P.sdofs[i] | (own ? kOwnerStoreBit : 0u), P.s_idx.data() + P.s_off[i], P.s_off[i + 1] - P.s_off[i], seg);
   }
   const uint32_t zero_slot = P.halo_off.empty() ? 0u : P.halo_off.back();
   for (uint32_t orph : P.orphans) add(orph, &zero_slot, 1, 0);
@@ -214,7 +217,10 @@
   DeviceArray<uint32_t> d_rec, d_tab;
   if (shared) {
     int rc;
-    if ((rc = d_rec.upload(P.sh_p2rec.data(), P.sh_p2rec.size()))) return rc;
+    std::vector<uint32_t> marked;
+    if (h->owner_store) mark_owner_stores_pass2(P, marked);
+    const std::vector<uint32_t> &rec = h->owner_store ? marked : P.sh_p2rec;
+    if ((rc = d_rec.upload(rec.data(), rec.size()))) return rc;
     if ((rc = d_tab.upload(P.sh_p2tab.data(), P.sh_p2tab.size()))) return rc;
   }
   for (size_t g = 0; g < ng; ++g) {
@@ -321,11 +327,20 @@
     }
     h->shared_records = P.sh_use && !(d.flags & MFGPU_NO_SHARED_RECORDS) &&
                         kernel_exists(h->planes, P.n, d.number_type, false, true, d.mass_coefficient != nullptr);
-    const std::vector<uint32_t> &rd = h->shared_records ? P.sh_dofs : P.pr_dofs;
+    h->owner_store = h->twopass && owner_store_exists(h->planes) && !(d.flags & MFGPU_NO_OWNER_STORE);
+    std::vector<uint32_t> m_dofs, m_sh_dofs, m_sh_batch;
+    if (h->owner_store) {
+      mark_owner_stores(P, m_dofs, m_sh_dofs, m_sh_batch);
+      for (const uint32_t o : P.s_own) h->n_owner_stored += o;
+    }
+    const std::vector<uint32_t> &rd = h->shared_records ? (h->owner_store ? m_sh_dofs : P.sh_dofs)
+                                                        : (h->owner_store ? m_dofs : P.pr_dofs);
     const std::vector<uint32_t> &rx = h->shared_records ? P.sh_idx : P.pr_idx;
+    const std::vector<uint32_t> &rb = h->owner_store ? m_sh_batch : P.sh_batch;
+    h->n_dof_records = (h->owner_store ? m_sh_dofs : P.sh_dofs).size() / ((size_t)p_kgu(P.n) * 64);
     if ((rc = up(h->d_bdofsp, rd.data(), rd.size()))) return rc;
     if ((rc = up(h->d_idxp, rx.data(), rx.size()))) return rc;
-    if (h->shared_records && (rc = up(h->d_shtab, P.sh_batch.data(), P.sh_batch.size()))) return rc;
+    if (h->shared_records && (rc = up(h->d_shtab, rb.data(), rb.size()))) return rc;
     h->record_bytes = h->d_bdofsp.bytes() + h->d_idxp.bytes() + h->d_shtab.bytes();
   }
   if ((rc = up(h->d_orphans, P.orphans.data(), P.orphans.size()))) return rc;
@@ -477,7 +492,7 @@
                                            h->d_p2tab.get(), (uint32_t)(h->plan.batch_cell_off.size() - 1),
                                            (uint32_t)p_hs(h->plan.n) * 64u, h->p2_reverse ? 1 : 0, add, st));
   HIP_TRY(reduce_classes_launch<T>((T *)dst, (const T *)src, h->d_halo.as<const T>(), h->d_p2arr[group].get(),
-                                   h->d_p2tiles[group].get(), h->n_p2tiles[group], add, st));
+                                   h->d_p2tiles[group].get(), h->n_p2tiles[group], add, h->owner_store ? 1 : 0, st));
   return 0;
 }
 
@@ -971,15 +986,17 @@
   return 0;
 }
 
-int mfgpu_record_stats(const mfgpu_handle *h, uint64_t s[4]) {
+int mfgpu_record_stats(const mfgpu_handle *h, uint64_t s[6]) {
   if (!h || !s) return MFGPU_EINVAL;
   const Plan &P = h->plan;
-  const size_t n = (size_t)P.n, nb = (size_t)p_kgu((int)n) * 64, nx = ((n * n + 1) / 2) * (p_cells_per_wave((int)n) * n);
+  const size_t n = (size_t)P.n, nx = ((n * n + 1) / 2) * (p_cells_per_wave((int)n) * n);
   const bool planes = h->planes != PlaneKernel::none;
   s[0] = (h->shared_records ? 1 : 0) | (h->p2_shared ? 2 : 0);
-  s[1] = planes ? P.sh_dofs.size() / nb : 0;
+  s[1] = planes ? h->n_dof_records : 0;
   s[2] = planes ? P.sh_idx.size() / nx : 0;
   s[3] = h->record_bytes;
+  s[4] = h->owner_store ? 1 : 0;
+  s[5] = h->n_owner_stored;
   return 0;
 }
 
diff --git a/dealii-cuda_amd/csrc/mfgpu_internal.h b/dealii-cuda_amd/csrc/mfgpu_internal.h
--- a/dealii-cuda_amd/csrc/mfgpu_internal.h
+++ b/dealii-cuda_amd/csrc/mfgpu_internal.h
@@ -73,6 +73,7 @@
   bool sh_use = false;
   std::vector<uint32_t> sh_p2rec, sh_p2tab;
   bool sh_p2_use = false;
+  std::vector<uint32_t> s_own, batch_nown, batch_pad;
   uint64_t n_first = 0, n_add = 0;
 };
 
@@ -119,7 +120,14 @@
 constexpr double kShareMaxFraction = 0.5;
 void share_plane_records(Plan &plan);
 constexpr int kP2Header = 16, kP2MaxK = 12, kP2SlotBits = 12;
+constexpr int kP2OwnRow = 3 + kP2MaxK;
 void share_pass2_records(Plan &plan);
+
+constexpr uint32_t kOwnerStoreBit = 1u << 30, kDofIdMask = kOwnerStoreBit - 1u;
+constexpr bool owner_store_exists(PlaneKernel k) { return k == PlaneKernel::planes3; }
+void mark_owner_stores(const Plan &plan, std::vector<uint32_t> &pr_dofs, std::vector<uint32_t> &sh_dofs,
+                       std::vector<uint32_t> &sh_batch);
+void mark_owner_stores_pass2(const Plan &plan, std::vector<uint32_t> &sh_p2rec);
 
 int derive_tables(int n, const double *shape_values, const double *shape_gradients,
                   std::vector<double> &S, std::vector<double> &Dt);
diff --git a/dealii-cuda_amd/csrc/mfgpu_kernels.h b/dealii-cuda_amd/csrc/mfgpu_kernels.h
--- a/dealii-cuda_amd/csrc/mfgpu_kernels.h
+++ b/dealii-cuda_amd/csrc/mfgpu_kernels.h
@@ -139,7 +139,7 @@
                          const std::vector<uint32_t> &s_idx, std::vector<uint32_t> &arr, std::vector<uint32_t> &tiles);
 template <typename T>
 hipError_t reduce_classes_launch(T *dst, const T *src, const T *halo, const uint32_t *arr, const uint32_t *tiles,
-                                 uint32_t n_tiles, int add, hipStream_t st);
+                                 uint32_t n_tiles, int add, int marks, hipStream_t st);
 template <typename T>
 hipError_t reduce_classes_multi_launch(int nv, T *dst, const T *src, size_t stride, T *const *halos, const uint32_t *arr,
                                        const uint32_t *tiles, uint32_t n_tiles, int add, hipStream_t st);
diff --git a/dealii-cuda_amd/csrc/mfgpu_kernels_p.hip b/dealii-cuda_amd/csrc/mfgpu_kernels_p.hip
--- a/dealii-cuda_amd/csrc/mfgpu_kernels_p.hip
+++ b/dealii-cuda_amd/csrc/mfgpu_kernels_p.hip
@@ -106,8 +106,9 @@
     if (j < JI) {
       *dst_at(base, g) = ADD ? oldv + r : r;
     } else {
-      T *const hp = A.halo + (size_t)bb * (HS * 64) + lane;
-      hp[(j - JI) * 64] = r;
+      T *hp = A.halo + (size_t)bb * (HS * 64) + lane + (j - JI) * 64;
+      if (!ADD) hp = (g & kOwnerStoreBit) ? dst_at(base, g) : hp;
+      *hp = r;
     }
   };
 
diff --git a/dealii-cuda_amd/csrc/mfgpu_pass2.hip b/dealii-cuda_amd/csrc/mfgpu_pass2.hip
--- a/dealii-cuda_amd/csrc/mfgpu_pass2.hip
+++ b/dealii-cuda_amd/csrc/mfgpu_pass2.hip
@@ -11,7 +11,7 @@
 template <typename T, int K>
 __device__ __forceinline__ void reduce_two(T *__restrict__ dst, const T *__restrict__ src, const T *__restrict__ halo,
                                            const uint32_t *__restrict__ p, uint32_t cnt, uint32_t i0, uint32_t k,
-                                           int add) {
+                                           int add, int marks) {
   const uint32_t i1 = i0 + 256u;
   const uint32_t d0 = p[i0], d1 = p[i1];
   constexpr int KU = K > 0 ? K : 1;
@@ -22,15 +22,18 @@
     s1[t] = p[(size_t)(1 + t) * cnt + i1];
   }
   const bool on0 = d0 != 0xffffffffu, on1 = d1 != 0xffffffffu;
-  const uint32_t g0 = d0 & 0x7fffffffu, g1 = d1 & 0x7fffffffu;
+  const uint32_t idm = marks ? kDofIdMask : 0x7fffffffu;
+  const uint32_t g0 = d0 & idm, g1 = d1 & idm;
+  const bool own0 = marks && !add && (d0 & kOwnerStoreBit), own1 = marks && !add && (d1 & kOwnerStoreBit);
   T v0 = T(0), v1 = T(0), o0 = T(0), o1 = T(0);
   if (on0) {
     if (d0 >> 31) {
       v0 = src[g0];
     } else {
       T q[KU];
-#pragma unroll
-      for (int t = 0; t < KU; ++t) q[t] = halo[s0[t]];
+      q[0] = *(own0 ? (const T *)(dst + g0) : halo + s0[0]);
+#pragma unroll
+      for (int t = 1; t < KU; ++t) q[t] = halo[s0[t]];
       v0 = q[0];
 #pragma unroll
       for (int t = 1; t < KU; ++t) v0 += q[t];
@@ -44,8 +47,9 @@
       v1 = src[g1];
     } else {
       T q[KU];
-#pragma unroll
-      for (int t = 0; t < KU; ++t) q[t] = halo[s1[t]];
+      q[0] = *(own1 ? (const T *)(dst + g1) : halo + s1[0]);
+#pragma unroll
+      for (int t = 1; t < KU; ++t) q[t] = halo[s1[t]];
       v1 = q[0];
 #pragma unroll
       for (int t = 1; t < KU; ++t) v1 += q[t];
@@ -54,24 +58,24 @@
     }
     if (add) o1 = dst[g1];
   }
-  if (on0) dst[g0] = add ? o0 + v0 : v0;
-  if (on1) dst[g1] = add ? o1 + v1 : v1;
+  if (on0 && !(own0 && k == 1u)) dst[g0] = add ? o0 + v0 : v0;
+  if (on1 && !(own1 && k == 1u)) dst[g1] = add ? o1 + v1 : v1;
 }
 
 template <typename T>
 __global__ void __launch_bounds__(256)
 reduce_classes(T *__restrict__ dst, const T *__restrict__ src, const T *__restrict__ halo,
-               const uint32_t *__restrict__ arr, const uint4 *__restrict__ tiles, int add) {
+               const uint32_t *__restrict__ arr, const uint4 *__restrict__ tiles, int add, int marks) {
   const uint4 td = tiles[blockIdx.x];
   const uint32_t *p = arr + td.x;
   const uint32_t i0 = td.w + threadIdx.x;
   switch (td.y) {
-    case 1: reduce_two<T, 1>(dst, src, halo, p, td.z, i0, 1, add); break;
-    case 2: reduce_two<T, 2>(dst, src, halo, p, td.z, i0, 2, add); break;
-    case 3: reduce_two<T, 3>(dst, src, halo, p, td.z, i0, 3, add); break;
-    case 4: reduce_two<T, 4>(dst, src, halo, p, td.z, i0, 4, add); break;
-    case 8: reduce_two<T, 8>(dst, src, halo, p, td.z, i0, 8, add); break;
-    default: reduce_two<T, 0>(dst, src, halo, p, td.z, i0, td.y, add); break;
+    case 1: reduce_two<T, 1>(dst, src, halo, p, td.z, i0, 1, add, marks); break;
+    case 2: reduce_two<T, 2>(dst, src, halo, p, td.z, i0, 2, add, marks); break;
+    case 3: reduce_two<T, 3>(dst, src, halo, p, td.z, i0, 3, add, marks); break;
+    case 4: reduce_two<T, 4>(dst, src, halo, p, td.z, i0, 4, add, marks); break;
+    case 8: reduce_two<T, 8>(dst, src, halo, p, td.z, i0, 8, add, marks); break;
+    default: reduce_two<T, 0>(dst, src, halo, p, td.z, i0, td.y, add, marks); break;
   }
 }
 
@@ -167,13 +171,17 @@
 #pragma unroll
   for (int t = 0; t < KU; ++t) w[t] = (uint32_t)t < kk ? r[r[3 + t] + e] : 0u;
   if (d == 0xffffffffu) return;
+  const bool own = !add && (d & kOwnerStoreBit);
+  if (own && kk == 1u) return;
+  T *const out = dst + (d & kDofIdMask);
   T v;
   if (d >> 31) {
-    v = src[d & 0x7fffffffu];
+    v = src[d & kDofIdMask];
   } else {
     T q[KU];
-#pragma unroll
-    for (int t = 0; t < KU; ++t) q[t] = (uint32_t)t < kk ? partial(w[t]) : T(0);
+    q[0] = own ? *out : partial(w[0]);
+#pragma unroll
+    for (int t = 1; t < KU; ++t) q[t] = (uint32_t)t < kk ? partial(w[t]) : T(0);
     v = q[0];
 #pragma unroll
     for (int t = 1; t < KU; ++t)
@@ -182,7 +190,6 @@
       for (uint32_t t = 1; t < kw; ++t)
         if (t < kk) v += partial(r[r[3 + t] + e]);
   }
-  T *const out = dst + (d & 0x7fffffffu);
   *out = add ? *out + v : v;
 }
 
@@ -251,10 +258,10 @@
 
 template <typename T>
 hipError_t reduce_classes_launch(T *dst, const T *src, const T *halo, const uint32_t *arr, const uint32_t *tiles,
-                                 uint32_t n_tiles, int add, hipStream_t st) {
+                                 uint32_t n_tiles, int add, int marks, hipStream_t st) {
   if (n_tiles == 0) return hipSuccess;
   hipLaunchKernelGGL(reduce_classes<T>, dim3(n_tiles), dim3(256), 0, st, dst, src, halo, arr,
-                     reinterpret_cast<const uint4 *>(tiles), add);
+                     reinterpret_cast<const uint4 *>(tiles), add, marks);
   return hipGetLastError();
 }
 template <typename T>
@@ -288,8 +295,8 @@
 template hipError_t reduce_owner_batches_launch<float>(float *, const float *, const float *, const uint32_t *,
                                                        const uint32_t *, uint32_t, uint32_t, int, int, hipStream_t);
 template hipError_t reduce_classes_launch<double>(double *, const double *, const double *, const uint32_t *,
-                                                  const uint32_t *, uint32_t, int, hipStream_t);
+                                                  const uint32_t *, uint32_t, int, int, hipStream_t);
 template hipError_t reduce_classes_launch<float>(float *, const float *, const float *, const uint32_t *,
-                                                 const uint32_t *, uint32_t, int, hipStream_t);
-
-}
+                                                 const uint32_t *, uint32_t, int, int, hipStream_t);
+
+}
diff --git a/dealii-cuda_amd/csrc/mfgpu_plan.cpp b/dealii-cuda_amd/csrc/mfgpu_plan.cpp
--- a/dealii-cuda_amd/csrc/mfgpu_plan.cpp
+++ b/dealii-cuda_amd/csrc/mfgpu_plan.cpp
@@ -503,6 +503,37 @@
     if (la != lb) return la < lb;
     return a < b2;
   };
+  std::vector<uint8_t> own(N, 0);
+  std::vector<uint32_t> pad_target(nb, NONE);
+  auto plane_batch = [&](uint32_t b) { return interior_max && (!batch_masked[b] || masked_planes); };
+  if (interior_max) {
+    std::vector<uint8_t> is_target(N, 0);
+    for (uint32_t b = 0; b < nb; ++b) {
+      if (!plane_batch(b)) continue;
+      uint32_t best = NONE;
+      bool best_mine = false;
+      for (size_t t = nint[b]; t < bd[b].size(); ++t) {
+        const uint32_t g = bd[b][t];
+        if (constrained[g]) {
+          best = g;
+          break;
+        }
+        const bool mine = order[touchers[t_off[sid[g]]]] == b;
+        if (best == NONE || (mine && !best_mine) || (mine == best_mine && ntouch[g] > ntouch[best])) {
+          best = g;
+          best_mine = mine;
+        }
+      }
+      pad_target[b] = best;
+      if (best != NONE) is_target[best] = 1;
+    }
+    for (size_t i = 0; i < ns; ++i) {
+      const uint32_t g = shared_ids[i];
+      if (constrained[g] || is_target[g] || t_off[i + 1] == t_off[i]) continue;
+      own[g] = plane_batch(order[touchers[t_off[i]]]);
+    }
+  }
+  auto owned_by = [&](uint32_t g, uint32_t b) { return own[g] && order[touchers[t_off[sid[g]]]] == b; };
   auto same_group = [&](uint32_t a, uint32_t b2) {
     const uint32_t la = t_off[a + 1] - t_off[a], lb = t_off[b2 + 1] - t_off[b2];
     return la == lb && std::equal(&touchers[t_off[a]], &touchers[t_off[a]] + la, &touchers[t_off[b2]]);
@@ -512,8 +543,11 @@
   std::sort(sorder.begin(), sorder.end(), seq_less);
   std::vector<uint32_t> spos(N, NONE);
   for (size_t i = 0; i < ns; ++i) spos[shared_ids[sorder[i]]] = (uint32_t)i;
-  for (uint32_t b = 0; b < nb; ++b)
+  std::vector<uint32_t> nown(nb, 0);
+  for (uint32_t b = 0; b < nb; ++b) {
     std::sort(bd[b].begin() + nint[b], bd[b].end(), [&](uint32_t x, uint32_t y) { return spos[x] < spos[y]; });
+    for (size_t t = nint[b]; t < bd[b].size(); ++t) nown[b] += owned_by(bd[b][t], b) ? 1u : 0u;
+  }
 
   P.cell_order.clear();
   P.cell_order.reserve(nc);
@@ -527,11 +561,18 @@
   P.max_batch_dofs = P.max_batch_cells = 0;
   P.n_first = P.n_add = 0;
   P.batch_nint.clear();
+  P.batch_nown.clear();
+  P.batch_pad.clear();
   P.halo_off.assign(1, 0);
   for (uint32_t k = 0; k < nb; ++k) {
     const uint32_t b = order[k];
     const std::vector<uint32_t> &v = bd[b];
     P.batch_nint.push_back(nint[b]);
+    if (interior_max) {
+      P.batch_nown.push_back(nown[b]);
+      const auto it = std::find(v.begin() + nint[b], v.end(), pad_target[b]);
+      P.batch_pad.push_back(it == v.end() ? nint[b] : (uint32_t)(it - v.begin()));
+    }
     P.halo_off.push_back(P.halo_off.back() +
                          (interior_max && (!batch_masked[b] || masked_planes) ? limits->halo_stride
                                                                               : (uint32_t)(v.size() - nint[b])));
@@ -572,9 +613,11 @@
     if (!touched[g]) P.orphans.push_back(g | (constrained[g] ? 0x80000000u : 0u));
   {
     P.sdofs.resize(ns);
+    P.s_own.assign(interior_max ? ns : 0, 0u);
     for (size_t i = 0; i < ns; ++i) {
       const uint32_t g = shared_ids[sorder[i]];
       P.sdofs[i] = g | (constrained[g] ? 0x80000000u : 0u);
+      if (interior_max) P.s_own[i] = own[g];
     }
     P.s_off.assign(ns + 1, 0);
     for (size_t i = 0; i < ns; ++i) P.s_off[i + 1] = P.s_off[i] + ntouch[P.sdofs[i] & 0x7fffffffu];
@@ -631,11 +674,16 @@
       set_error("internal: batch does not fit the plane kernel's dof-list slots");
       return MFGPU_EINVAL;
     }
+    const uint32_t pad = b < P.batch_pad.size() ? P.batch_pad[b] : ni;
+    if (pad < ni || pad >= nbd) {
+      set_error("internal: a batch's padding target is not a dof pass 2 writes");
+      return MFGPU_EINVAL;
+    }
     slot_of.assign(nbd, 0u);
     for (uint32_t t = 0; t < nbd; ++t) slot_of[t] = t < ni ? t : (uint32_t)JI + (t - ni);
     for (int t = 0; t < NB; ++t) {
       uint32_t src_t;
-      if (t < JI) src_t = (uint32_t)t < ni ? (uint32_t)t : ni;
+      if (t < JI) src_t = (uint32_t)t < ni ? (uint32_t)t : pad;
       else src_t = std::min<uint32_t>(ni + (uint32_t)(t - JI), nbd - 1);
       bd[b * NB + t] = P.bdofs[d0 + src_t];
     }
@@ -771,6 +819,7 @@
   P.sh_p2tab.assign(2 * nb, 0u);
   std::unordered_multimap<uint64_t, std::pair<uint32_t, uint32_t>> seen;
   std::vector<uint32_t> rec;
+  size_t host_only = 0;
   for (size_t b = 0; b < nb; ++b) {
     std::vector<uint32_t> &m = owned[b];
     auto k_of = [&](uint32_t i) { return P.s_off[i + 1] - P.s_off[i]; };
@@ -795,6 +844,14 @@
         rec[rec[3 + t] + e] = ((tb - (uint32_t)b) << kP2SlotBits) | (slot - tb * hs);
       }
     }
+    uint32_t mark_words = 0;
+    if (!P.s_own.empty()) {
+      rec[kP2OwnRow] = (uint32_t)rec.size();
+      rec.resize(rec.size() + e0 / 32, 0u);
+      mark_words = e0 / 32;
+      for (uint32_t e = 0; e < ne; ++e)
+        if (P.s_own[m[e]]) rec[rec[kP2OwnRow] + e / 32] |= 1u << (e % 32);
+    }
     const uint64_t h = hash_words(rec.data(), rec.size());
     uint32_t off = 0xffffffffu;
     const auto range = seen.equal_range(h);
@@ -806,12 +863,52 @@
       off = (uint32_t)P.sh_p2rec.size();
       P.sh_p2rec.insert(P.sh_p2rec.end(), rec.begin(), rec.end());
       seen.emplace(h, std::make_pair(off, (uint32_t)rec.size()));
+      host_only += mark_words;
     }
     P.sh_p2tab[2 * b] = base;
     P.sh_p2tab[2 * b + 1] = off;
   }
-  const size_t shared = P.sh_p2rec.size() + P.sh_p2tab.size();
+  const size_t shared = P.sh_p2rec.size() - host_only + P.sh_p2tab.size();
   P.sh_p2_use = (double)shared <= kShareMaxFraction * (double)expanded;
+}
+
+void mark_owner_stores(const Plan &P, std::vector<uint32_t> &dofs, std::vector<uint32_t> &sh_dofs,
+                       std::vector<uint32_t> &sh_batch) {
+  const size_t NB = (size_t)p_kgu(P.n) * 64, JI = (size_t)p_ji(P.n) * 64, nbat = P.n_plane_batches;
+  dofs = P.pr_dofs;
+  std::vector<uint32_t> owner(P.n_dofs, 0xffffffffu);
+  for (size_t i = 0; i < P.s_own.size(); ++i)
+    if (P.s_own[i])
+      owner[P.sdofs[i] & 0x7fffffffu] =
+          (uint32_t)(std::upper_bound(P.halo_off.begin(), P.halo_off.end(), P.s_idx[P.s_off[i]]) - P.halo_off.begin()) - 1u;
+  for (size_t b = 0; b < nbat; ++b) {
+    const uint32_t np2 = P.batch_dof_off[b + 1] - P.batch_dof_off[b] - P.batch_nint[b];
+    for (uint32_t t = 0; t < np2; ++t)
+      if (owner[dofs[b * NB + JI + t] & 0x7fffffffu] == (uint32_t)b) dofs[b * NB + JI + t] |= kOwnerStoreBit;
+  }
+  sh_dofs.clear();
+  sh_batch = P.sh_batch;
+  std::unordered_multimap<uint64_t, uint32_t> seen;
+  std::vector<uint32_t> rel(NB);
+  for (size_t b = 0; b < nbat; ++b) {
+    const uint32_t base = sh_batch[b * kShBatchWords];
+    for (size_t t = 0; t < NB; ++t) rel[t] = dofs[b * NB + t] - base;
+    sh_batch[b * kShBatchWords + 1] = intern_record(sh_dofs, seen, rel.data(), NB);
+  }
+}
+
+void mark_owner_stores_pass2(const Plan &P, std::vector<uint32_t> &rec) {
+  rec = P.sh_p2rec;
+  std::vector<uint32_t> offs;
+  for (size_t b = 0; 2 * b + 1 < P.sh_p2tab.size(); ++b) offs.push_back(P.sh_p2tab[2 * b + 1]);
+  std::sort(offs.begin(), offs.end());
+  offs.erase(std::unique(offs.begin(), offs.end()), offs.end());
+  for (const uint32_t off : offs) {
+    uint32_t *r = rec.data() + off;
+    if (!r[kP2OwnRow]) continue;
+    for (uint32_t e = 0; e < r[0]; ++e)
+      if ((r[r[kP2OwnRow] + e / 32] >> (e % 32)) & 1u) r[kP2Header + e] |= kOwnerStoreBit;
+  }
 }
 
 int choose_kernel_and_plan(const mfgpu_desc &d, PlaneKernel &pk, BatchKernel &bk, Plan &plan) {
@@ -980,6 +1077,9 @@
     case 19: v = &p->plan.sh_batch; break;
     case 20: v = &p->plan.sh_p2rec; break;
     case 21: v = &p->plan.sh_p2tab; break;
+    case 22: v = &p->plan.s_own; break;
+    case 23: v = &p->plan.batch_nown; break;
+    case 24: v = &p->plan.batch_pad; break;
     default: mfgpu::set_error("bad array id"); return MFGPU_EINVAL;
   }
   *ptr = v->data();
diff --git a/dealii-cuda_amd/pymfgpu/__init__.py b/dealii-cuda_amd/pymfgpu/__init__.py
--- a/dealii-cuda_amd/pymfgpu/__init__.py
+++ b/dealii-cuda_amd/pymfgpu/__init__.py
@@ -13,6 +13,7 @@
 EUNSUPPORTED = -4
 MULTI_ADD, MULTI_LOOP, MULTI_FUSED = 1, 2, 4
 UNIFORM_J0, HANGING_NODES, COLORED_SCATTER, NO_SHARED_RECORDS = 1, 2, 1 << 8, 1 << 9
+NO_OWNER_STORE = 1 << 11
 UPDATABLE_COEFFICIENTS = 1 << 10
 KERNEL_AUTO, KERNEL_PENCILS, KERNEL_PENCILS_X, KERNEL_PLANES, KERNEL_PLANES_2W = 0, 1, 2, 3, 4
 
@@ -425,6 +426,9 @@
     sh_p2rec = property(lambda s: s._u32(20))
     sh_p2tab = property(lambda s: s._u32(21).reshape(-1, 2))
     shares_pass2_records = property(lambda s: bool(lib().mfgpu_plan_shares_records(s._h) & 2))
+    s_own = property(lambda s: s._u32(22))
+    batch_nown = property(lambda s: s._u32(23))
+    batch_pad = property(lambda s: s._u32(24))
 
     @property
     def lmap(self):
@@ -562,11 +566,12 @@
         keys = ["n_batches", "n_launches", "batch_dofs", "max_batch_dofs", "max_batch_cells", "n_orphans",
                 "first_touch_or_shared_dofs", "rmw_adds_or_halo_slots"]
         out = dict(zip(keys, [int(v) for v in s]))
-        r = (C.c_uint64 * 4)()
+        r = (C.c_uint64 * 6)()
         _check(lib().mfgpu_record_stats(self._h, r))
         out.update(index_records="shared" if r[0] & 1 else "expanded",
                    pass2_records="shared" if r[0] & 2 else "expanded", distinct_dof_records=int(r[1]),
-                   distinct_index_records=int(r[2]), index_record_bytes=int(r[3]))
+                   distinct_index_records=int(r[2]), index_record_bytes=int(r[3]),
+                   owner_store=bool(r[4]), owner_stored_dofs=int(r[5]))
         return out
 
     def kernel_name(self):
diff --git a/include/mfgpu.h b/include/mfgpu.h
--- a/include/mfgpu.h
+++ b/include/mfgpu.h
@@ -23,6 +23,8 @@
 #define MFGPU_COLORED_SCATTER (1u << 8)
 
 #define MFGPU_NO_SHARED_RECORDS (1u << 9)
+
+#define MFGPU_NO_OWNER_STORE (1u << 11)
 
 #define MFGPU_UPDATABLE_COEFFICIENTS (1u << 10)
 
@@ -90,7 +92,7 @@
 
 int mfgpu_plan_stats(const mfgpu_handle *h, uint64_t stats[8]);
 
-int mfgpu_record_stats(const mfgpu_handle *h, uint64_t stats[4]);
+int mfgpu_record_stats(const mfgpu_handle *h, uint64_t stats[6]);
 
 const char *mfgpu_kernel_name(const mfgpu_handle *h);
 
```
